# DeepakSridhar/fgdm

Hardware: AMD Instinct MI355X
Metric: 512x512 images/sec @ 50 DDIM steps, seg-ControlNet+CFG (higher is better)
Workload: dtype f16

## Files before the change

fgdm_amd/_lib.py:

```python
import ctypes as C
import os

HERE = os.path.dirname(os.path.abspath(__file__))
LIB_PATH = os.path.join(HERE, 'libfgdm_hip.so')

MAX_LEVELS = 8
MAX_CONTROLNETS = 4

FLAG_USE_ORIGINAL = 1
FLAG_ONLY_MID_CONTROL = 2
FLAG_NO_CONTROL = 4
FLAG_CFG_PAIRS = 8

ACT_NONE, ACT_SILU, ACT_RELU, ACT_GEGLU, ACT_QGELU = 0, 1, 2, 3, 4
OUT_F16, OUT_F32, OUT_F32_NCHW, OUT_F16_T = 0, 1, 2, 3
STRIDE2_PAD_BR = -2


class FgdmConfig(C.Structure):
    _fields_ = [
        ('in_channels', C.c_int32), ('out_channels', C.c_int32), ('model_channels', C.c_int32),
        ('num_res_blocks', C.c_int32), ('n_levels', C.c_int32), ('channel_mult', C.c_int32 * MAX_LEVELS),
        ('n_attention_resolutions', C.c_int32), ('attention_resolutions', C.c_int32 * MAX_LEVELS),
        ('num_heads', C.c_int32), ('context_dim', C.c_int32), ('use_adapter', C.c_int32),
        ('n_controlnets', C.c_int32), ('hint_channels', C.c_int32), ('workspace_bytes', C.c_int64),
        ('vae_ch', C.c_int32), ('vae_n_levels', C.c_int32), ('vae_ch_mult', C.c_int32 * MAX_LEVELS),
        ('vae_num_res_blocks', C.c_int32), ('vae_z_channels', C.c_int32), ('vae_out_ch', C.c_int32),
        ('clip_layers', C.c_int32), ('clip_width', C.c_int32), ('clip_heads', C.c_int32), ('clip_mlp', C.c_int32),
        ('clip_vocab', C.c_int32), ('clip_max_len', C.c_int32),
        ('n_extra_adapters', C.c_int32),
        ('vae_encoder', C.c_int32),
    ]


class FgdmConfig2(FgdmConfig):
    _fields_ = [('num_head_channels', C.c_int32), ('use_linear_in_transformer', C.c_int32)]


class FgdmDdimParams(C.Structure):
    _fields_ = [('struct_size', C.c_int64)] + [(name, C.c_void_p) for name in (
        'x', 'cond', 'uncond', 'timesteps', 'alphas', 'alphas_prev', 'sqrt_one_minus_alphas', 'control_scales', 'sigmas',
        'cfg_scales', 'step_noise', 'mask', 'x0', 'q_noise', 'sqrt_alphas_cumprod_t', 'sqrt_one_minus_alphas_cumprod_t',
        'log_steps', 'x_inter_out', 'pred_x0_out')] + [('cfg_scale', C.c_float)] + [(name, C.c_int32) for name in (
            'S', 'B', 'H', 'W', 'flags', 'n_log', 'reserved0')]


class FgdmPlmsParams(C.Structure):
    _fields_ = [('struct_size', C.c_int64)] + [(name, C.c_void_p) for name in (
        'x', 'cond', 'uncond', 'timesteps', 'alphas', 'alphas_prev', 'sqrt_one_minus_alphas', 'control_scales', 'mask', 'x0',
        'q_noise', 'sqrt_alphas_cumprod_t', 'sqrt_one_minus_alphas_cumprod_t', 'log_steps', 'x_inter_out', 'pred_x0_out')] + [
            ('cfg_scale', C.c_float)] + [(name, C.c_int32) for name in ('S', 'B', 'H', 'W', 'flags', 'n_log', 'reserved0')]


class FgdmDpmppParams(C.Structure):
    _fields_ = [('struct_size', C.c_int64)] + [(name, C.c_void_p) for name in (
        'x', 'cond', 'uncond', 'control_scales', 't_float', 'inv_alpha', 'neg_sigma_over_alpha', 'update_kind', 'c1', 'cm0',
        'cm1')] + [('cfg_scale', C.c_float)] + [(name, C.c_int32) for name in (
            'n_eval', 'B', 'H', 'W', 'flags', 'reserved0', 'reserved1')]


DPMPP_FIRST, DPMPP_SECOND = 1, 2
PLMS_PROBE, PLMS_FINISH_FIRST, PLMS_MULTISTEP = 0, 1, 2

_p = C.c_void_p
_f = C.c_float
_i = C.c_int
_i64 = C.c_int64

SIGNATURES = {
    'fgdm_create': (_i, [C.POINTER(FgdmConfig), _i, C.POINTER(_p)]),
    'fgdm_destroy': (None, [_p]),
    'fgdm_last_error': (C.c_char_p, [_p]),
    'fgdm_param_count': (_i, [C.POINTER(FgdmConfig)]),
    'fgdm_param_info': (_i, [C.POINTER(FgdmConfig), _i, C.c_char_p, _i, C.POINTER(_i64), C.POINTER(_i)]),
    'fgdm_load_tensor': (_i, [_p, C.c_char_p, _p, _i, C.POINTER(_i64), _i]),
    'fgdm_finalize_weights': (_i, [_p]),
    'fgdm_set_hint': (_i, [_p, _i, _p, _i, _i, _i, _p]),
    'fgdm_set_concat': (_i, [_p, _p, _i, _i, _i, _i, _p]),
    'fgdm_set_adapter_conds': (_i, [_p, _p, _i, _i, _i, _i, _p]),
    'fgdm_set_context': (_i, [_p, _p, _i, _p]),
    'fgdm_apply_model': (_i, [_p, _p, _p, _p, _p, _p, _p, _i, _i, _i, _i, _p, _p]),
    'fgdm_clip_encode': (_i, [_p, _p, _i, _i, _p, _p]),
    'fgdm_clip_encode_skip': (_i, [_p, _p, _i, _i, _i, _p, _p]),
    'fgdm_set_context_tokens': (_i, [_p, _i]),
    'fgdm_get_context_tokens': (_i, [_p]),
    'fgdm_run_block': (_i, [_p, C.c_char_p, _p, _i, _p, _i, _p, _p, _i, _i, _i, _p, _i64, C.POINTER(_i64), _p]),
    'fgdm_vae_decode': (_i, [_p, _p, _i, _i, _i, _f, _p, _p]),
    'fgdm_vae_encode': (_i, [_p, _p, _i, _i, _i, _p, _p]),
    'fgdm_unfold': (_i, [_p] + [_i] * 10 + [_p, _p]),
    'fgdm_fold_weighted': (_i, [_p, _p, _p] + [_i] * 9 + [_p, _p]),
    'fgdm_vae_decode_patches': (_i, [_p, _p, _i, _i, _i, _f] + [_i] * 5 + [_p, _p, _i, _p, _p]),
    'fgdm_apply_model_patches': (_i, [_p, _p, _p, _p, _p] + [_i] * 7 + [_p, _p, _i, _i, _p, _p]),
    'fgdm_posterior_sample': (_i, [_p, _p, _f, _p, _i, _i, _i, _p]),
    'fgdm_image_to_uint8': (_i, [_p, _i, _i, _i, _i, _i, _p, _p]),
    'fgdm_resize_linear_uint8': (_i, [_p, _i, _i, _i, _i, _i, _i, _p, _p]),
    'fgdm_uint8_to_hint': (_i, [_p, _i, _i, _i, _i, _p, _p]),
    'fgdm_controlnet': (_i, [_p, _i, _p, _p, _p, _i, _i, _i, _p, _i64, _p]),
    'fgdm_ddim_step': (_i, [_p, _p, _p, _f, _f, _f, _f, _f, _p, _p, _p, _p, _i64, _p]),
    'fgdm_plms_combine': (_i, [_p, _p, _p, _p, _i, _p, _i64, _p]),
    'fgdm_axpby': (_i, [_p, _f, _p, _f, _p, _i64, _p]),
    'fgdm_mask_blend': (_i, [_p, _p, _p, _p, _i64, _p]),
    'fgdm_ancestral_step': (_i, [_p, _p, _f, _f, _f, _f, _f, _p, _p, _i64, _p]),
    'fgdm_sample_ddim': (_i, [_p, _p, _p, _p, _f, _i, C.POINTER(_i64), C.POINTER(_f), C.POINTER(_f), C.POINTER(_f),
                              _p, _i, _i, _i, _i, _p]),
    'fgdm_sample_ddim_ex': (_i, [_p, C.POINTER(FgdmDdimParams), _p]),
    'fgdm_op_ddim_loop_step': (_i, [_p, _p, _p, _f, _f, _f, _f, _f, _p, _p, _p, _p, _f, _f, _p, _p, _p, _p, _p, _i64, _p]),
    'fgdm_sample_plms': (_i, [_p, C.POINTER(FgdmPlmsParams), _p]),
    'fgdm_sample_dpmpp': (_i, [_p, C.POINTER(FgdmDpmppParams), _p]),
    'fgdm_op_plms_loop_step': (_i, [_p, _p, _p, _f, _i, _i, _p, _p, _p, _p, _f, _f, _f, _p, _p, _p, _f, _f, _p, _p, _p, _p, _p,
                                    _i64, _p]),
    'fgdm_op_dpmpp_loop_step': (_i, [_p, _p, _p, _f, _f, _f, _p, _i, _f, _f, _f, _p, _p, _p, _p, _i64, _p]),
    'fgdm_profile_begin': (_i, [_p, _i]),
    'fgdm_profile_end': (_i, [_p, C.POINTER(C.c_double)]),
    'fgdm_workspace_stats': (_i, [_p, C.POINTER(_i64), C.POINTER(_i64)]),
    'fgdm_launch_stats': (_i, [_p, C.POINTER(_i64), C.POINTER(_i64), C.POINTER(_i64)]),
    'fgdm_replay_plan': (_i, [_i, _p, _p, _p, _p, _i, _i, _p, _i, _p]),
    'fgdm_op_conv2d': (_i, [_p, _i, _p, _i, _p, _p, _p, _p, _i, _i, _i, _i, _i, _i, _i, _i, _f, _p, _p]),
    'fgdm_op_linear': (_i, [_p, _p, _p, _p, _i, _i, _i, _i, _i, _i, _i, _p, _p]),
    'fgdm_debug_force_igemm_cfg': (_i, [_i]),
    'fgdm_bench_igemm': (_i, [_i] * 13 + [C.POINTER(_f)]),
    'fgdm_op_linear_ln_linear': (_i, [_p] * 8 + [_i] * 5 + [_p, _p, C.POINTER(_i), _p]),
    'fgdm_bench_norm': (_i, [_i] * 7 + [C.POINTER(_f)]),
    'fgdm_bench_attention': (_i, [_i] * 6 + [C.POINTER(_f)]),
    'fgdm_bench_ff': (_i, [_i] * 4 + [C.POINTER(_f)]),
    'fgdm_op_groupnorm': (_i, [_p, _i, _p, _i, _i, _i, _p, _p, _f, _i, _p, _p]),
    'fgdm_op_layernorm': (_i, [_p, _i, _i, _p, _p, _f, _p, _p]),
    'fgdm_op_attention': (_i, [_p, _i, _p, _i, _p, _i, _p, _i, _i, _i, _i, _i, _i, _p]),
    'fgdm_op_attention_ex': (_i, [_p, _i, _p, _i, _p, _i, _p, _i, _i, _i, _i, _i, _i, _i, _p]),
    'fgdm_debug_last_attention_kernel': (_i, []),
    'fgdm_op_small_attention': (_i, [_p, _i, _i, _i, _p, _i, _i, _i, _i, _i, _i, _p]),
    'fgdm_op_vae_attention': (_i, [_p, _p, _p, _p, _i, _i, _i, _p]),
    'fgdm_op_softmax_rows': (_i, [_p, _p, _i, _i, _p]),
    'fgdm_op_nchw_to_nhwc': (_i, [_p, _p, _i, _i, _i, _i, _p]),
    'fgdm_op_nhwc_to_nchw': (_i, [_p, _p, _i, _i, _i, _p]),
    'fgdm_op_pack_xcat': (_i, [_p, _p, _i, _i, _i, _i, _i, _i, _p, _p]),
    'fgdm_op_avgpool2': (_i, [_p, _p, _i, _i, _i, _i, _p]),
    'fgdm_op_transpose_pad': (_i, [_p, _p, _i, _i, _i, _i, _p]),
    'fgdm_op_timestep_embed': (_i, [_p, _p, _p, _i, _i, _i, _p]),
    'fgdm_op_add_f16': (_i, [_p, _p, _p, _i64, _p]),
    'fgdm_op_ln_qkv': (_i, [_p] * 6 + [_i] * 5 + [_p, _p, _p]),
}

_lib = None


def load():
    global _lib
    if _lib is not None:
        return _lib
    try:
        import torch
    except ImportError:
        pass
    path = os.environ.get('FGDM_LIB') or LIB_PATH
    if not os.path.exists(path):
        raise RuntimeError(f'{path} not found: build it with `python -m fgdm_amd.build` '
                           '(the HIP engine is mandatory, there is no CPU fallback)')
    lib = C.CDLL(os.path.abspath(path))
    for name, (res, args) in SIGNATURES.items():
        fn = getattr(lib, name)
        fn.restype = res
        fn.argtypes = args
    _lib = lib
    return lib
```

fgdm_amd/csrc/common.h:

```cpp
#pragma once
#include <hip/hip_runtime.h>
#include <stdint.h>

typedef _Float16 half_t;
typedef _Float16 h8 __attribute__((ext_vector_type(8)));
typedef _Float16 h4 __attribute__((ext_vector_type(4)));
typedef _Float16 h2 __attribute__((ext_vector_type(2)));
typedef float f32x16 __attribute__((ext_vector_type(16)));
typedef float f32x4 __attribute__((ext_vector_type(4)));

__device__ __forceinline__ float gelu_f(float x) {
    const float z = fminf(fabsf(x), 6.0f);
    float p = -4.7132482596e-04f;
    p = __builtin_fmaf(p, z, 7.0652551839e-03f);
    p = __builtin_fmaf(p, z, -5.1762067461e-02f);
    p = __builtin_fmaf(p, z, -4.6008771426e-01f);
    p = __builtin_fmaf(p, z, -1.1507295505e+00f);
    p = __builtin_fmaf(p, z, -4.8959157159e-05f - 1.0f);
    const float t = __builtin_amdgcn_exp2f(p);
    return __builtin_fmaf(fabsf(x), 0.5f - t, 0.5f * x);
}

typedef float f32x2 __attribute__((ext_vector_type(2)));
__device__ __forceinline__ f32x2 gelu2_f(f32x2 x) {
    const f32x2 ax = {fabsf(x[0]), fabsf(x[1])};
    const f32x2 z = {fminf(ax[0], 6.0f), fminf(ax[1], 6.0f)};
    auto c = [](float k) { return f32x2{k, k}; };
    f32x2 p = c(-4.7132482596e-04f);
    p = __builtin_elementwise_fma(p, z, c(7.0652551839e-03f));
    p = __builtin_elementwise_fma(p, z, c(-5.1762067461e-02f));
    p = __builtin_elementwise_fma(p, z, c(-4.6008771426e-01f));
    p = __builtin_elementwise_fma(p, z, c(-1.1507295505e+00f));
    p = __builtin_elementwise_fma(p, z, c(-4.8959157159e-05f - 1.0f));
    const f32x2 t = {__builtin_amdgcn_exp2f(p[0]), __builtin_amdgcn_exp2f(p[1])};
    return __builtin_elementwise_fma(ax, c(0.5f) - t, c(0.5f) * x);
}

__device__ __forceinline__ float silu_f(float x, float k = 1.0f) {
    return x * __builtin_amdgcn_rcpf(1.0f + __builtin_amdgcn_exp2f(-1.4426950408889634f * k * x));
}

__device__ __forceinline__ float ln_scale(float acc, float mean, float rstd, float u) {
    float t, w;
    asm("v_fma_f32 %0, %1, %2, %3" : "=v"(t) : "v"(-mean), "v"(u), "v"(acc));
    asm("v_mul_f32 %0, %1, %2" : "=v"(w) : "v"(rstd), "v"(t));
    return w;
}

#define FGDM_OK 0
#define FGDM_ERR_ARG -1
#define FGDM_ERR_HIP -2
#define FGDM_ERR_STATE -3
#define FGDM_ERR_NOMEM -4

enum IgemmMode { IG_LINEAR = 0, IG_CONV3 = 1, IG_CONV3_S2 = 2, IG_CONV3_UP2 = 3, IG_CONV3_S2_BR = 4, IG_CONV2_PHASE = 5 };
enum IgemmAct { ACT_NONE = 0, ACT_SILU = 1, ACT_RELU = 2, ACT_GEGLU = 3, ACT_QGELU = 4  };
enum IgemmOut { OUT_F16 = 0, OUT_F32 = 1, OUT_F32_NCHW = 2, OUT_F16_T = 3 };

struct IgemmArgs {
    const half_t* A0;
    const half_t* A1;
    const half_t* Wt;
    const float* bias;
    const float* rowvec;
    const half_t* resid;
    void* out;
    const half_t* zero;
    int C0, C1;
    int B, H, W;
    int Ho, Wo;
    int M, N;
    int K;
    int mode, act, out_kind;
    int ld_out, ld_res;
    int rv_stride;
    int rows_per_sample;
    float scale;
    int force_cfg;
    int splitk;
    float* ws;
    int debug;
    const float* ln_stats;
    const float* ln_u;
    int ln_slots;
    float ln_eps;
    float* stats_out;
    void* out2;
    int split_n, out_kind2, ld_out2;
};

int igemm_launch(const IgemmArgs& a, hipStream_t s);
bool igemm_up_phase(const IgemmArgs& a);
IgemmArgs igemm_phase_args(const IgemmArgs& a, const half_t* wt_phase);
void igemm_set_force_cfg(int cfg);
void igemm_set_twin_layers(bool on);
void igemm_set_pair_hint(int mult);
int igemm2_launch(const IgemmArgs& a, int cfg, hipStream_t s);
int igemm_stats_slots(const IgemmArgs& a);
int row_stats_slots(int C);
int row_stats_launch(const half_t* x, int rows, int C, float* stats , hipStream_t s);
int igemm_splitk_factor(const IgemmArgs& a);
int igemm_splitk_reduce(const IgemmArgs& a, hipStream_t s);
size_t igemm_npad(int n);

#define GN_PIX_PER_CHUNK 256
void groupnorm_set_group(bool on);
int groupnorm_launch(const half_t* x0, int C0, const half_t* x1, int C1, int B, int HW,
                     const float* gamma, const float* beta, float eps, int silu,
                     half_t* out, float* ws , hipStream_t s);
size_t groupnorm_ws_floats(int B, int HW);
int layernorm_launch(const half_t* x, int rows, int C, const float* gamma, const float* beta, float eps,
                     half_t* out, hipStream_t s);

int attention_launch(const half_t* Q, int ldq, const half_t* K, int ldk, const half_t* Vt, int ldvt,
                     half_t* O, int ldo, int B, int H, int T, int Tk, int d, int q_prescaled, hipStream_t s);
int attention_last_kernel();

int nchw_f32_to_nhwc_f16(const float* x, half_t* y, int B, int C, int HW, int Cpad, hipStream_t s);
int pack_xcat(const float* x, const half_t* cc, half_t* y, int B, int Bc, int Cc, int HW, int Cpad, hipStream_t s);
int f32_to_f16(const float* x, half_t* y, size_t n, hipStream_t s);
int silu_f32_to_f16(const float* x, half_t* y, size_t n, hipStream_t s);
int nhwc_f16_to_nchw_f32(const half_t* x, float* y, int B, int C, int HW, hipStream_t s);
int im2col3x3(const half_t* x, half_t* A, int B, int H, int W, int C, int stride, int Kpad, hipStream_t s);
int avgpool2(const half_t* x, half_t* y, int B, int H, int W, int C, hipStream_t s);
int add_f16(const half_t* a, const half_t* b, half_t* y, size_t n, hipStream_t s);
int add_f16_to_f32(const float* a, const half_t* b, float* y, size_t n, hipStream_t s);
int timestep_embed(const int64_t* t, const float* t_float, half_t* y, int B, int dim, int rows_pad, hipStream_t s);
int vae_prequant(const float* z, const float* wb, float scale, half_t* y, int B, int HW, hipStream_t s);
int vae_moments(const float* h, const float* wb, float* moments, int B, int HW, hipStream_t s);
int posterior_sample(const float* moments, const float* noise, float scale, float* z, int B, int zc, int HW, hipStream_t s);
int softmax_rows(const float* S, half_t* P, int rows, int cols, hipStream_t s);
int image_to_u8(const float* x, uint8_t* y, int B, int C, int HW, int mode, hipStream_t s);
int resize_linear_u8(const uint8_t* src, uint8_t* dst, int B, int H, int W, int C, int Ho, int Wo, hipStream_t s);
int u8_to_hint(const uint8_t* src, float* dst, int B, int HW, int C, hipStream_t s);
int embed_tokens(const int64_t* ids, const float* tok, const float* pos, float* out, int rows, int T, int W, int vocab,
                 hipStream_t s);
int layernorm32_launch(const float* x, int rows, int C, const float* gamma, const float* beta, float eps, half_t* out16,
                       float* out32, hipStream_t s);
int f16_to_f32(const half_t* x, float* y, size_t n, hipStream_t s);
int small_attention_launch(const half_t* qkv, int ld, int koff, int voff, half_t* out, int ldo, int B, int heads, int T,
                           int d, int causal, hipStream_t s);
int transpose_pad_keys(const half_t* v, half_t* vt, int B, int Tk, int C, int Tkpad, hipStream_t s);
int ddim_step(const float* x, const float* e_cond, const float* e_uncond, float cfg_scale,
              float a_t, float a_prev, float sigma_t, float sqrt_one_minus_at, const float* noise,
              float* x_prev, float* pred_x0, float* e_out, size_t n, hipStream_t s);
struct DdimLoopStep {
    const float *x, *ec, *eu, *noise, *mask, *x0, *qnoise;
    float *x_out, *xin_a, *xin_b, *log_x, *log_p0;
    float cfg, a_t, a_prev, sigma, s1m, sa_next, s1m_next;
    size_t n;
};
int ddim_loop_step(const DdimLoopStep& a, hipStream_t s);
enum { PLMS_PROBE = 0, PLMS_FINISH_FIRST = 1, PLMS_MULTISTEP = 2 };
struct PlmsLoopStep {
    const float *x, *ec, *eu, *e1, *e2, *e3, *mask, *x0, *qnoise;
    float *e_out, *x_out, *xin_a, *xin_b, *log_x, *log_p0;
    float cfg, a_t, a_prev, s1m, sa_next, s1m_next;
    int mode, order;
    size_t n;
};
int plms_loop_step(const PlmsLoopStep& a, hipStream_t s);
enum { DPMPP_FIRST = 1, DPMPP_SECOND = 2 };
struct DpmppLoopStep {
    const float *x, *ec, *eu, *m1;
    float *m0_out, *x_out, *xin_a, *xin_b;
    float cfg, inv_alpha, neg_sigma_over_alpha, c1, cm0, cm1;
    int kind;
    size_t n;
};
int dpmpp_loop_step(const DpmppLoopStep& a, hipStream_t s);
int plms_combine(const float* e_t, const float* e1, const float* e2, const float* e3, int order,
                 float* e_prime, size_t n, hipStream_t s);
int axpby(const float* a, float ca, const float* b, float cb, float* y, size_t n, hipStream_t s);
int mask_blend(const float* a, const float* b, const float* m, float* y, size_t n, hipStream_t s);
int ancestral_step(const float* x, const float* eps, float sqrt_recip, float sqrt_recipm1, float coef1, float coef2,
                   float std, const float* noise, float* out, size_t n, hipStream_t s);

struct PatchGeom { int B, C, H, W, kh, kw, sh, sw, Ly, Lx; };
int patch_plan(int H, int W, int kh, int kw, int sh, int sw, bool must_cover, int* Ly, int* Lx);
int unfold_crops(const float* x, float* out , const PatchGeom& g, int l0, int n, hipStream_t s);
int fold_accumulate(const float* o, const float* w_pix, const float* w_tie, float* acc, const PatchGeom& g, int l0, int n,
                    hipStream_t s);
int fold_finish(const float* acc, const float* w_pix, const float* w_tie, float* out, const PatchGeom& g, hipStream_t s);
int repeat_words(const void* src, void* dst , size_t words , int reps, hipStream_t s);

#define HIP_TRY(expr) do { hipError_t _e = (expr); if (_e != hipSuccess) return FGDM_ERR_HIP; } while (0)

template <auto Kernel>
int fgdm_dyn_lds(int bytes) {
    constexpr int MAXDEV = 64;
    static bool set[MAXDEV] = {};
    int dev = -1;
    if (hipGetDevice(&dev) != hipSuccess || dev < 0 || dev >= MAXDEV) return FGDM_ERR_HIP;
    if (!set[dev]) {
        HIP_TRY(hipFuncSetAttribute((const void*)Kernel, hipFuncAttributeMaxDynamicSharedMemorySize, bytes));
        set[dev] = true;
    }
    return FGDM_OK;
}

#include <functional>
#define FGDM_MAX_GROUP 5
bool fgdm_recording();
void fgdm_record(std::function<int(hipStream_t)> run);
#define FGDM_GROUP_BLOB sizeof(IgemmArgs)
typedef int (*FgdmGroupFn)(const void* const* args, int n, unsigned grid_x, hipStream_t s);
void fgdm_record(std::function<int(hipStream_t)> run, const void* key, FgdmGroupFn group, const void* args, size_t nbytes,
                 unsigned grid_x, unsigned long long shape);
#define FGDM_LAUNCH(kernel, grid, block, smem, stream, ...)                                                                  \
    do {                                                                                                                     \
        if (fgdm_recording()) {                                                                                              \
            fgdm_record([=](hipStream_t fgdm_s_) -> int {                                                                    \
                hipLaunchKernelGGL(kernel, grid, block, smem, fgdm_s_, __VA_ARGS__);                                         \
                return hipGetLastError() == hipSuccess ? FGDM_OK : FGDM_ERR_HIP;                                             \
            });                                                                                                              \
        } else {                                                                                                             \
            hipLaunchKernelGGL(kernel, grid, block, smem, stream, __VA_ARGS__);                                              \
        }                                                                                                                    \
    } while (0)
```

fgdm_amd/csrc/engine.hip:

```cpp
#include "model.h"
#include "knobs.h"
#include "replay.h"

#include <algorithm>
#include <array>
#include <cmath>
#include <cstdlib>
#include <cstdio>
#include <cstring>
#include <map>
#include <memory>
#include <string>
#include <unordered_map>
#include <vector>

namespace {

struct Arena {
    struct Blk { char* p; size_t sz; bool free; };
    std::vector<std::vector<Blk>> slabs;
    std::vector<char*> bases;
    size_t slab_bytes = (size_t)4 << 30;
    size_t in_use = 0, peak = 0;
    bool scoped = false;
// ... 174 lines not shown
        }
        g.N = N; g.K = K; g.k_real = K_src;
        g.w = upload(w);
        g.bias = upload(bias);
        g.ln_u = ln_gamma ? upload(lnu) : nullptr;
        if (ln_gamma && !kmap.empty()) return fail(FGDM_ERR_ARG, "LayerNorm fold: plain Linear weights only");
        return (g.w && g.bias && (!ln_gamma || g.ln_u)) ? FGDM_OK : fail(FGDM_ERR_NOMEM, "hipMalloc failed while packing weights");
    }
    int pack_linear(GemmW& g, const std::string& pre, bool has_bias, bool geglu = false, float wscale = 1.f,
                    const std::string& ln = std::string()) {
        const ParamSlot* w = slot(pre + ".weight");
        if (!w) return FGDM_ERR_STATE;
        const ParamSlot *lg = nullptr, *lb = nullptr;
        if (!ln.empty()) { lg = slot(ln + ".weight"); lb = slot(ln + ".bias"); if (!lg || !lb) return FGDM_ERR_STATE; }
        const ParamSlot* b = has_bias ? slot(pre + ".bias") : nullptr;
        if (has_bias && !b) return FGDM_ERR_STATE;
        const int N = (int)w->shape[0], K = (int)(w->numel() / w->shape[0]);
        if (K & 63) return fail(FGDM_ERR_ARG, "linear K not a multiple of 64: " + pre);
        if (lg && (int)lg->numel() != K) return fail(FGDM_ERR_ARG, "LayerNorm fold: width mismatch for " + pre);
        return pack_rows(g, {{w->host.data(), N}}, K, K, {}, {b ? b->host.data() : nullptr}, geglu, {wscale},
                         lg ? lg->host.data() : nullptr, lb ? lb->host.data() : nullptr);
    }
    int pack_stack(GemmW& g, const std::vector<std::string>& pres, bool has_bias, const std::vector<float>& scales = {},
                   const std::string& ln = std::string()) {
        const ParamSlot *lg = nullptr, *lb = nullptr;
        if (!ln.empty()) { lg = slot(ln + ".weight"); lb = slot(ln + ".bias"); if (!lg || !lb) return FGDM_ERR_STATE; }
        std::vector<std::pair<const float*, int>> srcs;
        std::vector<const float*> biases;
        int K = 0;
        for (auto& pre : pres) {
            const ParamSlot* w = slot(pre + ".weight");
            if (!w) return FGDM_ERR_STATE;
            K = (int)(w->numel() / w->shape[0]);
            srcs.push_back({w->host.data(), (int)w->shape[0]});
            if (has_bias) { const ParamSlot* b = slot(pre + ".bias"); if (!b) return FGDM_ERR_STATE; biases.push_back(b->host.data()); }
        }
        return pack_rows(g, srcs, K, K, {}, biases, false, scales, lg ? lg->host.data() : nullptr, lb ? lb->host.data() : nullptr);
    }
    int pack_conv3(GemmW& g, const std::string& pre, bool up = false) {
        const ParamSlot* w = slot(pre + ".weight");
        const ParamSlot* b = slot(pre + ".bias");
        if (!w || !b) return FGDM_ERR_STATE;
        const int N = (int)w->shape[0], Cin = (int)w->shape[1];
        int cp = 0;
        const std::vector<int> kmap = conv3_kmap(Cin, &cp);
        g.im2col = (Cin % 64) != 0;
        g.cin_pad = cp;
        g.wph = nullptr;
        if (up && Cin % 64 == 0 && N % 320 == 0) {
            g.wph = upload(up_phase_pack(w->host.data(), N, Cin, igemm_npad(N)));
            if (!g.wph) return fail(FGDM_ERR_NOMEM, "hipMalloc failed while packing weights");
        }
        return pack_rows(g, {{w->host.data(), N}}, Cin * 9, (int)kmap.size(), kmap, {b->host.data()}, false);
    }
    int pack_norm(NormW& n, const std::string& pre) {
        const ParamSlot* w = slot(pre + ".weight");
        const ParamSlot* b = slot(pre + ".bias");
        if (!w || !b) return FGDM_ERR_STATE;
        n.C = (int)w->shape[0];
        n.g = upload(w->host);
        n.b = upload(b->host);
        return (n.g && n.b) ? FGDM_OK : fail(FGDM_ERR_NOMEM, "hipMalloc failed");
    }
    int pack_pointwise(float** dst, const std::string& pre) {
        const ParamSlot* w = slot(pre + ".weight");
        const ParamSlot* b = slot(pre + ".bias");
        if (!w || !b) return FGDM_ERR_STATE;
        std::vector<float> wb(w->host);
        wb.insert(wb.end(), b->host.begin(), b->host.end());
        *dst = upload(wb);
        return *dst ? FGDM_OK : fail(FGDM_ERR_NOMEM, "hipMalloc failed");
    }
    int pack_table(float** dst, const std::string& name) {
        const ParamSlot* w = slot(name);
        if (!w) return FGDM_ERR_STATE;
        *dst = upload(w->host);
        return *dst ? FGDM_OK : fail(FGDM_ERR_NOMEM, "hipMalloc failed");
    }
    struct Packer {
        fgdm_engine& e;
        int rc = FGDM_OK;
        template <class F> void run(F pack) { if (rc == FGDM_OK) rc = pack(); }
        static float qscale(const LinOpt& o) { return o.q_head_dim ? 1.4426950408889634f / sqrtf((float)o.q_head_dim) : 1.f; }
        std::string fold(const LinOpt& o) const { return e.ln_fold ? o.ln : std::string(); }
        void layernorm(NormW& n, const std::string& pre, int C) { if (!e.ln_fold) norm(n, pre, C); }
        void norm(NormW& n, const std::string& pre, int) { run([&] { return e.pack_norm(n, pre); }); }
        void conv3(GemmW& g, const std::string& pre, int, int) { run([&] { return e.pack_conv3(g, pre); }); }
        void conv3_up(GemmW& g, const std::string& pre, int, int) { run([&] { return e.pack_conv3(g, pre, true); }); }
        void pointwise(float*& dst, const std::string& pre, int, int) { run([&] { return e.pack_pointwise(&dst, pre); }); }
        void table(float*& dst, const std::string& key, int, int) { run([&] { return e.pack_table(&dst, key); }); }
        void source(const std::string&, int, int, bool) {}
        void linear(GemmW& g, const std::string& pre, int, int, bool, bool bias, const LinOpt& o = LinOpt()) {
            run([&] { return e.pack_linear(g, pre, bias, o.geglu, qscale(o), fold(o)); });
        }
        void stack(GemmW& g, const std::vector<std::string>& pres, bool bias, const LinOpt& o = LinOpt()) {
            run([&] { return e.pack_stack(g, pres, bias, o.q_head_dim ? std::vector<float>{qscale(o)} : std::vector<float>(), fold(o)); });
        }
    };
    int repack(int c) {
        Component& comp = comps[c];
        if (comp.packed && !comp.dirty) return FGDM_OK;
        for (auto& name : order) {
            const ParamSlot& ps = params[name];
            if (ps.comp == c && ps.loaded && ps.host.empty())
                return fail(FGDM_ERR_STATE, "tensor " + name + " was released after packing: reload every tensor of " + comp.prefix +
                                            " before finalizing again");
        }
        for (void* p : comp.allocs) (void)hipFree(p);
        comp.allocs.clear();
        cur_comp = c;
        Packer pk{*this};
        visit_component(c, pk);
        cur_comp = -1;
        if (pk.rc != FGDM_OK) return pk.rc;
        for (auto& name : order) { ParamSlot& ps = params[name]; if (ps.comp == c) std::vector<float>().swap(ps.host); }
        comp.packed = true;
        comp.dirty = false;
        return FGDM_OK;
    }

#define CHK(x) do { int _rc = (x); if (_rc != FGDM_OK) return _rc; } while (0)
    int dcopy(void* dst, const void* src, size_t bytes) {
        auto run = [=](hipStream_t rs) -> int { return hipMemcpyAsync(dst, src, bytes, hipMemcpyDeviceToDevice, rs) == hipSuccess ? FGDM_OK : FGDM_ERR_HIP; };
        if (!fgdm_recording()) return run(s);
        fgdm_record(run);
        return FGDM_OK;
    }
    int dzero(void* dst, size_t bytes) {
        auto run = [=](hipStream_t rs) -> int { return hipMemsetAsync(dst, 0, bytes, rs) == hipSuccess ? FGDM_OK : FGDM_ERR_HIP; };
        if (!fgdm_recording()) return run(s);
        fgdm_record(run);
        return FGDM_OK;
    }
    Tensor talloc(int B, int H, int W, int C) {
        Tensor t; t.B = B; t.H = H; t.W = W; t.C = C;
        t.p = (half_t*)ar->alloc(t.numel() * sizeof(half_t));
        return t;
    }
    void tfree(Tensor& t) { ar->release(t.p); t.p = nullptr; }

    struct LnStats { float* p = nullptr; int slots = 0; };
    struct Epi {
        const LnStats* ln = nullptr;
        LnStats* stats = nullptr;
        int act = ACT_NONE;
        const float* rowvec = nullptr; int rv_stride = 0;
        const half_t* resid = nullptr; int ld_res = 0;
        float scale = 1.f;
        int out_kind = OUT_F16;
        void* out = nullptr;
        int ld_out = 0;
        void* out2 = nullptr; int out_kind2 = OUT_F16, ld_out2 = 0, split_n = 0;
        int rps = 0;
    };
    int gemm(const GemmW& w, int mode, const Tensor& x0, const Tensor* x1, int Ho, int Wo, const Epi& e, Tensor* out) {
        IgemmArgs a{};
        a.A0 = x0.p; a.C0 = x0.C;
        a.A1 = x1 ? x1->p : nullptr; a.C1 = x1 ? x1->C : 0;
        a.Wt = w.w; a.bias = w.bias;
        a.rowvec = e.rowvec; a.rv_stride = e.rv_stride;
        a.resid = e.resid; a.ld_res = e.ld_res;
        a.zero = zero;
        a.B = x0.B; a.H = x0.H; a.W = x0.W; a.Ho = Ho; a.Wo = Wo;
        a.M = x0.B * Ho * Wo;
        a.N = w.N;
        a.K = w.K;
        a.mode = mode; a.act = e.act; a.out_kind = e.out_kind;
        const int nout = e.act == ACT_GEGLU ? w.N / 2 : w.N;
        a.out = e.out ? e.out : (void*)out->p;
        a.ld_out = e.ld_out ? e.ld_out : nout;
        a.rows_per_sample = e.rps ? e.rps : Ho * Wo;
        a.scale = e.scale;
        a.out2 = e.out2; a.out_kind2 = e.out_kind2; a.ld_out2 = e.ld_out2; a.split_n = e.split_n;
        const int taps = mode == IG_LINEAR ? 1 : 9;
        if (taps * (a.C0 + a.C1) != a.K) return fail(FGDM_ERR_ARG, "gemm: K mismatch");
        if (!a.out) return fail(FGDM_ERR_NOMEM, "gemm: null output (workspace exhausted?)");
        if (w.wph && !e.stats && !e.ln && igemm_up_phase(a)) a = igemm_phase_args(a, w.wph);
        char tag[56] = "";
        if (prof.on) snprintf(tag, sizeof(tag), "igemm M%d N%d K%d mode%d act%d out%d l%ds%dr%dv%d", a.M, a.N, a.K, a.mode, a.act, a.out_kind,
                              e.ln ? 1 : 0, e.stats ? 1 : 0, e.resid ? 1 : 0, e.rowvec ? 1 : 0);
        a.splitk = igemm_splitk_factor(a);
        if (a.splitk > 1) {
            a.ws = (float*)ar->alloc((size_t)a.splitk * a.M * a.N * sizeof(float));
            if (!a.ws) return fail(FGDM_ERR_NOMEM, "workspace (split-K partials)");
        }
        if (e.ln) {
            if (!w.ln_u || !e.ln->p || a.splitk > 1) return fail(FGDM_ERR_STATE, "gemm: LayerNorm fold without folded weights / statistics");
            a.ln_stats = e.ln->p; a.ln_slots = e.ln->slots; a.ln_u = w.ln_u; a.ln_eps = w.ln_eps;
        } else if (w.ln_u) {
            return fail(FGDM_ERR_STATE, "gemm: these weights have a LayerNorm folded in; statistics are required");
        }
        if (e.stats) {
            e.stats->slots = igemm_stats_slots(a);
            e.stats->p = (float*)ar->alloc((size_t)a.M * std::max(e.stats->slots, row_stats_slots(nout)) * 2 * sizeof(float));
            if (!e.stats->p) return fail(FGDM_ERR_NOMEM, "workspace (LayerNorm statistics)");
            if (e.stats->slots) a.stats_out = e.stats->p;
        }
        double nbytes = 0.0;
        if (prof.on) {
            const double in_b = 2.0 * ((double)x0.numel() + (x1 ? (double)x1->numel() : 0.0));
            const double out_b = (double)a.M * nout * (e.out_kind == OUT_F16 || e.out_kind == OUT_F16_T ? 2.0 : 4.0);
            nbytes = in_b + 2.0 * (double)w.N * w.K + out_b + (e.resid ? 2.0 * (double)a.M * nout : 0.0);
        }
        prof.begin(PC_IGEMM, s, 2.0 * (double)x0.B * Ho * Wo * (double)w.N * (double)w.k_real, tag, nbytes);
        int rc = igemm_launch(a, s);
        prof.end(s);
        if (a.ws) ar->release(a.ws);
        if (rc == FGDM_OK && e.stats && e.stats->slots == 0) {
            if (a.out_kind != OUT_F16 || a.ld_out != nout) return fail(FGDM_ERR_ARG, "gemm: row statistics need a dense fp16 output");
            e.stats->slots = row_stats_slots(nout);
            prof.begin(PC_NORM, s, 2.0 * (double)a.M * nout, "row_stats");
            rc = row_stats_launch((const half_t*)a.out, a.M, nout, e.stats->p, s);
            prof.end(s);
        }
        return rc == FGDM_OK ? rc : fail(rc, "igemm launch failed");
    }
    int conv3(const GemmW& w, const Tensor& x, const Tensor* x1, int stride, bool up, Epi e, Tensor* out) {
        int Ho = x.H, Wo = x.W, mode = IG_CONV3;
        if (up) { Ho *= 2; Wo *= 2; mode = IG_CONV3_UP2; }
        else if (stride == 2) { Ho = (x.H - 1) / 2 + 1; Wo = (x.W - 1) / 2 + 1; mode = IG_CONV3_S2; }
        else if (stride == FGDM_STRIDE2_PAD_BR) { Ho = (x.H - 2) / 2 + 1; Wo = (x.W - 2) / 2 + 1; mode = IG_CONV3_S2_BR; }
        const bool own_out = (e.out == nullptr);
        if (own_out) { *out = talloc(x.B, Ho, Wo, w.N); if (!out->p) return fail(FGDM_ERR_NOMEM, "workspace"); }
        if (!w.im2col) return gemm(w, mode, x, x1, Ho, Wo, e, out);
        if (up || x1 || x.C != w.cin_pad || stride == FGDM_STRIDE2_PAD_BR) return fail(FGDM_ERR_ARG, "im2col conv path: unsupported combination");
        Tensor A = talloc(1, 1, x.B * Ho * Wo, w.K);
        if (!A.p) return fail(FGDM_ERR_NOMEM, "workspace (im2col)");
        prof.begin(PC_ELEM, s, 2.0 * (double)A.numel() + 2.0 * (double)x.numel());
        bool in_gemm = false;
        const int rc = im2col_conv(x.p, A.p, x.B, x.H, x.W, x.C, stride, w.K, s, [&]() { prof.end(s); },
            [&](half_t* Ap, int Bv, int Hv, int Wv, int Kv, int rps) {
                in_gemm = true;
                Tensor Av; Av.p = Ap; Av.B = Bv; Av.H = Hv; Av.W = Wv; Av.C = Kv;
                if (!e.rps) e.rps = rps;
                return gemm(w, IG_LINEAR, Av, nullptr, Hv, Wv, e, out);
            });
        if (rc != FGDM_OK && !in_gemm) return fail(rc, "im2col failed");
        tfree(A);
        return rc;
    }
    int linear(const GemmW& w, const Tensor& x, Epi e, Tensor* out, const Tensor* x1 = nullptr) {
        if (!e.out) { *out = talloc(x.B, x.H, x.W, e.act == ACT_GEGLU ? w.N / 2 : w.N); if (!out->p) return fail(FGDM_ERR_NOMEM, "workspace"); }
        return gemm(w, IG_LINEAR, x, x1, x.H, x.W, e, out);
    }
    int gnorm(const NormW& n, const Tensor& x, const Tensor* x1, float eps, bool silu, Tensor* out) {
        const int C = x.C + (x1 ? x1->C : 0);
        *out = talloc(x.B, x.H, x.W, C);
        float* ws = (float*)ar->alloc(groupnorm_ws_floats(x.B, x.H * x.W) * sizeof(float));
        if (!out->p || !ws) return fail(FGDM_ERR_NOMEM, "workspace");
        char tag[56] = "";
        if (prof.on) snprintf(tag, sizeof(tag), "groupnorm B%d HW%d C%d", x.B, x.H * x.W, C);
        prof.begin(PC_NORM, s, 4.0 * (double)out->numel(), tag);
        const int rc = groupnorm_launch(x.p, x.C, x1 ? x1->p : nullptr, x1 ? x1->C : 0, x.B, x.H * x.W, n.g, n.b, eps,
                                        silu ? 1 : 0, out->p, ws, s);
        prof.end(s);
        ar->release(ws);
        return rc == FGDM_OK ? rc : fail(rc, "groupnorm launch failed");
    }
    int lnorm(const NormW& n, const Tensor& x, Tensor* out) {
        *out = talloc(x.B, x.H, x.W, x.C);
        if (!out->p) return fail(FGDM_ERR_NOMEM, "workspace");
        char tag[56] = "";
        if (prof.on) snprintf(tag, sizeof(tag), "layernorm rows%d C%d", x.rows(), x.C);
        prof.begin(PC_NORM, s, 4.0 * (double)out->numel(), tag);
        const int rc = layernorm_launch(x.p, x.rows(), x.C, n.g, n.b, 1e-5f, out->p, s);
        prof.end(s);
        return rc == FGDM_OK ? rc : fail(rc, "layernorm launch failed");
    }

    struct EmbCtx { const float* emb_all; int stride; };

    int res_fwd(const Layer& l, const Tensor& x, const Tensor* x1, const EmbCtx& ec, Tensor* out) {
        Tensor g1, h, g2, sk, xp;
        CHK(gnorm(l.gn1, x, x1, l.eps, true, &g1));
        const Tensor* xs = &x;
        if (l.down) {
            if (x1) return fail(FGDM_ERR_ARG, "down ResBlock with a concatenated input");
            Tensor gp = talloc(x.B, x.H / 2, x.W / 2, x.C);
            xp = talloc(x.B, x.H / 2, x.W / 2, x.C);
            if (!gp.p || !xp.p) return fail(FGDM_ERR_NOMEM, "workspace");
            if (avgpool2(g1.p, gp.p, x.B, x.H, x.W, x.C, s) != FGDM_OK || avgpool2(x.p, xp.p, x.B, x.H, x.W, x.C, s) != FGDM_OK)
                return fail(FGDM_ERR_ARG, "avgpool2: latent size must be divisible by 8 for the adapter");
            tfree(g1);
            g1 = gp;
            xs = &xp;
        }
        Epi e1;
        if (l.emb_off >= 0) { e1.rowvec = ec.emb_all + l.emb_off; e1.rv_stride = ec.stride; }
        CHK(conv3(l.c1, g1, nullptr, 1, false, e1, &h));
        tfree(g1);
        CHK(gnorm(l.gn2, h, nullptr, l.eps, true, &g2));
        tfree(h);
        Epi e2;
        if (l.cin != l.cout) {
            CHK(linear(l.skip, *xs, Epi{}, &sk, x1));
            e2.resid = sk.p; e2.ld_res = sk.C;
        } else {
            e2.resid = xs->p; e2.ld_res = xs->C;
        }
        CHK(conv3(l.c2, g2, nullptr, 1, false, e2, out));
        tfree(g2);
        if (sk.p) tfree(sk);
        if (xp.p) tfree(xp);
        return FGDM_OK;
    }

    int cross_kv(const Layer& l, const Tensor& ctx16, bool persistent, Tensor* k2, Tensor* v2t) {
        const int B = ctx16.B, C = l.cin, Tk = ctx16.H * ctx16.W, Tkp = roundup(Tk, 64);
        if (persistent) {
            k2->B = B; k2->H = ctx16.H; k2->W = ctx16.W; k2->C = C;
            v2t->B = B; v2t->H = 1; v2t->W = C; v2t->C = Tkp;
            if (hipMalloc(&k2->p, k2->numel() * sizeof(half_t)) != hipSuccess ||
                hipMalloc(&v2t->p, v2t->numel() * sizeof(half_t)) != hipSuccess) return fail(FGDM_ERR_NOMEM, "hipMalloc (context cache)");
            { Epi e; e.out = k2->p; e.ld_out = C; CHK(linear(l.k2, ctx16, e, nullptr)); }
        } else {
            CHK(linear(l.k2, ctx16, Epi{}, k2));
            *v2t = talloc(B, 1, C, Tkp);
            if (!v2t->p) return fail(FGDM_ERR_NOMEM, "workspace");
        }
        if (Tkp != Tk) CHK(dzero(v2t->p, v2t->numel() * sizeof(half_t)));
        { Epi e; e.out_kind = OUT_F16_T; e.out = v2t->p; e.ld_out = Tkp; e.rps = Tk; CHK(linear(l.v2, ctx16, e, nullptr)); }
        return FGDM_OK;
    }
    void drop_context() {
        for (auto& kv : ctx_cache) { (void)hipFree(kv.second.k.p); (void)hipFree(kv.second.vt.p); }
        ctx_cache.clear();
        ctx_B = 0;
    }
    int set_context(const float* ctx, int B) {
        if (!finalized) return fail(FGDM_ERR_STATE, "weights not finalized");
        if (B <= 0) return fail(FGDM_ERR_ARG, "bad shape");
        drop_context();
        Tensor ctx16 = talloc(B, 1, ctx_tokens, cfg.context_dim);
        if (!ctx16.p) return fail(FGDM_ERR_NOMEM, "workspace");
        if (f32_to_f16(ctx, ctx16.p, ctx16.numel(), s) != FGDM_OK) return fail(FGDM_ERR_HIP, "convert kernel");
        auto walk = [&](const Block& blk) -> int {
            for (const Layer& l : blk)
                if (l.type == L_ATTN) { CtxKV kv; CHK(cross_kv(l, ctx16, true, &kv.k, &kv.vt)); ctx_cache[&l] = kv; }
            return FGDM_OK;
        };
        CHK(for_each_block(unet, false, walk));
        for (auto& n : cns) CHK(for_each_block(n, false, walk));
        tfree(ctx16);
        ctx_B = B; ctx_T = ctx_tokens;
        return FGDM_OK;
    }

    int attn_fwd(const Layer& l, const Tensor& x_in, const Tensor& ctx16, Tensor* out, bool dup = false) {
        Tensor x = x_in, x_full;
        int B = x.B;
        const int T = x.H * x.W, C = x.C, d = C / l.heads;
        Tensor g, h, qk, vt, a, h2, q2, k2, v2t, f;
        LnStats s1, s2, s3;
        CHK(gnorm(l.gn, x, nullptr, 1e-6f, false, &g));
        Tensor nrm;
        { Epi e; if (ln_fold) e.stats = &s1; CHK(linear(l.pin, g, e, &h)); }
        tfree(g);
        if (!ln_fold) CHK(lnorm(l.ln1, h, &nrm));
        const Tensor& a1 = ln_fold ? h : nrm;
        const int Tp = roundup(T, 64);
        qk = talloc(B, x.H, x.W, 2 * C);
        vt = talloc(B, 1, C, Tp);
        if (!qk.p || !vt.p) return fail(FGDM_ERR_NOMEM, "workspace");
        if (Tp != T) CHK(dzero(vt.p, vt.numel() * sizeof(half_t)));
        { Epi e; if (ln_fold) e.ln = &s1; e.out = qk.p; e.ld_out = 2 * C; e.rps = T;
          e.out2 = vt.p; e.out_kind2 = OUT_F16_T; e.ld_out2 = Tp; e.split_n = 2 * C;
          CHK(linear(l.qkv1, a1, e, nullptr)); }
        if (s1.p) ar->release(s1.p);
        if (nrm.p) tfree(nrm);
        a = talloc(B, x.H, x.W, C);
        if (!a.p) return fail(FGDM_ERR_NOMEM, "workspace");
        { char tag[56]; snprintf(tag, sizeof(tag), "attn B%d T%d Tk%d d%d", B, T, T, d);
          prof.begin(PC_ATTN, s, 4.0 * (double)B * T * (double)T * C, tag);
          int rc = attention_launch(qk.p, 2 * C, qk.p + C, 2 * C, vt.p, Tp, a.p, C, B, l.heads, T, T, d, 1, s);
          prof.end(s);
          if (rc != FGDM_OK) return fail(rc, "attention launch failed (unsupported head dim?)"); }
        tfree(qk); tfree(vt);
        { Epi e; e.resid = h.p; e.ld_res = C; if (ln_fold) e.stats = &s2; CHK(linear(l.o1, a, e, &h2)); }
        tfree(a); tfree(h);
        if (dup) {
            Tensor f2;
            CHK(dup_rows(h2, &f2)); tfree(h2); h2 = f2;
            CHK(dup_rows(x, &x_full)); x = x_full;
            B *= 2;
        }
        if (dup && ln_fold) {
            const size_t sb = (size_t)(B / 2) * T * s2.slots * 2 * sizeof(float);
            float* s2f = (float*)ar->alloc(2 * sb);
            if (!s2f) return fail(FGDM_ERR_NOMEM, "workspace");
            CHK(dcopy(s2f, s2.p, sb));
            CHK(dcopy((char*)s2f + sb, s2.p, sb));
            ar->release(s2.p); s2.p = s2f;
        }
        if (!ln_fold) CHK(lnorm(l.ln2, h2, &nrm));
        { Epi e; if (ln_fold) e.ln = &s2; CHK(linear(l.q2, ln_fold ? h2 : nrm, e, &q2)); }
        if (s2.p) ar->release(s2.p);
        if (nrm.p) tfree(nrm);
        int Tk, Tkp;
        const bool cached = (ctx16.p == nullptr);
        if (cached) {
            auto it = ctx_cache.find(&l);
            if (it == ctx_cache.end() || ctx_B != B) return fail(FGDM_ERR_STATE, "no cached context for this batch (fgdm_set_context)");
            k2 = it->second.k; v2t = it->second.vt;
            Tk = ctx_T; Tkp = roundup(Tk, 64);
        } else {
            Tk = ctx16.H * ctx16.W; Tkp = roundup(Tk, 64);
            CHK(cross_kv(l, ctx16, false, &k2, &v2t));
        }
        a = talloc(B, x.H, x.W, C);
        if (!a.p) return fail(FGDM_ERR_NOMEM, "workspace");
        { char tag[56]; snprintf(tag, sizeof(tag), "attn B%d T%d Tk%d d%d", B, T, Tk, d);
          prof.begin(PC_ATTN, s, 4.0 * (double)B * T * (double)Tk * C, tag);
          int rc = attention_launch(q2.p, C, k2.p, C, v2t.p, Tkp, a.p, C, B, l.heads, T, Tk, d, 1, s);
          prof.end(s);
          if (rc != FGDM_OK) return fail(rc, "attention launch failed"); }
        tfree(q2);
        if (!cached) { tfree(k2); tfree(v2t); }
        { Epi e; e.resid = h2.p; e.ld_res = C; if (ln_fold) e.stats = &s3; CHK(linear(l.o2, a, e, &h)); }
        tfree(a); tfree(h2);
        if (!ln_fold) CHK(lnorm(l.ln3, h, &nrm));
        { Epi e; if (ln_fold) e.ln = &s3; e.act = ACT_GEGLU; CHK(linear(l.ffp, ln_fold ? h : nrm, e, &f)); }
        if (s3.p) ar->release(s3.p);
        if (nrm.p) tfree(nrm);
        { Epi e; e.resid = h.p; e.ld_res = C; CHK(linear(l.ffo, f, e, &h2)); }
        tfree(f); tfree(h);
        { Epi e; e.resid = x.p; e.ld_res = C; CHK(linear(l.pout, h2, e, out)); }
        tfree(h2);
        if (x_full.p) tfree(x_full);
        return FGDM_OK;
    }

    int dup_rows(const Tensor& h, Tensor* full) {
        *full = talloc(2 * h.B, h.H, h.W, h.C);
        if (!full->p) return fail(FGDM_ERR_NOMEM, "workspace");
        const size_t bytes = h.numel() * sizeof(half_t);
        CHK(dcopy(full->p, h.p, bytes));
        CHK(dcopy((char*)full->p + bytes, h.p, bytes));
        return FGDM_OK;
    }
    int block_fwd_shared(const Block& blk, Tensor xh, bool own_x, const EmbCtx& ec, const Tensor& ctx16, Tensor* out) {
        Tensor cur = xh;
        bool own = own_x, full = false;
        for (size_t j = 0; j < blk.size(); ++j) {
            const Layer& l = blk[j];
            Tensor nxt;
            switch (l.type) {
                case L_CONV: CHK(conv3(l.conv, cur, nullptr, 1, false, Epi{}, &nxt)); break;
// ... 1370 lines not shown
```

fgdm_amd/csrc/igemm.hip:

```cpp
#include "common.h"
#include "knobs.h"
#include <algorithm>

#define LDS_AS __attribute__((address_space(3)))
#define GLB_AS __attribute__((address_space(1)))

__device__ __forceinline__ void glds16(const void* g, void* lds_wave_base) {
    __builtin_amdgcn_global_load_lds((const GLB_AS void*)g, (LDS_AS void*)lds_wave_base, 16, 0, 0);
}

template <int BM, int BN, int WM, int WN>
__global__ __launch_bounds__(WM * WN * 64) void igemm_kernel(const IgemmArgs a) {
    constexpr int T = WM * WN * 64;
    constexpr int TM = BM / WM, TN = BN / WN;
    constexpr int MI = TM / 32, NI = TN / 32;
    constexpr int A_IT = BM * 8 / T, B_IT = BN * 8 / T;
    constexpr int A_BYTES = BM * 128, STAGE = (BM + BN) * 128;
    static_assert(A_IT >= 1 && B_IT >= 1, "tile too small for the thread count");
    extern __shared__ __attribute__((aligned(16))) char smem[];

    const int tid = threadIdx.x, lane = tid & 63;
    const int wave = __builtin_amdgcn_readfirstlane(tid >> 6);
    const int wm = wave / WN, wn = wave % WN;

// ... 168 lines not shown
            float gbias = 0.f;
            if (geglu) gbias = a.bias ? a.bias[pcol + 32] : 0.f;
            const int ocol = geglu ? ((pcol >> 6) << 5) + lrow : pcol - ncol0;
            float rvv[16];
#pragma unroll
            for (int r = 0; r < 16; ++r) {
                const int row = m0 + wm * TM + i * 32 + (r & 3) + 8 * (r >> 2) + 4 * lh;
                rvv[r] = (a.rowvec && row < a.M) ? a.rowvec[(size_t)(row / rps) * a.rv_stride + pcol] : 0.f;
            }
#pragma unroll
            for (int g = 0; g < 4; ++g) {
                const int row0 = m0 + wm * TM + i * 32 + 8 * g + 4 * lh;
                float v[4];
#pragma unroll
                for (int e = 0; e < 4; ++e) {
                    const int row = row0 + e;
                    float x = acc[i][j][g * 4 + e] + bias + rvv[g * 4 + e];
                    if (a.act == ACT_SILU) x = silu_f(x);
                    else if (a.act == ACT_RELU) x = fmaxf(x, 0.f);
                    else if (a.act == ACT_QGELU) x = silu_f(x, 1.702f);
                    else if (geglu) {
                        if constexpr (NI >= 2) x = x * gelu_f(acc[i][j | 1][g * 4 + e] + gbias);
                    }
                    v[e] = x * a.scale;
                }
                if (okind == OUT_F16) {
                    half_t* o = (half_t*)outp;
#pragma unroll
                    for (int e = 0; e < 4; ++e) {
                        const int row = row0 + e;
                        if (row < a.M) {
                            half_t x = (half_t)v[e];
                            if (a.resid) x = (half_t)((float)x + (float)a.resid[(size_t)row * a.ld_res + ocol]);
                            o[(size_t)row * ldo + ocol] = x;
                        }
                    }
                } else if (okind == OUT_F32) {
                    float* o = (float*)outp;
#pragma unroll
                    for (int e = 0; e < 4; ++e)
                        if (row0 + e < a.M) o[(size_t)(row0 + e) * ldo + ocol] = v[e];
                } else {
                    const bool vec = ((rps & 3) == 0) && (row0 + 3 < a.M);
                    if (vec) {
                        const int b = row0 / rps, t = row0 - b * rps;
                        const size_t off = ((size_t)b * nchan + ocol) * ldo + t;
                        if (okind == OUT_F16_T) {
                            h4 pk = {(half_t)v[0], (half_t)v[1], (half_t)v[2], (half_t)v[3]};
                            *(h4*)((half_t*)outp + off) = pk;
                        } else {
                            f32x4 pk = {v[0], v[1], v[2], v[3]};
                            *(f32x4*)((float*)outp + off) = pk;
                        }
                    } else {
#pragma unroll
                        for (int e = 0; e < 4; ++e) {
                            const int row = row0 + e;
                            if (row < a.M) {
                                const int b = row / rps, t = row - b * rps;
                                const size_t off = ((size_t)b * nchan + ocol) * ldo + t;
                                if (okind == OUT_F16_T) ((half_t*)outp)[off] = (half_t)v[e];
                                else ((float*)outp)[off] = v[e];
                            }
                        }
                    }
                }
            }
        }
    }
}

size_t igemm_npad(int n) { return (size_t)((n + 127) / 128) * 128; }

template <int BM, int BN, int WM, int WN>
static int launch_cfg(const IgemmArgs& a, hipStream_t s) {
    constexpr int smem = 2 * (BM + BN) * 128;
    constexpr auto k = igemm_kernel<BM, BN, WM, WN>;
    if (fgdm_dyn_lds<k>(smem) != FGDM_OK) return FGDM_ERR_HIP;
    const int ntm = (a.M + BM - 1) / BM, ntn = (a.N + BN - 1) / BN;
    FGDM_LAUNCH(k, dim3(ntm * ntn), dim3(WM * WN * 64), smem, s, a);
    return hipGetLastError() == hipSuccess ? FGDM_OK : FGDM_ERR_HIP;
}

static int g_force_cfg = 0;
void igemm_set_force_cfg(int cfg) { g_force_cfg = cfg; }
static thread_local int g_pair_mult = 1;
void igemm_set_pair_hint(int mult) { g_pair_mult = mult > 1 ? mult : 1; }

static int pick_force(const IgemmArgs& a) {
    int force = a.force_cfg ? a.force_cfg : g_force_cfg;
    if (a.act == ACT_QGELU) {
        if (force >= 4) force = 0;
        if (force == 0) return 0;
    }
    const bool small_tiles = knob_once(KNOB_IGEMM_SMALL_TILES) != 0;
    const bool other_widths = knob_once(KNOB_IGEMM_OTHER_WIDTHS) != 0;
    if (a.mode == IG_CONV2_PHASE) {
        if (force >= 4) return force;
        return (long)((a.M + 255) / 256) * (a.N / 320) * 4 * g_pair_mult >= 192 ? 4 : 6;
    }
    if (force == 0) {
        const bool geglu = a.act == ACT_GEGLU;
        if (!geglu && a.N % 320 == 0) {
            const long b256 = (long)((a.M + 255) / 256) * (a.N / 320);
            const long b128 = (long)((a.M + 127) / 128) * (a.N / 320);
            const bool small_m = knob_once(KNOB_IGEMM_SMALL_M) != 0;
            const bool lin64 = a.mode == IG_LINEAR && !(a.K & 31) && !(a.C0 & 31) && !(a.C1 & 31) && small_tiles;
            const long b64 = (long)((a.M + 63) / 64) * (a.N / 160);
            const long b256n = (long)((a.M + 255) / 256) * (a.N / 128);
            if (b256 * g_pair_mult >= 192) force = 4;
            else if (small_m && lin64 && a.K >= 2560 && !(a.N % 128) && !a.ln_stats && !a.stats_out && !a.out2 && b128 >= 96 && b128 * g_pair_mult < 192 &&
                     b64 >= 512 && b256n >= 144 && b256n <= 256) force = 10;
            else if (b128 >= 96 && !(small_m && lin64 && b128 * g_pair_mult < 192 && b64 >= 512)) force = 6;
            else if (lin64 && b64 >= 128) force = 11;
        } else if (geglu && a.N % 256 == 0 && (long)((a.M + 255) / 256) * (a.N / 256) >= 128) {
            force = 5;
        } else if (!geglu && !a.ln_stats && !(a.K & 31) && !(a.C0 & 31) && !(a.C1 & 31) && other_widths) {
            const long rows = (a.M + 255) / 256;
            if (a.N % 256 == 0 && rows * (a.N / 256) >= 192) force = 5;
            else if (a.N == 128 && rows >= 192) force = 10;
        }
    }
    return force;
}

int igemm_stats_slots(const IgemmArgs& a) {
    if (a.out_kind != OUT_F16 || a.act == ACT_GEGLU || a.splitk > 1 || (a.N % 320) || (a.K & 31) || (a.C0 & 31) || (a.C1 & 31)) return 0;
    const int f = pick_force(a);
    if (f < 4) return 0;
    const int tile = (f - 4) & 15;
    const bool stats64 = knob_once(KNOB_IGEMM_STATS64) != 0;
    return (tile == 0 || tile == 2 || tile == 3 || tile == 5 || (tile == 7 && stats64)) ? a.N / 160 : 0;
}

bool igemm_up_phase(const IgemmArgs& a) {
    if (!knob_once(KNOB_IGEMM_UP_PHASE)) return false;
    const int force = a.force_cfg ? a.force_cfg : g_force_cfg;
    if (force >= 1 && force <= 3) return false;
    if (a.H * a.W < 64) return false;
    return a.mode == IG_CONV3_UP2 && !a.C1 && a.C0 > 0 && !(a.C0 & 63) && a.K == 9 * a.C0 && a.N % 320 == 0 && a.out_kind == OUT_F16 &&
           a.act != ACT_GEGLU && a.act != ACT_QGELU && !a.rowvec && !a.stats_out && !a.out2 && !a.ln_stats;
}
IgemmArgs igemm_phase_args(const IgemmArgs& a, const half_t* wt_phase) {
    IgemmArgs p = a;
    p.mode = IG_CONV2_PHASE;
    p.Wt = wt_phase;
    p.K = 4 * a.C0;
    p.M = a.B * a.H * a.W;
    p.rows_per_sample = a.H * a.W;
    p.splitk = 1; p.ws = nullptr;
    return p;
}

int igemm_launch(const IgemmArgs& a, hipStream_t s) {
    if (a.M <= 0 || a.N <= 0 || a.K <= 0 || (a.K & 63) || (a.C0 & 63) || (a.C1 & 63)) return FGDM_ERR_ARG;
    if (a.act == ACT_GEGLU && (a.N & 63)) return FGDM_ERR_ARG;
    if (a.ln_stats && (a.mode != IG_LINEAR || a.C1 || a.ln_slots <= 0 || !a.ln_u)) return FGDM_ERR_ARG;
    if (a.stats_out && igemm_stats_slots(a) == 0) return FGDM_ERR_ARG;
    if (a.out2 && (a.act == ACT_GEGLU || a.splitk > 1 || a.stats_out || a.split_n <= 0 || a.split_n >= a.N || (a.split_n % 640))) return FGDM_ERR_ARG;
    if (a.mode == IG_CONV2_PHASE && (a.splitk > 1 || a.N % 320)) return FGDM_ERR_ARG;
    if (a.splitk > 1) {
        if (!a.ws || a.ln_stats) return FGDM_ERR_ARG;
        const bool fat = (long)((a.M + 255) / 256) * (a.N / 320) * a.splitk >= 192 && !(a.K & 31) && !(a.C0 & 31) && !(a.C1 & 31);
        const int rc = igemm2_launch(a, fat ? 0 : 2, s);
        return rc == FGDM_OK ? igemm_splitk_reduce(a, s) : rc;
    }
    int force = pick_force(a);
    const bool mfma32 = knob_once(KNOB_IGEMM_MFMA32) != 0;
    if (mfma32 && force >= 4 && force <= 6 && !a.force_cfg && !g_force_cfg) force += 3;
    if (force >= 4) return igemm2_launch(a, force - 4, s);
    struct Cfg { int bm, bn; float eff; int per_cu; };
    static const Cfg cfgs[] = {{128, 128, 1.00f, 2}, {128, 64, 0.80f, 3}, {64, 64, 0.62f, 4}};
    int best = 0;
    float best_cost = 1e30f;
    for (int i = 0; i < 3; ++i) {
        const Cfg& c = cfgs[i];
        const long nblk = (long)((a.M + c.bm - 1) / c.bm) * ((a.N + c.bn - 1) / c.bn);
        const long slots = 256L * c.per_cu;
        const float rounds = (float)((nblk + slots - 1) / slots);
        const long conc = std::min<long>(c.per_cu, (nblk + 255) / 256);
        const float cost = rounds * (float)conc * (float)(c.bm * c.bn) / c.eff;
        if (cost < best_cost) { best_cost = cost; best = i; }
    }
    if ((long)((a.M + 127) / 128) * ((a.N + 127) / 128) < 256) best = 2;
    if (a.act == ACT_GEGLU) best = 0;
    if (force >= 1 && force <= 3) best = force - 1;
    switch (best) {
        case 0: return launch_cfg<128, 128, 2, 2>(a, s);
        case 1: return launch_cfg<128, 64, 2, 2>(a, s);
        default: return launch_cfg<64, 64, 2, 2>(a, s);
    }
}
```

fgdm_amd/csrc/igemm2.hip:

```cpp
#include "common.h"
#include "knobs.h"
#include <algorithm>
#include <type_traits>

#pragma clang diagnostic ignored "-Winline-asm"
#define LDS_AS __attribute__((address_space(3)))
#define GLB_AS __attribute__((address_space(1)))

namespace {

__device__ __forceinline__ void glds16(const void* g, unsigned lds_wave_addr) {
    unsigned keep;
    asm volatile("s_mov_b32 %0, m0\n\ts_mov_b32 m0, %2\n\ts_nop 0\n\tglobal_load_lds_dwordx4 %1, off\n\ts_mov_b32 m0, %0"
                 : "=&s"(keep)
                 : "v"(g), "s"(lds_wave_addr)
                 : "memory", "m0");
}
__device__ __forceinline__ void glds16_m0(const void* g, unsigned lds_wave_addr) {
    asm volatile("s_mov_b32 m0, %1\n\ts_nop 0\n\tglobal_load_lds_dwordx4 %0, off" ::"v"(g), "s"(lds_wave_addr) : "memory", "m0");
}
__device__ __forceinline__ void glds16_sv(unsigned voff, const void* sbase, unsigned lds_wave_addr) {
    asm volatile("s_mov_b32 m0, %2\n\ts_nop 0\n\tglobal_load_lds_dwordx4 %0, %1" ::"v"(voff), "s"(sbase), "s"(lds_wave_addr) : "memory", "m0");
}
__device__ __forceinline__ unsigned lds_addr(const void* p) { return (unsigned)(size_t)(LDS_AS const void*)p; }
template <int N> __device__ __forceinline__ void wait_vmcnt() {
    asm volatile("s_waitcnt vmcnt(%0)" ::"n"(N) : "memory");
}

constexpr int BK = 32;
constexpr int ROWB = BK * 2;

constexpr int RV_MAX = 6;

template <int BM> constexpr int halo_px() { return BM == 256 ? 400 : 272; }
template <int BM, int BN, int STAGES, int PIPE> constexpr int ring_bytes() {
    return PIPE == 2 ? 2 * halo_px<BM>() * ROWB + STAGES * BN * ROWB : STAGES * (BM + BN) * ROWB;
}

template <int BM, int BN, int WM, int WN, int STAGES, int CONV, bool GEGLU, bool SPLIT, int MS, bool LN, int PATH, int PIPE, bool ABL>
__device__ __forceinline__ void igemm2_body(const IgemmArgs& a, const int yb) {
    constexpr int NW = WM * WN, T = NW * 64;
    constexpr int TM = BM / WM, TN = BN / WN;
    constexpr int MI = TM / MS, NI = TN / MS;
    constexpr int KS = MS == 32 ? 2 : 1;
    constexpr int AR = MS == 32 ? 16 : 4;
    typedef float acc_t __attribute__((ext_vector_type(AR)));
    auto swz_of = [](int r) { return MS == 32 ? ((r >> 2) & 3) : (((r >> 3) & 1) << 1); };
    constexpr int A_INSTR = BM * 4 / 64, B_INSTR = BN * 4 / 64;
    static_assert(A_INSTR % NW == 0, "A tile must split evenly over the waves");
    constexpr int LA = A_INSTR / NW, LB = (B_INSTR + NW - 1) / NW;
    constexpr int LPS = LA + LB;
    constexpr int STAGE_BYTES = (BM + BN) * ROWB;
    constexpr int A_BYTES = BM * ROWB;
    constexpr int RING_BYTES = ring_bytes<BM, BN, STAGES, PIPE>();
    static_assert(TM % 32 == 0 && TN % MS == 0, "wave tile: 32-pixel epilogue passes, MFMA-sized channel tiles");
    static_assert(!GEGLU || TN % 64 == 0, "GEGLU: whole 64-row [32 value | 32 gate] groups per wave");
    extern __shared__ __attribute__((aligned(16))) char smem[];

    const int tid = threadIdx.x, lane = tid & 63;
    const int wave = __builtin_amdgcn_readfirstlane(tid >> 6);
    const int wm = wave / WN, wn = wave % WN;

    const int ntn = (a.N + BN - 1) / BN;
    const int nb = gridDim.x;
    int logical;
    {
        const int bid = blockIdx.x, xcd = bid & 7, q = nb >> 3, r = nb & 7;
        logical = (xcd < r ? xcd * (q + 1) : r * (q + 1) + (xcd - r) * q) + (bid >> 3);
    }
    const int nsplit = SPLIT ? a.splitk : 1;
    int split = 0, m0, n0;
    if (SPLIT) {
        const int ntm = (a.M + BM - 1) / BM;
        const int row = logical % ntm, pair = logical / ntm;
        split = pair % nsplit; n0 = (pair / nsplit) * BN; m0 = row * BM;
    } else {
        m0 = (logical / ntn) * BM; n0 = (logical % ntn) * BN;
    }

    const int nk_all = a.K >> 5;
    const int per = (nk_all + nsplit - 1) / nsplit;
    const int k_begin = split * per;
    const int nk = max(0, min(per, nk_all - k_begin));

    int a_pix[LA], a_yx[LA], a_off[LA];
    int b_off[LB], b_lds[LB];
    const int br = (CONV && a.mode == IG_CONV3_S2_BR) ? 1 : 0;
    const int sy = (CONV && (a.mode == IG_CONV3_S2 || a.mode == IG_CONV3_S2_BR)) ? 2 : 1;
    const int up = (CONV && a.mode == IG_CONV3_UP2) ? 1 : 0;
    constexpr bool ph = CONV == 2;
    const int pa = ph ? (yb >> 1) : 0, pb = ph ? (yb & 1) : 0;
    const int NT = ph ? 4 : 9;
    const int Wq = ph ? a.W : a.Wo, hwq = ph ? a.H * a.W : a.Ho * a.Wo;
    const half_t* const Wt = ph ? a.Wt + (size_t)yb * (size_t)((a.N + 127) / 128 * 128) * (size_t)a.K : a.Wt;
#pragma unroll
    for (int i = 0; i < LA; ++i) {
        const int q = (wave + i * NW) * 64 + lane, r = q >> 2, s = q & 3;
        a_off[i] = (s ^ swz_of(r)) << 3;
        a_pix[i] = -1; a_yx[i] = 0;
        const int m = m0 + r;
        if (PIPE == 0 && m < a.M) {
            if (!CONV) {
                a_pix[i] = m;
            } else {
                const int b = m / hwq, rem = m - b * hwq;
                const int oy = rem / Wq, ox = rem - oy * Wq;
                a_pix[i] = b * a.H * a.W;
                a_yx[i] = ((oy * sy + br) << 16) | (ox * sy + br);
            }
        }
    }
#pragma unroll
    for (int i = 0; i < LB; ++i) {
        int idx = wave + i * NW;
        if (idx >= B_INSTR) idx = B_INSTR - 1;
        const int q = idx * 64 + lane, r = q >> 2, s = q & 3;
        b_off[i] = (n0 + r) * a.K + ((s ^ swz_of(r)) << 3);
        b_lds[i] = A_BYTES + idx * 1024;
    }
    const unsigned Hu = (unsigned)(a.H << up), Wu = (unsigned)(a.W << up);
    unsigned a_b0[LA], a_b1[LA], a_msk[LA], b_b[LB];
    if constexpr (PIPE == 2) {
#pragma unroll
        for (int i = 0; i < LB; ++i) b_b[i] = (unsigned)b_off[i] * 2u;
    }
    if constexpr (PIPE == 1) {
#pragma unroll
        for (int i = 0; i < LA; ++i) {
            a_b0[i] = a_b1[i] = a_msk[i] = 0;
            const int q = (wave + i * NW) * 64 + lane, r = q >> 2;
            const int m = m0 + r;
            if (m < a.M) {
                unsigned cen = (unsigned)m;
                a_msk[i] = 1;
                if (CONV) {
                    const int b = m / hwq, rem = m - b * hwq;
                    const int oy = (rem / Wq) * sy + br, ox = (rem - (rem / Wq) * Wq) * sy + br;
                    cen = (unsigned)(b * a.H * a.W + (oy >> up) * a.W + (ox >> up));
                    unsigned msk = 0;
#pragma unroll
                    for (int t = 0; t < 9; ++t) {
                        const int uy = oy + (ph ? pa - 1 + (t >> 1) : t / 3 - 1), ux = ox + (ph ? pb - 1 + (t & 1) : t % 3 - 1);
                        if ((!ph || t < 4) && (unsigned)uy < Hu && (unsigned)ux < Wu) msk |= 1u << t;
                    }
                    if (up) msk |= ((oy & 1) ? 0u : 1u << 16) | ((ox & 1) ? 0u : 1u << 17);
                    a_msk[i] = msk;
                }
                a_b0[i] = (cen * (unsigned)a.C0 + (unsigned)a_off[i]) * 2u;
                a_b1[i] = (cen * (unsigned)a.C1 + (unsigned)a_off[i]) * 2u;
            }
        }
#pragma unroll
        for (int i = 0; i < LB; ++i) b_b[i] = (unsigned)b_off[i] * 2u;
    }

    auto stage_piece = [&](int kt, int tap, int cc, int buf, int p) {
        const unsigned base = __builtin_amdgcn_readfirstlane(lds_addr(smem) + buf * STAGE_BYTES);
        if (p < LA) {
            const int i = p;
            const half_t* src = a.A0;
            int Cs = a.C0, co = cc;
            if (co >= a.C0) { src = a.A1; Cs = a.C1; co -= a.C0; }
            const int ky = ph ? pa - 1 + (tap >> 1) : tap / 3 - 1, kx = ph ? pb - 1 + (tap & 1) : tap - (tap / 3) * 3 - 1;
            const half_t* ptr = a.zero;
            if (!CONV) {
                if (a_pix[i] >= 0) ptr = src + (size_t)a_pix[i] * Cs + co + a_off[i];
            } else {
                const int uy = (a_yx[i] >> 16) + ky, ux = (a_yx[i] & 0xffff) + kx;
                if (a_pix[i] >= 0 && (unsigned)uy < Hu && (unsigned)ux < Wu)
                    ptr = src + (size_t)(a_pix[i] + (uy >> up) * a.W + (ux >> up)) * Cs + co + a_off[i];
            }
            if constexpr (ABL) { if (a.debug & 8) ptr = a.zero; }
            glds16(ptr, base + (wave + i * NW) * 1024);
        } else {
            const int i = p - LA;
            const half_t* ptr = Wt + (size_t)b_off[i] + (ph ? (size_t)(tap * a.C0 + cc) : ((size_t)(k_begin + kt) << 5));
            if constexpr (ABL) { if (a.debug & 8) ptr = a.zero; }
            glds16(ptr, base + b_lds[i]);
        }
    };
    auto stage = [&](int kt, int tap, int cc, int buf) {
#pragma unroll
        for (int p = 0; p < LPS; ++p) stage_piece(kt, tap, cc, buf, p);
    };

    acc_t acc[NI][MI];
#pragma unroll
    for (int j = 0; j < NI; ++j)
#pragma unroll
        for (int i = 0; i < MI; ++i)
#pragma unroll
            for (int r = 0; r < AR; ++r) acc[j][i][r] = 0.f;

    const int lrow = lane & (MS - 1), lh = lane / MS, swz = swz_of(lrow);
    const int lq = 4 * lh;
    int koff[KS];
#pragma unroll
    for (int ks = 0; ks < KS; ++ks) koff[ks] = lrow * ROWB + ((((MS == 32 ? ks * 2 : 0) + lh) ^ swz) << 4);

    int tap = 0, cc = k_begin << 5;
    if (CONV) { const int q = k_begin >> 1; tap = q % NT; cc = (q / NT) * 64 + (k_begin & 1) * 32; }
    auto advance = [&]() {
        if (!CONV) { cc += 32; return; }
        if (cc & 32) {
            if (++tap == NT) { tap = 0; cc += 32; } else { cc -= 32; }
        } else {
            cc += 32;
        }
    };
    struct StageSc { const char* sbase; const char* wbase; unsigned lbase; bool s1; int tap; int dyE, dyO, dxE, dxO; };
    auto stage_scalars = [&](int kn, int tap, int cc) {
        StageSc sc;
        sc.s1 = cc >= a.C0;
        const half_t* src = sc.s1 ? a.A1 : a.A0;
        const int Cs = sc.s1 ? a.C1 : a.C0;
        int disp = sc.s1 ? cc - a.C0 : cc;
        const int ky = ph ? pa - 1 + (tap >> 1) : tap / 3 - 1, kx = ph ? pb - 1 + (tap & 1) : tap - (tap / 3) * 3 - 1;
        sc.dyE = sc.dyO = sc.dxE = sc.dxO = 0;
        if (CONV) {
            if (!up) {
                disp += (ky * a.W + kx) * Cs;
            } else {
                sc.dyE = ky < 0 ? -a.W * Cs * 2 : 0; sc.dyO = ky > 0 ? a.W * Cs * 2 : 0;
                sc.dxE = kx < 0 ? -Cs * 2 : 0;       sc.dxO = kx > 0 ? Cs * 2 : 0;
            }
        }
        sc.sbase = (const char*)src + (ptrdiff_t)disp * 2;
        sc.wbase = (const char*)Wt + (ph ? ((size_t)(tap * a.C0 + cc) << 1) : ((size_t)(k_begin + kn) << 6));
        sc.lbase = __builtin_amdgcn_readfirstlane(lds_addr(smem) + (kn & 3) * STAGE_BYTES);
        sc.tap = tap;
        return sc;
    };
    auto lean_piece = [&](const StageSc& sc, int p) {
        bool zsrc = false;
        if constexpr (ABL) zsrc = (a.debug & 8) != 0;
        if (p < LA) {
            unsigned off = sc.s1 ? a_b1[p] : a_b0[p];
            if (CONV && up) off += (unsigned)(((a_msk[p] >> 16) & 1 ? sc.dyE : sc.dyO) + ((a_msk[p] >> 17) & 1 ? sc.dxE : sc.dxO));
            const char* ptr = ((a_msk[p] >> sc.tap) & 1) ? sc.sbase + off : (const char*)a.zero;
            if constexpr (ABL) { if (zsrc) ptr = (const char*)a.zero; }
            glds16_m0(ptr, sc.lbase + (wave + p * NW) * 1024);
        } else if (ABL && zsrc) {
            glds16_m0(a.zero, sc.lbase + b_lds[p - LA]);
        } else {
            glds16_sv(b_b[p - LA], sc.wbase, sc.lbase + b_lds[p - LA]);
        }
    };
    auto advance_bf = [&]() {
        if (!CONV) { cc += 32; return; }
        const bool second = (cc & 32) != 0, wrap = second && tap == NT - 1;
        cc = second ? (wrap ? cc + 32 : cc - 32) : cc + 32;
        tap = second ? (wrap ? 0 : tap + 1) : tap;
    };
#pragma unroll
    for (int s = 0; s < STAGES - 1; ++s) {
        if (PIPE != 2 && s < nk) {
            if constexpr (PIPE == 0) { stage(s, tap, cc, s); advance(); }
            else if constexpr (PIPE == 1) {
                const StageSc sc = stage_scalars(s, tap, cc);
#pragma unroll
                for (int pp = 0; pp < LPS; ++pp) lean_piece(sc, pp);
                advance_bf();
            }
        }
    }

    float* bias_l = (float*)(smem + RING_BYTES);
    float* rv_l = bias_l + BN;
    float* mr_l = rv_l + RV_MAX * BN;
    float* u_l = mr_l + 2 * BM;
    const int rps = a.rows_per_sample;
    const int smp0 = m0 / rps;
    const int last_row = min(m0 + BM, a.M) - 1;
    const int nsmp = a.rowvec ? last_row / rps - smp0 + 1 : 0;
    const bool rv_in_lds = nsmp <= RV_MAX;
    for (int c = tid; c < BN; c += T) bias_l[c] = a.bias ? a.bias[n0 + c] : 0.f;
    if constexpr (LN) {
        for (int c = tid; c < BN; c += T) u_l[c] = a.ln_u[n0 + c];
        for (int r = tid; r < BM; r += T) {
            float mean = 0.f, rstd = 0.f;
            if (m0 + r < a.M) {
                const float* sp = a.ln_stats + (size_t)(m0 + r) * a.ln_slots * 2;
                float sm = 0.f, sq = 0.f;
                for (int p = 0; p < a.ln_slots; ++p) { sm += sp[2 * p]; sq += sp[2 * p + 1]; }
                const double mu = (double)sm / (double)a.C0;
                double var = (double)sq / (double)a.C0 - mu * mu;
                if (var < 0.0) var = 0.0;
                mean = (float)mu;
                rstd = (float)(1.0 / sqrt(var + (double)a.ln_eps));
            }
            mr_l[2 * r] = mean; mr_l[2 * r + 1] = rstd;
        }
    }
    if (a.rowvec && rv_in_lds)
        for (int c = tid; c < nsmp * BN; c += T) {
            const int sidx = c / BN, ch = c - sidx * BN;
            rv_l[c] = a.rowvec[(size_t)(smp0 + sidx) * a.rv_stride + n0 + ch];
        }

    if constexpr (PIPE == 0) {
        auto wait_stage = [&](int k_needed) {
            const int younger = min(nk - 1 - k_needed, STAGES - 2);
            if (STAGES >= 4 && younger >= 2) wait_vmcnt<2 * LPS>();
            else if (STAGES >= 3 && younger == 1) wait_vmcnt<LPS>();
            else wait_vmcnt<0>();
        };
        for (int kt = 0; kt < nk; ++kt) {
            wait_stage(kt);
            __builtin_amdgcn_s_waitcnt(0xC07F);
            __builtin_amdgcn_s_barrier();
            bool refill = kt + STAGES - 1 < nk;
            if constexpr (ABL) refill = refill && !(a.debug & 1);
            if (refill) { stage(kt + STAGES - 1, tap, cc, (kt + STAGES - 1) % STAGES); advance(); }
            const char* As = smem + (kt % STAGES) * STAGE_BYTES + (wm * TM) * ROWB;
            const char* Bs = smem + (kt % STAGES) * STAGE_BYTES + A_BYTES + (wn * TN) * ROWB;
            h8 xf[KS][MI], wf[KS][NI];
#pragma unroll
            for (int ks = 0; ks < KS; ++ks) {
#pragma unroll
                for (int i = 0; i < MI; ++i) xf[ks][i] = *(const h8*)(As + i * MS * ROWB + koff[ks]);
#pragma unroll
                for (int j = 0; j < NI; ++j) wf[ks][j] = *(const h8*)(Bs + j * MS * ROWB + koff[ks]);
            }
            __builtin_amdgcn_sched_barrier(0);
#pragma unroll
            for (int ks = 0; ks < KS; ++ks)
#pragma unroll
                for (int j = 0; j < NI; ++j)
#pragma unroll
                    for (int i = 0; i < MI; ++i) {
                        if constexpr (MS == 32) acc[j][i] = __builtin_amdgcn_mfma_f32_32x32x16_f16(wf[ks][j], xf[ks][i], acc[j][i], 0, 0, 0);
                        else acc[j][i] = __builtin_amdgcn_mfma_f32_16x16x32_f16(wf[ks][j], xf[ks][i], acc[j][i], 0, 0, 0);
                    }
        }
    } else if constexpr (PIPE == 2) {
        static_assert(CONV && MS == 16 && STAGES == 4 && !ABL, "halo loop: 3x3 stride-1 convolution on the 16x16x32 MFMA");
        constexpr int RW = NI % 5 == 0 ? 5 : 4, WD = 3;
        static_assert(NI % RW == 0 && WD < RW && NI >= RW, "W ring");
        constexpr int HB = halo_px<BM>() * ROWB, HPCS = halo_px<BM>() / 16;
        constexpr int LH = (HPCS + NW - 1) / NW;
        constexpr int WST = BN * ROWB;
        const int Wd = a.W, Pp = Wd + 2, hwp = a.H * a.W;
        const bool whole = hwp < BM;
        const int RS = whole ? a.H : BM / Wd, HP1 = (RS + 2) * Pp, NSL = whole ? BM / hwp : 1, NPX = NSL * HP1;
        const int bimg = m0 / hwp, y0 = whole ? 0 : (m0 - bimg * hwp) / Wd;
        const int nsub = nk / 9, sub0 = k_begin / 9;
        unsigned h_pix[LH], h_pc[LH];
        bool h_ok[LH];
#pragma unroll
        for (int u = 0; u < LH; ++u) {
            const int q = (wave + u * NW) * 64 + lane, hp = q >> 2, sp = q & 3;
            const int img = hp / HP1, rem = hp - img * HP1, hr = rem / Pp, hx = rem - hr * Pp, y = y0 + hr - 1, x = hx - 1;
            h_ok[u] = hp < NPX && (unsigned)x < (unsigned)Wd && (unsigned)y < (unsigned)a.H && bimg + img < a.B;
            h_pix[u] = h_ok[u] ? (unsigned)((bimg + img) * hwp + y * Wd + x) : 0u;
            h_pc[u] = (unsigned)((sp ^ ((hp >> 2) & 3)) << 4);
        }
        const unsigned lds_h = __builtin_amdgcn_readfirstlane(lds_addr(smem)), lds_w = lds_h + 2 * HB;
        auto issue_halo = [&](int sub) {
            const int cch = (sub0 + sub) << 5;
            const bool s1 = cch >= a.C0;
            const char* sb = s1 ? (const char*)(a.A1 + (cch - a.C0)) : (const char*)(a.A0 + cch);
            const unsigned rowb = (unsigned)(s1 ? a.C1 : a.C0) * 2u;
            const unsigned lb = lds_h + (unsigned)(sub & 1) * HB;
#pragma unroll
            for (int u = 0; u < LH; ++u)
                if (wave + u * NW < HPCS) {
                    const char* ptr = h_ok[u] ? sb + (h_pix[u] * rowb + h_pc[u]) : (const char*)a.zero;
                    glds16_m0(ptr, lb + (unsigned)(wave + u * NW) * 1024u);
                }
        };
        auto w_src = [&](int sub, int tp) { const int sa = sub0 + sub; return (const char*)a.Wt + ((size_t)(((sa >> 1) * 9 + tp) * 64 + (sa & 1) * 32) << 1); };
        auto issue_w = [&](int kn, int sub, int tp, int p) { glds16_sv(b_b[p], w_src(sub, tp), lds_w + (unsigned)(kn & 3) * WST + (unsigned)(b_lds[p] - A_BYTES)); };
        int hpc[MI];
#pragma unroll
        for (int i = 0; i < MI; ++i) {
            const int pl = wm * TM + i * MS + lrow, img = pl / (RS * Wd), rem = pl - img * RS * Wd, r = rem / Wd, x = rem - r * Wd;
            hpc[i] = img * HP1 + (r + 1) * Pp + x + 1;
        }
        auto rdXh = [&](int sub, int tp, int i) {
            const int hp = hpc[i] + (tp / 3 - 1) * Pp + (tp - (tp / 3) * 3 - 1);
            return *(const h8*)(smem + (sub & 1) * HB + hp * ROWB + ((lh ^ ((hp >> 2) & 3)) << 4));
        };
        auto rdWh = [&](int kt, int j) { return *(const h8*)(smem + 2 * HB + (kt & 3) * WST + (wn * TN + j * MS) * ROWB + koff[0]); };
        int subI = 0, tapI = 0;
        auto next_st = [](int& sub, int& tp) { const bool wrap = tp == 8; tp = wrap ? 0 : tp + 1; sub += wrap ? 1 : 0; };
        issue_halo(0);
#pragma unroll
        for (int sg = 0; sg < STAGES - 1; ++sg)
            if (sg < nk) {
#pragma unroll
                for (int p2 = 0; p2 < LB; ++p2) issue_w(sg, subI, tapI, p2);
                next_st(subI, tapI);
            }
        h8 xa[MI], xb[MI], wr[RW];
        {
            const int younger = min(nk - 1, STAGES - 2);
            if (younger >= 2) wait_vmcnt<2 * LB>(); else if (younger == 1) wait_vmcnt<LB>(); else wait_vmcnt<0>();
            __builtin_amdgcn_s_barrier();
#pragma unroll
            for (int i = 0; i < MI; ++i) xa[i] = rdXh(0, 0, i);
#pragma unroll
            for (int d = 0; d < WD; ++d) wr[d] = rdWh(0, d);
        }
        int subK = 0, tapK = 0, subR = 0, tapR = 1;
        auto step = [&](auto RF, int kt, h8 (&cur)[MI], h8 (&nxt)[MI]) {
            constexpr bool REFILL = decltype(RF)::value;
            if (REFILL || kt + 2 < nk) wait_vmcnt<LB>(); else wait_vmcnt<0>();
            __builtin_amdgcn_s_waitcnt(0xC07F);
            __builtin_amdgcn_s_barrier();
            if (tapK == 0 && subK + 1 < nsub) issue_halo(subK + 1);
#pragma unroll
            for (int j = 0; j < NI; ++j) {
                __builtin_amdgcn_sched_barrier(0);
                if constexpr (REFILL) {
#pragma unroll
                    for (int p2 = 0; p2 < LB; ++p2)
                        if (p2 * NI / LB == j) issue_w(kt + STAGES - 1, subI, tapI, p2);
                }
                { const int jn = j + WD; wr[jn % RW] = jn < NI ? rdWh(kt, jn) : rdWh(kt + 1, jn - NI); }
#pragma unroll
                for (int i = 0; i < MI; ++i)
                    if (i * NI / MI == j) nxt[i] = rdXh(subR, tapR, i);
#pragma unroll
                for (int i = 0; i < MI; ++i)
                    acc[j][i] = __builtin_amdgcn_mfma_f32_16x16x32_f16(wr[j % RW], cur[i], acc[j][i], 0, 0, 0);
            }
            __builtin_amdgcn_sched_barrier(0);
            if constexpr (REFILL) next_st(subI, tapI);
// ... 169 lines not shown
                if (PATH == 2 || (PATH == 0 && a.rowvec)) {
                    if (PATH == 2 || rv_in_lds) {
                        const f32x4 rq = *(const f32x4*)(rw + wc);
#pragma unroll
                        for (int e = 0; e < 4; ++e) v[e] += rq[e];
                    } else if (row < a.M) {
#pragma unroll
                        for (int e = 0; e < 4; ++e) v[e] += a.rowvec[(size_t)bsmp * a.rv_stride + n0 + wn * TN + wc + e];
                    }
                }
                if (PATH == 0 && a.act == ACT_SILU) {
#pragma unroll
                    for (int e = 0; e < 4; ++e) v[e] = silu_f(v[e]);
                } else if (PATH == 0 && a.act == ACT_RELU) {
#pragma unroll
                    for (int e = 0; e < 4; ++e) v[e] = fmaxf(v[e], 0.f);
                }
                if constexpr (GEGLU) {
                    constexpr int GJ = MS == 32 ? 1 : 2;
                    const f32x4 gq = *(const f32x4*)(bw + wc + 32);
                    const f32x2 g01 = gelu2_f(f32x2{acc[j + GJ][i][g * 4] + gq[0], acc[j + GJ][i][g * 4 + 1] + gq[1]});
                    const f32x2 g23 = gelu2_f(f32x2{acc[j + GJ][i][g * 4 + 2] + gq[2], acc[j + GJ][i][g * 4 + 3] + gq[3]});
                    v[0] *= g01[0]; v[1] *= g01[1]; v[2] *= g23[0]; v[3] *= g23[1];
                }
#pragma unroll
                for (int e = 0; e < 4; ++e) v[e] *= a.scale;
                const int oc = !GEGLU ? wc : (MS == 32 ? (j >> 1) * 32 + 8 * g + lq : (j >> 2) * 32 + (j & 1) * 16 + lq);
                if (TR && tr) {
#pragma unroll
                    for (int e = 0; e < 4; ++e) *(half_t*)(cst + (oc + e) * TPITCH + prow * 2) = (half_t)v[e];
                } else if (PATH != 0 || okind == OUT_F16) {
                    h4 pk = {(half_t)v[0], (half_t)v[1], (half_t)v[2], (half_t)v[3]};
                    *(h4*)(cst + prow * PITCH + oc * 2) = pk;
                } else if (row < a.M && ocol0 + oc < nvalid) {
                    const int ch = ocol0 + oc;
                    if (okind == OUT_F32) {
                        f32x4 pk = {v[0], v[1], v[2], v[3]};
                        *(f32x4*)((float*)outp + (size_t)row * ldo + ch) = pk;
                    } else {
                        const int b = row / rps, t = row - b * rps;
#pragma unroll
                        for (int e = 0; e < 4; ++e) {
                            const size_t off = ((size_t)b * nvalid + ch + e) * ldo + t;
                            if (okind == OUT_F16_T) ((half_t*)outp)[off] = (half_t)v[e];
                            else ((float*)outp)[off] = v[e];
                        }
                    }
                }
            }
        }
      }
        if (TR && tr) {
            asm volatile("s_waitcnt lgkmcnt(0)" ::: "memory");
            const int row0 = m0 + wm * TM + ip * 32;
            const int b = row0 / rps, t0 = row0 - b * rps;
            constexpr int TT = OUT_TN * 4;
            if (row0 < a.M) {
#pragma unroll
                for (int it = 0; it < (TT + 63) / 64; ++it) {
                    const int task = lane + it * 64, c = task >> 2, q = task & 3;
                    if (task < TT && ocol0 + c < nvalid) {
                        const h8 val = *(const h8*)(cst + c * TPITCH + q * 16);
                        *(h8*)((half_t*)outp + ((size_t)b * nvalid + ocol0 + c) * ldo + t0 + q * 8) = val;
                    }
                }
            }
            asm volatile("s_waitcnt lgkmcnt(0)" ::: "memory");
        } else if (PATH != 0 || okind == OUT_F16) {
            asm volatile("s_waitcnt lgkmcnt(0)" ::: "memory");
            h8 v[WB_IT], rr[WB_IT];
            size_t goff[WB_IT];
            bool ok[WB_IT];
#pragma unroll
            for (int it = 0; it < WB_IT; ++it) {
                const int c = lane + it * 64;
                const int pr = c / CPR, ck = c - pr * CPR;
                const int grow = m0 + wm * TM + ip * 32 + pr;
                const int gcol = ocol0 + ck * 8;
                ok[it] = c < 32 * CPR && grow < a.M && gcol < nvalid;
                size_t orow = (size_t)grow;
                if (ph) {
                    const int img = grow / hwq, rem = grow - img * hwq, si = rem / a.W, sj = rem - si * a.W;
                    orow = ((size_t)img * a.Ho + (size_t)(2 * si + pa)) * a.Wo + (size_t)(2 * sj + pb);
                }
                goff[it] = orow * ldo + gcol;
                if (ok[it]) {
                    const char* sp = cst + pr * PITCH + ck * 16;
                    const h4 lo = *(const h4*)sp, hi = *(const h4*)(sp + 8);
                    v[it] = h8{lo[0], lo[1], lo[2], lo[3], hi[0], hi[1], hi[2], hi[3]};
                    if (a.resid) rr[it] = *(const h8*)(a.resid + orow * a.ld_res + gcol);
                }
            }
            bool want_stats = false;
            constexpr bool HALF = OUT_TN == 80 && WN == 2 && TM == 32 && !GEGLU;
            if constexpr (OUT_TN == 160 || HALF) want_stats = a.stats_out != nullptr;
            float* tab = (float*)cst;
            if (want_stats) asm volatile("s_waitcnt lgkmcnt(0)" ::: "memory");
#pragma unroll
            for (int it = 0; it < WB_IT; ++it) {
                if (ok[it]) {
                    if (a.resid) v[it] = v[it] + rr[it];
                    *(h8*)((half_t*)outp + goff[it]) = v[it];
                }
                if (want_stats) {
                    const int c = lane + it * 64;
                    if (c < 32 * CPR) {
                        float sm = 0.f, sq = 0.f;
                        if (ok[it]) {
#pragma unroll
                            for (int e = 0; e < 8; ++e) { const float f = (float)v[it][e]; sm += f; sq += f * f; }
                        }
                        tab[2 * c] = sm; tab[2 * c + 1] = sq;
                    }
                }
            }
            asm volatile("s_waitcnt lgkmcnt(0)" ::: "memory");
            if constexpr (HALF) {
                if (want_stats) {
                    __builtin_amdgcn_s_barrier();
                    if (wn == 0 && lane < 32) {
                        const float* tab1 = (const float*)(smem + (wave + 1) * CST_BYTES);
                        const int grow = m0 + wm * TM + ip * 32 + lane;
                        float sm = 0.f, sq = 0.f;
#pragma unroll
                        for (int k = 0; k < CPR; ++k) { sm += tab[2 * (lane * CPR + k)]; sq += tab[2 * (lane * CPR + k) + 1]; }
#pragma unroll
                        for (int k = 0; k < CPR; ++k) { sm += tab1[2 * (lane * CPR + k)]; sq += tab1[2 * (lane * CPR + k) + 1]; }
                        if (grow < a.M) {
                            float* dst = a.stats_out + ((size_t)grow * (a.N / 160) + n0 / 160) * 2;
                            dst[0] = sm; dst[1] = sq;
                        }
                    }
                    asm volatile("s_waitcnt lgkmcnt(0)" ::: "memory");
                }
            } else
            if (want_stats) {
                if (lane < 32) {
                    const int grow = m0 + wm * TM + ip * 32 + lane;
                    float sm = 0.f, sq = 0.f;
#pragma unroll
                    for (int k = 0; k < CPR; ++k) { sm += tab[2 * (lane * CPR + k)]; sq += tab[2 * (lane * CPR + k) + 1]; }
                    if (grow < a.M) {
                        float* dst = a.stats_out + ((size_t)grow * (a.N / 160) + (n0 + wn * TN) / 160) * 2;
                        dst[0] = sm; dst[1] = sq;
                    }
                }
                asm volatile("s_waitcnt lgkmcnt(0)" ::: "memory");
            }
        }
    }
    }
}

template <int BM, int BN, int WM, int WN, int STAGES, int CONV, bool GEGLU, bool SPLIT, int MS, bool LN, int PATH, int PIPE, bool ABL>
__global__ __launch_bounds__(WM * WN * 64) void igemm2_kernel(const IgemmArgs a) {
    igemm2_body<BM, BN, WM, WN, STAGES, CONV, GEGLU, SPLIT, MS, LN, PATH, PIPE, ABL>(a, (int)blockIdx.y);
}
struct IgemmArgsG { IgemmArgs g[FGDM_MAX_GROUP]; };
template <int BM, int BN, int WM, int WN, int STAGES, int CONV, bool GEGLU, bool SPLIT, int MS, bool LN, int PATH, int PIPE, bool ABL>
__global__ __launch_bounds__(WM * WN * 64) void igemm2_pair_kernel(const IgemmArgsG p) {
    igemm2_body<BM, BN, WM, WN, STAGES, CONV, GEGLU, SPLIT, MS, LN, PATH, PIPE, ABL>(p.g[blockIdx.y], 0);
}

template <bool LN>
__global__ __launch_bounds__(512) void igemm2_geglu_persist_kernel(const IgemmArgs a, int ntiles, int contiguous) {
    constexpr int BM = 256, BN = 256, WM = 4, WN = 2, NW = 8, T = 512, STAGES = 4, MS = 16;
    constexpr int TM = BM / WM, TN = BN / WN, MI = TM / MS, NI = TN / MS, AR = 4;
    typedef float acc_t __attribute__((ext_vector_type(AR)));
    constexpr int LA = BM * 4 / 64 / NW, LB = BN * 4 / 64 / NW, LPS = LA + LB;
    constexpr int STAGE_BYTES = (BM + BN) * ROWB, A_BYTES = BM * ROWB, RING_BYTES = STAGES * STAGE_BYTES;
    constexpr int OPS_FLOATS = BN + 2 * BM + BN;
    extern __shared__ __attribute__((aligned(16))) char smem[];
    auto swz_of = [](int r) { return ((r >> 3) & 1) << 1; };

    const int tid = threadIdx.x, lane = tid & 63;
    const int wave = __builtin_amdgcn_readfirstlane(tid >> 6);
    const int wm = wave / WN, wn = wave % WN;
    const int ntn = a.N / BN;
    const int nk = a.K >> 5;
    const int xcd = blockIdx.x & 7, G8 = gridDim.x >> 3, tq = ntiles >> 3, tr = ntiles & 7;
    const int x_first = xcd < tr ? xcd * (tq + 1) : tr * (tq + 1) + (xcd - tr) * tq, x_count = tq + (xcd < tr ? 1 : 0);
    const int per = (x_count + G8 - 1) / G8, jw = blockIdx.x >> 3;
    const int t_first = contiguous ? x_first + jw * per : x_first + jw;
    const int t_count = contiguous ? min(per, x_count - jw * per) : (x_count - jw + G8 - 1) / G8;
    const int t_step = contiguous ? 1 : G8;
    int local = 0;
    if (t_count <= 0) return;

    const int lrow = lane & (MS - 1), lh = lane / MS, lq = 4 * lh;
    const int koff = lrow * ROWB + ((lh ^ swz_of(lrow)) << 4);
    unsigned a_b0[LA], a_ok[LA], b_b[LB];
    int b_lds[LB];
    auto setup = [&](int m0x, int n0x) {
#pragma unroll
        for (int i = 0; i < LA; ++i) {
            const int q = (wave + i * NW) * 64 + lane, r = q >> 2, sp = q & 3, m = m0x + r;
            a_ok[i] = m < a.M ? 1u : 0u;
            a_b0[i] = a_ok[i] ? ((unsigned)m * (unsigned)a.C0 + (unsigned)((sp ^ swz_of(r)) << 3)) * 2u : 0u;
        }
#pragma unroll
        for (int i = 0; i < LB; ++i) {
            const int idx = wave + i * NW, q = idx * 64 + lane, r = q >> 2, sp = q & 3;
            b_b[i] = ((unsigned)(n0x + r) * (unsigned)a.K + (unsigned)((sp ^ swz_of(r)) << 3)) * 2u;
            b_lds[i] = A_BYTES + idx * 1024;
        }
    };
    const unsigned lds0 = __builtin_amdgcn_readfirstlane(lds_addr(smem));
    auto issue_stage = [&](int kn) {
        const char* sbase = (const char*)a.A0 + ((size_t)kn << 6);
        const char* wbase = (const char*)a.Wt + ((size_t)kn << 6);
        const unsigned lbase = lds0 + (unsigned)(kn & 3) * STAGE_BYTES;
#pragma unroll
        for (int p2 = 0; p2 < LA; ++p2) glds16_m0(a_ok[p2] ? sbase + a_b0[p2] : (const char*)a.zero, lbase + (unsigned)(wave + p2 * NW) * 1024u);
#pragma unroll
        for (int p2 = 0; p2 < LB; ++p2) glds16_sv(b_b[p2], wbase, lbase + (unsigned)b_lds[p2]);
    };
    float* const ops = (float*)(smem + RING_BYTES);
    auto stage_ops = [&](int m0x, int n0x, int set, bool same_rows) {
        float* bias_l = ops + set * OPS_FLOATS, *mr_l = bias_l + BN, *u_l = mr_l + 2 * BM;
        for (int c = tid; c < BN; c += T) bias_l[c] = a.bias ? a.bias[n0x + c] : 0.f;
        if constexpr (LN) {
            for (int c = tid; c < BN; c += T) u_l[c] = a.ln_u[n0x + c];
            if (same_rows) {
                const float* prev = ops + (set ^ 1) * OPS_FLOATS + BN;
                for (int r = tid; r < 2 * BM; r += T) mr_l[r] = prev[r];
            } else
            for (int r = tid; r < BM; r += T) {
                float mean = 0.f, rstd = 0.f;
                if (m0x + r < a.M) {
                    const float* sp = a.ln_stats + (size_t)(m0x + r) * a.ln_slots * 2;
                    float sm = 0.f, sq = 0.f;
                    for (int p2 = 0; p2 < a.ln_slots; ++p2) { sm += sp[2 * p2]; sq += sp[2 * p2 + 1]; }
                    const double mu = (double)sm / (double)a.C0;
                    double var = (double)sq / (double)a.C0 - mu * mu;
                    if (var < 0.0) var = 0.0;
                    mean = (float)mu;
                    rstd = (float)(1.0 / sqrt(var + (double)a.ln_eps));
                }
                mr_l[2 * r] = mean; mr_l[2 * r + 1] = rstd;
            }
        }
    };

    int logical = t_first;
    int m0 = (logical / ntn) * BM, n0 = (logical % ntn) * BN;
    setup(m0, n0);
#pragma unroll
    for (int sg = 0; sg < STAGES - 1; ++sg)
        if (sg < nk) issue_stage(sg);
    stage_ops(m0, n0, 0, false);
    int set = 0;
    bool first = true;
    for (;;) {
        acc_t acc[NI][MI];
#pragma unroll
        for (int j = 0; j < NI; ++j)
#pragma unroll
            for (int i = 0; i < MI; ++i)
#pragma unroll
                for (int r = 0; r < AR; ++r) acc[j][i][r] = 0.f;
        constexpr int RW = 4, WD = 3;
        auto rdX = [&](int kt, int i) { return *(const h8*)(smem + (kt & 3) * STAGE_BYTES + (wm * TM + i * MS) * ROWB + koff); };
        auto rdW = [&](int kt, int j) { return *(const h8*)(smem + (kt & 3) * STAGE_BYTES + A_BYTES + (wn * TN + j * MS) * ROWB + koff); };
        h8 xa[MI], xb[MI], wr[RW];
        {
            if (first) {
                const int younger = min(nk - 1, STAGES - 2);
                if (younger >= 2) wait_vmcnt<2 * LPS>(); else if (younger == 1) wait_vmcnt<LPS>(); else wait_vmcnt<0>();
            } else {
                if (nk > 2) wait_vmcnt<LPS>(); else wait_vmcnt<0>();
            }
            __builtin_amdgcn_s_waitcnt(0xC07F);
            __builtin_amdgcn_s_barrier();
#pragma unroll
            for (int i = 0; i < MI; ++i) xa[i] = rdX(0, i);
#pragma unroll
            for (int d = 0; d < WD; ++d) wr[d] = rdW(0, d);
        }
        auto step = [&](auto RF, int kt, h8 (&cur)[MI], h8 (&nxt)[MI]) {
            constexpr bool REFILL = decltype(RF)::value;
            if (REFILL || kt + 2 < nk) wait_vmcnt<LPS>(); else wait_vmcnt<0>();
            __builtin_amdgcn_s_waitcnt(0xC07F);
            __builtin_amdgcn_s_barrier();
            const char* sbase = (const char*)a.A0 + ((size_t)(kt + STAGES - 1) << 6);
            const char* wbase = (const char*)a.Wt + ((size_t)(kt + STAGES - 1) << 6);
            const unsigned lbase = lds0 + (unsigned)((kt + STAGES - 1) & 3) * STAGE_BYTES;
#pragma unroll
            for (int j = 0; j < NI; ++j) {
                __builtin_amdgcn_sched_barrier(0);
                if constexpr (REFILL) {
#pragma unroll
                    for (int p2 = 0; p2 < LPS; ++p2)
                        if (p2 * NI / LPS == j) {
                            if (p2 < LA) glds16_m0(a_ok[p2] ? sbase + a_b0[p2] : (const char*)a.zero, lbase + (unsigned)(wave + p2 * NW) * 1024u);
                            else glds16_sv(b_b[p2 - LA], wbase, lbase + (unsigned)b_lds[p2 - LA]);
                        }
                }
                { const int jn = j + WD; wr[jn % RW] = jn < NI ? rdW(kt, jn) : rdW(kt + 1, jn - NI); }
#pragma unroll
                for (int i = 0; i < MI; ++i)
                    if (i * NI / MI == j) nxt[i] = rdX(kt + 1, i);
#pragma unroll
                for (int i = 0; i < MI; ++i)
                    acc[j][i] = __builtin_amdgcn_mfma_f32_16x16x32_f16(wr[j % RW], cur[i], acc[j][i], 0, 0, 0);
            }
            __builtin_amdgcn_sched_barrier(0);
        };
        {
            const int nr = max(nk - (STAGES - 1), 0);
            int kt = 0;
            for (; kt + 1 < nr; kt += 2) {
                step(std::true_type{}, kt, xa, xb);
                step(std::true_type{}, kt + 1, xb, xa);
            }
            if (kt < nr) {
                step(std::true_type{}, kt, xa, xb);
                ++kt;
#pragma unroll
                for (int i = 0; i < MI; ++i) xa[i] = xb[i];
            }
            if (kt < nk) step(std::false_type{}, kt, xa, xb);
            if (kt + 1 < nk) step(std::false_type{}, kt + 1, xb, xa);
            if (kt + 2 < nk) step(std::false_type{}, kt + 2, xa, xb);
            wait_vmcnt<0>();
        }
        asm volatile("s_waitcnt lgkmcnt(0)" ::: "memory");
        __builtin_amdgcn_s_barrier();
        local += 1;
        const bool more = local < t_count;
        const int m0c = m0, n0c = n0;
        if (more) {
            logical = t_first + local * t_step;
            m0 = (logical / ntn) * BM; n0 = (logical % ntn) * BN;
            setup(m0, n0);
            if (nk > 0) issue_stage(0);
            if (nk > 1) issue_stage(1);
        }
        const float* bias_l = ops + set * OPS_FLOATS, *mr_l = bias_l + BN, *u_l = mr_l + 2 * BM;
        if constexpr (LN) {
            const float* uw = u_l + wn * TN;
#pragma unroll
            for (int j = 0; j < NI; ++j) {
                const f32x4 uq = *(const f32x4*)(uw + j * MS + lq);
#pragma unroll
                for (int i = 0; i < MI; ++i) {
                    const int trow = wm * TM + i * MS + lrow;
                    const float mean = mr_l[2 * trow], rstd = mr_l[2 * trow + 1];
#pragma unroll
                    for (int e = 0; e < 4; ++e) acc[j][i][e] = ln_scale(acc[j][i][e], mean, rstd, uq[e]);
                }
            }
        }
        constexpr int OUT_TN = TN / 2, PITCH = OUT_TN * 2 + 8, CPR = OUT_TN / 8, WB_IT = (32 * CPR + 63) / 64, CST_BYTES = 32 * PITCH;
        static_assert(NW * CST_BYTES <= 2 * STAGE_BYTES, "epilogue staging must fit ring slots 2 and 3");
        char* cst = smem + 2 * STAGE_BYTES + wave * CST_BYTES;
        const int ocol0 = (n0c + wn * TN) >> 1, nvalid = a.N / 2;
        const float* bw = bias_l + wn * TN;
#pragma unroll
        for (int ip = 0; ip < TM / 32; ++ip) {
#pragma unroll
            for (int hf = 0; hf < 2; ++hf) {
                const int i = ip * 2 + hf;
                const int prow = hf * MS + lrow;
#pragma unroll
                for (int j = 0; j < NI; ++j) {
                    if (j & 2) continue;
                    const int wc = j * MS + lq;
                    const f32x4 bq = *(const f32x4*)(bw + wc);
                    float v[4];
#pragma unroll
                    for (int e = 0; e < 4; ++e) v[e] = acc[j][i][e] + bq[e];
                    const f32x4 gq = *(const f32x4*)(bw + wc + 32);
                    const f32x2 g01 = gelu2_f(f32x2{acc[j + 2][i][0] + gq[0], acc[j + 2][i][1] + gq[1]});
                    const f32x2 g23 = gelu2_f(f32x2{acc[j + 2][i][2] + gq[2], acc[j + 2][i][3] + gq[3]});
                    v[0] *= g01[0]; v[1] *= g01[1]; v[2] *= g23[0]; v[3] *= g23[1];
#pragma unroll
                    for (int e = 0; e < 4; ++e) v[e] *= a.scale;
                    const int oc = (j >> 2) * 32 + (j & 1) * 16 + lq;
                    const h4 pk = {(half_t)v[0], (half_t)v[1], (half_t)v[2], (half_t)v[3]};
                    *(h4*)(cst + prow * PITCH + oc * 2) = pk;
                }
            }
            asm volatile("s_waitcnt lgkmcnt(0)" ::: "memory");
#pragma unroll
            for (int it = 0; it < WB_IT; ++it) {
                const int c = lane + it * 64, pr = c / CPR, ck = c - pr * CPR;
                const int grow = m0c + wm * TM + ip * 32 + pr, gcol = ocol0 + ck * 8;
                if (c < 32 * CPR && grow < a.M && gcol < nvalid) {
                    const char* sp = cst + pr * PITCH + ck * 16;
                    const h4 lo = *(const h4*)sp, hi = *(const h4*)(sp + 8);
                    *(h8*)((half_t*)a.out + (size_t)grow * a.ld_out + gcol) = h8{lo[0], lo[1], lo[2], lo[3], hi[0], hi[1], hi[2], hi[3]};
                }
            }
            asm volatile("s_waitcnt lgkmcnt(0)" ::: "memory");
        }
        if (!more) break;
        set ^= 1;
        stage_ops(m0, n0, set, m0 == m0c);
        asm volatile("s_waitcnt lgkmcnt(0)" ::: "memory");
        __builtin_amdgcn_s_barrier();
        if (nk > 2) issue_stage(2);
        first = false;
    }
}

template <bool LN>
int launch_geglu_persist(const IgemmArgs& a, int ntiles, int contiguous, hipStream_t s) {
    constexpr int smem = 4 * (256 + 256) * ROWB + 2 * (256 + 2 * 256 + 256) * 4;
    static_assert(smem <= 160 * 1024, "LDS budget");
    constexpr auto k = igemm2_geglu_persist_kernel<LN>;
    if (fgdm_dyn_lds<k>(smem) != FGDM_OK) return FGDM_ERR_HIP;
    FGDM_LAUNCH(k, dim3(256), dim3(512), smem, s, a, ntiles, contiguous);
    return hipGetLastError() == hipSuccess ? FGDM_OK : FGDM_ERR_HIP;
}

template <int BM, int BN, int WM, int WN, int STAGES, int CONV, bool GEGLU, bool SPLIT, int MS, bool LN, int PATH, int PIPE, bool ABL>
int launch2p(const IgemmArgs& a, hipStream_t s) {
    constexpr int ring = ring_bytes<BM, BN, STAGES, PIPE>();
    constexpr int smem = ring + (1 + RV_MAX) * BN * 4 + (2 * BM + BN) * 4;
    static_assert(smem <= 160 * 1024, "LDS budget");
    constexpr auto k = igemm2_kernel<BM, BN, WM, WN, STAGES, CONV, GEGLU, SPLIT, MS, LN, PATH, PIPE, ABL>;
    if (fgdm_dyn_lds<k>(smem) != FGDM_OK) return FGDM_ERR_HIP;
    const int ntm = (a.M + BM - 1) / BM, ntn = (a.N + BN - 1) / BN;
    const unsigned gx = (unsigned)(ntm * ntn * (SPLIT ? a.splitk : 1));
    constexpr bool phases = CONV == 2;
    const unsigned gy = phases ? 4u : 1u;
    if (fgdm_recording()) {
        auto single = [=](hipStream_t rs) -> int {
            hipLaunchKernelGGL(k, dim3(gx, gy), dim3(WM * WN * 64), smem, rs, a);
            return hipGetLastError() == hipSuccess ? FGDM_OK : FGDM_ERR_HIP;
        };
        if (phases) { fgdm_record(single); return FGDM_OK; }
        if constexpr (PIPE != 0 && PATH != 0 && !SPLIT && !ABL && MS == 16) {
            constexpr auto kp = igemm2_pair_kernel<BM, BN, WM, WN, STAGES, CONV, GEGLU, SPLIT, MS, LN, PATH, PIPE, ABL>;
            if (fgdm_dyn_lds<kp>(smem) != FGDM_OK) return FGDM_ERR_HIP;
            static_assert(sizeof(IgemmArgs) <= FGDM_GROUP_BLOB, "the recorded blob holds an IgemmArgs");
            FgdmGroupFn pf = [](const void* const* av, int n, unsigned grid_x, hipStream_t rs) -> int {
                if (n < 2 || n > FGDM_MAX_GROUP) return FGDM_ERR_ARG;
                IgemmArgsG pg;
                for (int i = 0; i < FGDM_MAX_GROUP; ++i) pg.g[i] = *(const IgemmArgs*)av[i < n ? i : 0];
                hipLaunchKernelGGL((igemm2_pair_kernel<BM, BN, WM, WN, STAGES, CONV, GEGLU, SPLIT, MS, LN, PATH, PIPE, ABL>), dim3(grid_x, n),
                                   dim3(WM * WN * 64), smem, rs, pg);
                return hipGetLastError() == hipSuccess ? FGDM_OK : FGDM_ERR_HIP;
            };
            fgdm_record(single, (const void*)kp, pf, &a, sizeof(a), gx, 0);
        } else {
            fgdm_record(single);
        }
        return FGDM_OK;
    }
    hipLaunchKernelGGL(k, dim3(gx, gy), dim3(WM * WN * 64), smem, s, a);
    return hipGetLastError() == hipSuccess ? FGDM_OK : FGDM_ERR_HIP;
}
template <int BM, bool GEGLU, bool LN>
int epilogue_path(const IgemmArgs& a) {
    if (a.out_kind != OUT_F16 || !(a.act == ACT_NONE || GEGLU)) return 0;
    if (a.out2 && a.out_kind2 != OUT_F16) {
        const bool staged = LN && a.out_kind2 == OUT_F16_T && a.rows_per_sample % 32 == 0 && a.M % 32 == 0 && a.ld_out2 % 8 == 0 &&
                            ((size_t)a.out2 & 15) == 0;
        if (!staged || a.rowvec) return 0;
    }
    if (!a.rowvec) return 1;
    return (BM - 1) / a.rows_per_sample + 2 <= RV_MAX ? 2 : 0;
}
template <int BM, int BN, int WM, int WN, int STAGES, int CONV, bool GEGLU, bool SPLIT, int MS, bool LN, bool FAST, int PIPE>
int launch2(const IgemmArgs& a, hipStream_t s) {
    const bool fast_on = knob_once(KNOB_IGEMM_EPI_PATHS) != 0;
    if constexpr (FAST && !SPLIT && !LN) {
        if (a.debug)
            return epilogue_path<BM, GEGLU, LN>(a) == 1 ? launch2p<BM, BN, WM, WN, STAGES, CONV, GEGLU, SPLIT, MS, LN, 1, (PIPE == 2 ? 1 : PIPE), true>(a, s)
                                                        : FGDM_ERR_ARG;
    }
    if (a.debug) return FGDM_ERR_ARG;
    if constexpr (SPLIT) return launch2p<BM, BN, WM, WN, STAGES, CONV, GEGLU, SPLIT, MS, LN, 0, PIPE, false>(a, s);
    if constexpr (FAST && !SPLIT) {
        switch (fast_on ? epilogue_path<BM, GEGLU, LN>(a) : 0) {
            case 1: return launch2p<BM, BN, WM, WN, STAGES, CONV, GEGLU, SPLIT, MS, LN, 1, PIPE, false>(a, s);
            case 2: if constexpr (!GEGLU && !LN && CONV != 2) return launch2p<BM, BN, WM, WN, STAGES, CONV, GEGLU, SPLIT, MS, LN, 2, PIPE, false>(a, s);
            default: break;
        }
    }
    if constexpr (CONV == 2 && BM == 256 && BN == 320 && MS == 16) return launch2p<128, BN, WM, WN, STAGES, CONV, GEGLU, SPLIT, MS, LN, 0, 0, false>(a, s);
    else return launch2p<BM, BN, WM, WN, STAGES, CONV, GEGLU, SPLIT, MS, LN, 0, 0, false>(a, s);
}
template <int BM, int BN, bool GEGLU, int MS, int PIPE, int WM, int WN>
int launch2m(const IgemmArgs& a, hipStream_t s) {
    constexpr int PL = PIPE == 2 ? 1 : PIPE;
    if (a.mode == IG_CONV2_PHASE) {
        if constexpr (!GEGLU) return launch2<BM, BN, WM, WN, 4, 2, false, false, MS, false, MS == 16, PL>(a, s);
        else return FGDM_ERR_ARG;
    }
    return a.mode == IG_LINEAR ? launch2<BM, BN, WM, WN, 4, 0, GEGLU, false, MS, false, MS == 16, PL>(a, s)
                               : launch2<BM, BN, WM, WN, 4, 1, GEGLU, false, MS, false, MS == 16, (GEGLU ? PL : PIPE)>(a, s);
}
template <int BM, int BN, bool GEGLU, int MS, int PIPE, int WM, int WN>
int launch2ln(const IgemmArgs& a, hipStream_t s) {
    return launch2<BM, BN, WM, WN, 4, false, GEGLU, false, MS, true, MS == 16, (PIPE == 2 ? 1 : PIPE)>(a, s);
}
template <int BM, int BN, int MS, int PIPE, int WM = 4, int WN = 2>
int launch_tile(const IgemmArgs& a, hipStream_t s) {
    const bool g = a.act == ACT_GEGLU;
    if (a.ln_stats) {
        if constexpr (BN == 256) { if (g) return launch2ln<BM, BN, true, MS, PIPE, WM, WN>(a, s); }
        if constexpr (BN == 128) return FGDM_ERR_ARG;
        else return launch2ln<BM, BN, false, MS, PIPE, WM, WN>(a, s);
    }
    if constexpr (BN == 256) { if (g) return launch2m<BM, BN, true, MS, PIPE, WM, WN>(a, s); }
    return launch2m<BM, BN, false, MS, PIPE, WM, WN>(a, s);
}

__global__ __launch_bounds__(256) void splitk_reduce_kernel(const IgemmArgs a) {
    const size_t total4 = (size_t)a.M * a.N / 4, plane = (size_t)a.M * a.N;
    for (size_t i = (size_t)blockIdx.x * 256 + threadIdx.x; i < total4; i += (size_t)gridDim.x * 256) {
        const size_t e0 = i * 4;
        const int row = (int)(e0 / a.N), col = (int)(e0 - (size_t)row * a.N);
        f32x4 v = *(const f32x4*)(a.ws + e0);
        for (int s = 1; s < a.splitk; ++s) {
            const f32x4 u = *(const f32x4*)(a.ws + (size_t)s * plane + e0);
            v[0] += u[0]; v[1] += u[1]; v[2] += u[2]; v[3] += u[3];
        }
        h4 r = {(half_t)0, (half_t)0, (half_t)0, (half_t)0};
        if (a.resid) r = *(const h4*)(a.resid + (size_t)row * a.ld_res + col);
        h4 o;
#pragma unroll
        for (int e = 0; e < 4; ++e) {
            float x = v[e] + (a.bias ? a.bias[col + e] : 0.f);
            if (a.rowvec) x += a.rowvec[(size_t)(row / a.rows_per_sample) * a.rv_stride + col + e];
            if (a.act == ACT_SILU) x = silu_f(x);
            else if (a.act == ACT_RELU) x = fmaxf(x, 0.f);
            else if (a.act == ACT_QGELU) x = silu_f(x, 1.702f);
            const half_t y = (half_t)(x * a.scale);
            o[e] = a.resid ? (half_t)((float)y + (float)r[e]) : y;
        }
        *(h4*)((half_t*)a.out + (size_t)row * a.ld_out + col) = o;
    }
}

}

static thread_local bool g_twin_layers = false;
void igemm_set_twin_layers(bool on) { g_twin_layers = on; }

int igemm_splitk_factor(const IgemmArgs& a) {
    if (a.force_cfg || a.act == ACT_GEGLU || a.out_kind != OUT_F16 || a.N % 320 || (a.K & 31)) return 1;
    if (a.mode == IG_CONV2_PHASE) return 1;
    const int nk = a.K >> 5;
    const bool fat = knob_once(KNOB_SPLITK_FAT) != 0;
    if (fat && a.rows_per_sample > 64 && a.rows_per_sample <= 256 && (nk >= 540 || (nk >= 360 && !g_twin_layers))) return 2;
    if (a.rows_per_sample > 64 || nk < 96) return 1;
    return (fat && nk >= 360) ? 8 : 4;
}
int igemm_splitk_reduce(const IgemmArgs& a, hipStream_t s) {
    const size_t total4 = (size_t)a.M * a.N / 4;
    const int grid = (int)std::min<size_t>(2048, (total4 + 255) / 256);
    FGDM_LAUNCH(splitk_reduce_kernel, dim3(grid), dim3(256), 0, s, a);
    return hipGetLastError() == hipSuccess ? FGDM_OK : FGDM_ERR_HIP;
}

static bool halo_geometry(const IgemmArgs& a) {
    if (a.mode != IG_CONV3 || a.Ho != a.H || a.Wo != a.W || (a.C0 & 63) || (a.C1 & 63) || (a.K % 288) || a.debug) return false;
    if ((a.W == 16 || a.W == 32 || a.W == 64) && (a.H * a.W) % 256 == 0) return true;
    return a.W == 8 && a.H == 8;
}

int igemm2_launch(const IgemmArgs& a, int cfg, hipStream_t s) {
    if ((a.K & 31) || (a.C0 & 31) || (a.C1 & 31)) return FGDM_ERR_ARG;
    const int pipe_default = knob_once(KNOB_IGEMM_PIPE);
    const int tile = cfg & 15, psel = cfg >> 4;
    const size_t px = a.mode == IG_LINEAR ? (size_t)a.M : (size_t)a.B * a.H * a.W;
    const bool small = px * (size_t)std::max(a.C0, a.C1) * 2 < (1ull << 32) && (size_t)(a.N + 320) * a.K * 2 < (1ull << 32);
    const bool pipe = (psel == 0 ? pipe_default != 0 : psel == 2) && small;
    if (a.mode == IG_CONV2_PHASE && (a.splitk > 1 || a.C1 || a.out_kind != OUT_F16 || a.stats_out || a.out2 || a.ln_stats || a.act == ACT_GEGLU ||
                                     a.Ho != 2 * a.H || a.Wo != 2 * a.W || a.K != 4 * a.C0 || a.M != a.B * a.H * a.W || !small))
        return FGDM_ERR_ARG;
    const bool halo = knob_once(KNOB_IGEMM_HALO) != 0 && pipe && halo_geometry(a);
    const int bn = (tile == 1 || tile == 4) ? 256 : tile == 6 ? 128 : tile == 7 ? 160 : 320;
    if (a.N % bn) return FGDM_ERR_ARG;
    if (a.act == ACT_GEGLU && bn != 256) return FGDM_ERR_ARG;
    if (a.splitk > 1) {
        if ((tile != 2 && tile != 0) || a.ln_stats) return FGDM_ERR_ARG;
        const int nk_all = a.K >> 5;
        if (halo && nk_all % a.splitk == 0 && (nk_all / a.splitk) % 9 == 0)
            return tile == 0 ? launch2<256, 320, 4, 2, 4, true, false, true, 16, false, false, 2>(a, s)
                             : launch2<128, 320, 4, 2, 4, true, false, true, 16, false, false, 2>(a, s);
        if (tile == 0 && pipe)
            return a.mode == IG_LINEAR ? launch2<256, 320, 4, 2, 4, false, false, true, 16, false, false, 1>(a, s)
                                       : launch2<256, 320, 4, 2, 4, true, false, true, 16, false, false, 1>(a, s);
        if (pipe)
            return a.mode == IG_LINEAR ? launch2<128, 320, 4, 2, 4, false, false, true, 16, false, false, 1>(a, s)
                                       : launch2<128, 320, 4, 2, 4, true, false, true, 16, false, false, 1>(a, s);
        return a.mode == IG_LINEAR ? launch2<128, 320, 4, 2, 4, false, false, true, 16, false, false, 0>(a, s)
                                   : launch2<128, 320, 4, 2, 4, true, false, true, 16, false, false, 0>(a, s);
    }
    if (a.ln_stats && a.mode != IG_LINEAR) return FGDM_ERR_ARG;
    const int persist_mode = knob_once(KNOB_IGEMM_PERSIST);
    const bool persist_on = persist_mode != 0;
    if (persist_on && tile == 1 && pipe && a.act == ACT_GEGLU && a.mode == IG_LINEAR && !a.C1 && a.out_kind == OUT_F16 && !a.rowvec &&
        !a.resid && !a.out2 && !a.stats_out && !a.debug && a.N % 256 == 0) {
        const int ntiles = ((a.M + 255) / 256) * (a.N / 256);
        if (ntiles > 256) return a.ln_stats ? launch_geglu_persist<true>(a, ntiles, persist_mode == 2, s) : launch_geglu_persist<false>(a, ntiles, persist_mode == 2, s);
    }
    switch (tile) {
        case 0: return halo ? launch_tile<256, 320, 16, 2>(a, s) : pipe ? launch_tile<256, 320, 16, 1>(a, s) : launch_tile<256, 320, 16, 0>(a, s);
        case 1: return pipe ? launch_tile<256, 256, 16, 1>(a, s) : launch_tile<256, 256, 16, 0>(a, s);
        case 2: return halo ? launch_tile<128, 320, 16, 2>(a, s) : pipe ? launch_tile<128, 320, 16, 1>(a, s) : launch_tile<128, 320, 16, 0>(a, s);
        case 3: return launch_tile<256, 320, 32, 0>(a, s);
        case 4: return launch_tile<256, 256, 32, 0>(a, s);
        case 5: return launch_tile<128, 320, 32, 0>(a, s);
        case 6: return pipe ? launch_tile<256, 128, 16, 1>(a, s) : launch_tile<256, 128, 16, 0>(a, s);
        case 7: return a.mode != IG_LINEAR ? FGDM_ERR_ARG : pipe ? launch_tile<64, 160, 16, 1, 2, 2>(a, s) : launch_tile<64, 160, 16, 0, 2, 2>(a, s);
        default: return FGDM_ERR_ARG;
    }
}
```

fgdm_amd/csrc/knobs.h:

```cpp
#pragma once
#include "common.h"
#include <array>
#include <cstdlib>

#define FGDM_STR_(x) #x
#define FGDM_STR(x) FGDM_STR_(x)

#define FGDM_KNOBS(X)                                                                                                          \
    X(ATTN_PP, "FGDM_ATTN_PP", "1", "0: the four-wave attention kernel where the eight-wave ping-pong one would run")           \
    X(ATTN_DQ, "FGDM_ATTN_DQ", "3", "long self-attention, d = 40: 3 = two-strand kernel, 32-wide V^T P^T; 1 = 16-wide; 0 = off") \
    X(ATTN_DQ80, "FGDM_ATTN_DQ80", "1", "0: the ping-pong kernel instead of the two-strand one at d = 64 / 80")                 \
    X(ATTN_ABL, "FGDM_ATTN_ABL", "0", "ablation instantiations of the two-strand kernel (tools/bench_attention.py only)")       \
    X(ATTN_CROSS, "FGDM_ATTN_CROSS", "4", "query chunks per wave of the text-token kernel (65 - 96 keys); 0 = off")             \
    X(ATTN_CROSS_LONG, "FGDM_ATTN_CROSS_LONG", "8", "query chunks per wave of the key-resident kernel (97 - 256 keys); 0 = off") \
    X(IGEMM_EPI_PATHS, "FGDM_IGEMM_EPI_PATHS", "1", "0: the general GEMM epilogue instead of the host-selected straight-line paths") \
    X(IGEMM_HALO, "FGDM_IGEMM_HALO", "1", "0: per-tap K loop instead of the halo-tile loop (stride-1 3x3 convolutions, split K too)") \
    X(IGEMM_MFMA32, "FGDM_IGEMM_MFMA32", "0", "1: automatic tile choices take the 32x32x16 MFMA instantiations")                \
    X(IGEMM_OTHER_WIDTHS, "FGDM_IGEMM_OTHER_WIDTHS", "1", "0: widths 128 / 256 / 512 back on the 2-stage kernel")               \
    X(IGEMM_PERSIST, "FGDM_IGEMM_PERSIST", "1", "GEGLU projections: 1 = persistent, tiles round-robin; 2 = contiguous runs; 0 = off") \
    X(IGEMM_PIPE, "FGDM_IGEMM_PIPE", "1", "0: the phase-locked K loop instead of the software-pipelined one")                   \
    X(IGEMM_UP_PHASE, "FGDM_IGEMM_UP_PHASE", "1", "0: Upsample convs as the 3x3 walk over the virtual upsampled image, not four 2x2 phase GEMMs") \
    X(IGEMM_SMALL_M, "FGDM_IGEMM_SMALL_M", "1", "0: linears with a thin 128-row grid stay on 128 x 320 tiles")                  \
    X(IGEMM_SMALL_TILES, "FGDM_IGEMM_SMALL_TILES", "1", "0: the 8x8 level's linears back on the 2-stage kernel")                \
    X(IGEMM_STATS64, "FGDM_IGEMM_STATS64", "1", "0: the 64 x 160 tile leaves the LayerNorm partial sums to the row-statistics pass") \
    X(SPLITK_FAT, "FGDM_SPLITK_FAT", "1", "0: split K four ways on 128 x 320 tiles at the 8x8 level only")                      \
    X(PAIR_FAT_TILES, "FGDM_PAIR_FAT_TILES", "1", "0: grouped launches keep the tile a single problem would take")              \
    X(GN_REG, "FGDM_GN_REG", "1024", "largest pixel count per sample of the register-resident GroupNorm; 0 = off")              \
    X(GN_REG_NG, "FGDM_GN_REG_NG", "4", "widest slice of the register-resident GroupNorm, in groups")                           \
    X(GN_FUSED_MAXKB, "FGDM_GN_FUSED_MAXKB", "64", "largest LDS slice (KB) of the single-kernel GroupNorm; 0 = always two kernels") \
    X(GN_CHUNK, "FGDM_GN_CHUNK", FGDM_STR(GN_PIX_PER_CHUNK), "pixels per partial-sum chunk of the two-kernel GroupNorm (multiples of 64)") \
    X(LN_FOLD, "FGDM_LN_FOLD", "1", "fgdm_create; 0: the transformer blocks' LayerNorms as kernels of their own")               \
    X(TWIN_STREAMS, "FGDM_TWIN_STREAMS", "0", "fgdm_create; 1: the ControlNets on a second stream next to the UNet encoder")    \
    X(PAIR_LAUNCH, "FGDM_PAIR_LAUNCH", "1", "fgdm_create; 0: no grouped launches of twin layers")                               \
    X(GROUP_MAX, "FGDM_GROUP_MAX", FGDM_STR(FGDM_MAX_GROUP), "fgdm_create; problems per grouped launch, clamped to [2, FGDM_MAX_GROUP]") \
    X(GN_GROUP, "FGDM_GN_GROUP", "1", "fgdm_create; 0: single-pass GroupNorm launches stay out of the grouped launches")        \
    X(PAIR_DEBUG, "FGDM_PAIR_DEBUG", nullptr, "set (to anything): fgdm_destroy prints how many replayed launches were fused")   \
    X(PROF_DUMP, "FGDM_PROF_DUMP", nullptr, "path: fgdm_profile_end writes the per-shape time table there")                     \
    X(BENCH_DATA_SCALE, "FGDM_BENCH_DATA_SCALE", "1", "atof; scale of the random operands of fgdm_bench_igemm / _attention")

enum Knob {
#define X(id, name, dflt, meaning) KNOB_##id,
    FGDM_KNOBS(X)
#undef X
    KNOB_COUNT
};
struct KnobDef { const char* name; const char* dflt; const char* meaning; };
inline constexpr KnobDef KNOB_TABLE[KNOB_COUNT] = {
#define X(id, name, dflt, meaning) {name, dflt, meaning},
    FGDM_KNOBS(X)
#undef X
};

inline const char* knob_text(Knob k) {
    const char* v = getenv(KNOB_TABLE[k].name);
    return v ? v : KNOB_TABLE[k].dflt;
}
inline int knob_int(Knob k) { return atoi(knob_text(k)); }
inline bool knob_on(Knob k) { return knob_int(k) != 0; }
inline int knob_once(Knob k) {
    static const std::array<int, KNOB_COUNT> v = [] {
        std::array<int, KNOB_COUNT> a{};
        for (int i = 0; i < KNOB_COUNT; ++i)
            if (KNOB_TABLE[i].dflt) a[i] = knob_int((Knob)i);
        return a;
    }();
    return v[k];
}
```

fgdm_amd/csrc/ops_abi.hip:

```cpp
#include "engine_shared.h"
#include "replay_plan.h"

static int op_pack(IgemmArgs& a, TmpDev& tmp, const float* w, const float* bias, int N, int K, int Ks, bool geglu,
                   const int* kmap = nullptr, const float* gamma = nullptr, const float* beta = nullptr) {
    auto host = [](const float* d, size_t n, std::vector<float>& v) { v.resize(n); return hipMemcpy(v.data(), d, n * sizeof(float), hipMemcpyDefault) == hipSuccess; };
    std::vector<float> wh, bh(N, 0.f), g, bt;
    if (!host(w, (size_t)N * Ks, wh) || (bias && !host(bias, N, bh))) return FGDM_ERR_HIP;
    if (gamma && (!host(gamma, K, g) || !host(beta, K, bt))) return FGDM_ERR_HIP;
    const size_t npad = igemm_npad(N);
    std::vector<half_t> pk(npad * (size_t)K, (half_t)0);
    std::vector<float> bp(npad, 0.f), u(gamma ? npad : 0, 0.f);
    for (int pr = 0; pr < N; ++pr) {
        int sr = pr;
        if (geglu) { const int grp = pr >> 6, within = pr & 63; sr = within < 32 ? grp * 32 + within : N / 2 + grp * 32 + (within - 32); }
        const float* row = &wh[(size_t)sr * Ks];
        double us = 0.0, cs = 0.0;
        for (int k = 0; k < K; ++k) {
            const int ks = kmap ? kmap[k] : k;
            if (ks < 0) continue;
            const half_t wq = (half_t)(gamma ? row[ks] * g[k] : row[ks]);
            pk[(size_t)pr * K + k] = wq;
            if (gamma) { us += (double)(float)wq; cs += (double)bt[k] * (double)row[ks]; }
        }
        bp[pr] = gamma ? (float)((double)bh[sr] + cs) : bh[sr];
        if (gamma) u[pr] = (float)us;
    }
    a.Wt = tmp.up(pk); a.bias = tmp.up(bp);
    if (gamma) a.ln_u = tmp.up(u);
    return a.Wt && a.bias && (!gamma || a.ln_u) ? FGDM_OK : FGDM_ERR_NOMEM;
}

static int op_gemm_rows(IgemmArgs& a, const half_t* A, int B, int Ho, int Wo, int K, int rps, TmpDev& tmp, hipStream_t s) {
    a.A0 = A; a.C0 = K; a.A1 = nullptr; a.C1 = 0;
    a.zero = g_zero_page();
    if (!a.zero) return FGDM_ERR_NOMEM;
    a.B = B; a.H = Ho; a.W = Wo; a.Ho = Ho; a.Wo = Wo;
    a.M = B * Ho * Wo; a.K = K; a.mode = IG_LINEAR; a.rows_per_sample = rps;
    if (plan_splitk(a, tmp) != FGDM_OK) return FGDM_ERR_NOMEM;
    return igemm_launch(a, s);
}

static int op_conv3_im2col(const half_t* x, int Cin, const float* w, const float* bias, const float* rowvec, const half_t* resid,
                           int B, int H, int W, int Cout, int stride, int act, float scale, void* out, hipStream_t s) {
    int cp = 0;
    const std::vector<int> kmap = conv3_kmap(Cin, &cp);
    const int K = (int)kmap.size(), Ho = (H - 1) / stride + 1, Wo = (W - 1) / stride + 1;
    TmpDev tmp;
    IgemmArgs a{};
    const int prc = op_pack(a, tmp, w, bias, Cout, K, Cin * 9, false, kmap.data());
    if (prc != FGDM_OK) return prc;
    half_t* A = tmp.alloc<half_t>((size_t)B * Ho * Wo * K);
    if (!A) return FGDM_ERR_NOMEM;
    a.rowvec = rowvec; a.rv_stride = Cout;
    a.resid = resid; a.ld_res = Cout;
    a.N = Cout; a.act = act; a.out_kind = OUT_F16; a.out = out; a.ld_out = Cout; a.scale = scale;
    const int rc = im2col_conv(x, A, B, H, W, cp, stride, K, s, []() {},
        [&](half_t* Ap, int Bv, int Hv, int Wv, int Kv, int rps) { return op_gemm_rows(a, Ap, Bv, Hv, Wv, Kv, rps, tmp, s); });
    (void)hipStreamSynchronize(s);
    return rc;
}

extern "C" {

int fgdm_op_conv2d(const void* x0, int C0, const void* x1, int C1, const float* w, const float* bias, const float* rowvec,
                   const void* resid, int B, int H, int W, int Cout, int ksize, int stride, int upsample, int act,
                   float scale, void* out, void* stream) {
    if (!x0 || !w || !out || (ksize != 1 && ksize != 3)) return FGDM_ERR_ARG;
    if (stride == FGDM_STRIDE2_PAD_BR && (ksize != 3 || upsample)) return FGDM_ERR_ARG;
    hipStream_t s = as_stream(stream);
    const int Cin = C0 + C1, taps = ksize * ksize, K = taps * Cin;
    if (B <= 0 || H <= 0 || W <= 0 || Cout <= 0 || C0 <= 0 || C1 < 0) return FGDM_ERR_ARG;
    if (Cin & 63) {
        if (ksize != 3 || C1 || x1 || upsample || (stride != 1 && stride != 2)) return FGDM_ERR_ARG;
        return op_conv3_im2col((const half_t*)x0, C0, w, bias, rowvec, (const half_t*)resid, B, H, W, Cout, stride, act, scale, out, s);
    }
    std::vector<int> kmap(K);
    for (int tap = 0; tap < taps; ++tap)
        for (int c = 0; c < Cin; ++c) kmap[taps == 9 ? ((c >> 6) * 9 + tap) * 64 + (c & 63) : c] = c * taps + tap;
    TmpDev tmp;
    IgemmArgs a{};
    const int prc = op_pack(a, tmp, w, bias, Cout, K, K, false, kmap.data());
    if (prc != FGDM_OK) return prc;
    a.A0 = (const half_t*)x0; a.C0 = C0; a.A1 = (const half_t*)x1; a.C1 = C1;
    a.zero = g_zero_page();
    if (!a.zero) return FGDM_ERR_NOMEM;
    a.rowvec = rowvec; a.rv_stride = Cout;
    a.resid = (const half_t*)resid; a.ld_res = Cout;
    a.B = B; a.H = H; a.W = W;
    a.Ho = H; a.Wo = W; a.mode = IG_LINEAR;
    if (ksize == 3) {
        a.mode = IG_CONV3;
        if (upsample) { a.Ho = 2 * H; a.Wo = 2 * W; a.mode = IG_CONV3_UP2; }
        else if (stride == 2) { a.Ho = (H - 1) / 2 + 1; a.Wo = (W - 1) / 2 + 1; a.mode = IG_CONV3_S2; }
        else if (stride == FGDM_STRIDE2_PAD_BR) {
            if (H < 2 || W < 2) return FGDM_ERR_ARG;
            a.Ho = (H - 2) / 2 + 1; a.Wo = (W - 2) / 2 + 1; a.mode = IG_CONV3_S2_BR;
        }
    }
    a.M = B * a.Ho * a.Wo; a.N = Cout; a.K = K;
    a.act = act; a.out_kind = OUT_F16; a.out = out; a.ld_out = Cout;
    a.rows_per_sample = a.Ho * a.Wo; a.scale = scale;
    if (igemm_up_phase(a)) {
        std::vector<float> wh((size_t)Cout * K);
        if (hipMemcpy(wh.data(), w, wh.size() * sizeof(float), hipMemcpyDefault) != hipSuccess) return FGDM_ERR_HIP;
        const half_t* wph = tmp.up(up_phase_pack(wh.data(), Cout, Cin, igemm_npad(Cout)));
        if (!wph) return FGDM_ERR_NOMEM;
        a = igemm_phase_args(a, wph);
    }
    if (plan_splitk(a, tmp) != FGDM_OK) return FGDM_ERR_NOMEM;
    const int rc = igemm_launch(a, s);
    (void)hipStreamSynchronize(s);
    return rc;
}

int fgdm_op_linear(const void* x, const float* w, const float* bias, const void* resid, int M, int K, int N, int act,
                   int out_kind, int rows_per_sample, int ld_out, void* out, void* stream) {
    if (!x || !w || !out || (K & 63)) return FGDM_ERR_ARG;
    hipStream_t s = as_stream(stream);
    TmpDev tmp;
    IgemmArgs a{};
    const int prc = op_pack(a, tmp, w, bias, N, K, K, act == ACT_GEGLU);
    if (prc != FGDM_OK) return prc;
    a.A0 = (const half_t*)x; a.C0 = K;
    a.zero = g_zero_page();
    if (!a.zero) return FGDM_ERR_NOMEM;
    const int nout = act == ACT_GEGLU ? N / 2 : N;
    a.resid = (const half_t*)resid; a.ld_res = nout;
    a.B = 1; a.H = 1; a.W = M; a.Ho = 1; a.Wo = M;
    a.M = M; a.N = N; a.K = K; a.mode = IG_LINEAR; a.act = act; a.out_kind = out_kind;
    a.out = out; a.ld_out = ld_out ? ld_out : nout;
    a.rows_per_sample = rows_per_sample ? rows_per_sample : M; a.scale = 1.f;
    const int rc = igemm_launch(a, s);
    (void)hipStreamSynchronize(s);
    return rc;
}

int fgdm_op_linear_ln_linear(const void* x, const float* w1, const float* b1, const void* resid, const float* gamma,
                             const float* beta, const float* w2, const float* b2, int M, int K1, int C, int N2, int act2,
                             void* h_out, void* y_out, int* slots_used, void* stream) {
    if (!x || !w1 || !gamma || !beta || !w2 || !h_out || !y_out || (K1 & 63) || (C & 63)) return FGDM_ERR_ARG;
    hipStream_t s = as_stream(stream);
    TmpDev tmp;
    IgemmArgs a{}, b{};
    int rc = op_pack(a, tmp, w1, b1, C, K1, K1, false);
    if (rc == FGDM_OK) rc = op_pack(b, tmp, w2, b2, N2, C, C, act2 == ACT_GEGLU, nullptr, gamma, beta);
    if (rc != FGDM_OK) return rc;
    a.A0 = (const half_t*)x; a.C0 = K1; a.zero = g_zero_page();
    a.resid = (const half_t*)resid; a.ld_res = C;
    a.B = 1; a.H = 1; a.W = M; a.Ho = 1; a.Wo = M; a.M = M; a.N = C; a.K = K1; a.mode = IG_LINEAR; a.act = ACT_NONE;
    a.out_kind = OUT_F16; a.out = h_out; a.ld_out = C; a.rows_per_sample = M; a.scale = 1.f;
    if (!a.zero) return FGDM_ERR_NOMEM;
    int slots = igemm_stats_slots(a);
    float* stats = tmp.alloc<float>((size_t)M * std::max(slots, row_stats_slots(C)) * 2);
    if (!stats) return FGDM_ERR_NOMEM;
// ... 20 lines not shown
    if ((long long)B * T > 0x7fffffffLL / (3 * C)) return FGDM_ERR_ARG;
    hipStream_t s = as_stream(stream);
    const int M = B * T, N = 3 * C;
    const size_t cc = (size_t)C * C;
    std::vector<float> w(3 * cc);
    const float* src[3] = {wq, wk, wv};
    for (int i = 0; i < 3; ++i)
        if (hipMemcpy(&w[i * cc], src[i], cc * sizeof(float), hipMemcpyDefault) != hipSuccess) return FGDM_ERR_HIP;
    TmpDev tmp;
    IgemmArgs a{};
    int rc = op_pack(a, tmp, w.data(), nullptr, N, C, C, false, nullptr, fold ? gamma : nullptr, fold ? beta : nullptr);
    if (rc != FGDM_OK) return rc;
    a.A0 = (const half_t*)h; a.C0 = C; a.zero = g_zero_page();
    if (!a.zero) return FGDM_ERR_NOMEM;
    a.B = B; a.H = 1; a.W = T; a.Ho = 1; a.Wo = T; a.M = M; a.N = N; a.K = C; a.mode = IG_LINEAR; a.act = ACT_NONE;
    a.out_kind = OUT_F16; a.out = qk; a.ld_out = 2 * C; a.rows_per_sample = T; a.scale = 1.f;
    a.out2 = vt; a.out_kind2 = OUT_F16_T; a.ld_out2 = Tp; a.split_n = 2 * C;
    if (fold) {
        const int slots = row_stats_slots(C);
        float* stats = tmp.alloc<float>((size_t)M * slots * 2);
        if (!stats) return FGDM_ERR_NOMEM;
        rc = row_stats_launch((const half_t*)h, M, C, stats, s);
        if (rc != FGDM_OK) { (void)hipStreamSynchronize(s); return rc; }
        a.ln_stats = stats; a.ln_slots = slots; a.ln_eps = 1e-5f;
    }
    rc = igemm_launch(a, s);
    (void)hipStreamSynchronize(s);
    return rc;
}

int fgdm_debug_force_igemm_cfg(int cfg) { igemm_set_force_cfg(cfg); return FGDM_OK; }

int fgdm_op_groupnorm(const void* x0, int C0, const void* x1, int C1, int B, int HW, const float* gamma, const float* beta,
                      float eps, int silu, void* out, void* stream) {
    if (!x0 || !gamma || !beta || !out) return FGDM_ERR_ARG;
    hipStream_t s = as_stream(stream);
    float* ws = nullptr;
    if (hipMalloc(&ws, groupnorm_ws_floats(B, HW) * sizeof(float)) != hipSuccess) return FGDM_ERR_NOMEM;
    const int rc = groupnorm_launch((const half_t*)x0, C0, (const half_t*)x1, C1, B, HW, gamma, beta, eps, silu, (half_t*)out, ws, s);
    (void)hipStreamSynchronize(s);
    (void)hipFree(ws);
    return rc;
}
int fgdm_op_layernorm(const void* x, int rows, int C, const float* gamma, const float* beta, float eps, void* out, void* stream) {
    if (!x || !gamma || !beta || !out) return FGDM_ERR_ARG;
    return layernorm_launch((const half_t*)x, rows, C, gamma, beta, eps, (half_t*)out, as_stream(stream));
}
int fgdm_op_attention(const void* q, int ldq, const void* k, int ldk, const void* vt, int ldvt, void* o, int ldo, int B,
                      int heads, int T, int Tk, int d, void* stream) {
    if (!q || !k || !vt || !o) return FGDM_ERR_ARG;
    return attention_launch((const half_t*)q, ldq, (const half_t*)k, ldk, (const half_t*)vt, ldvt, (half_t*)o, ldo, B, heads, T, Tk, d, 0, as_stream(stream));
}
int fgdm_op_attention_ex(const void* q, int ldq, const void* k, int ldk, const void* vt, int ldvt, void* o, int ldo, int B,
                         int heads, int T, int Tk, int d, int q_prescaled, void* stream) {
    if (!q || !k || !vt || !o) return FGDM_ERR_ARG;
    return attention_launch((const half_t*)q, ldq, (const half_t*)k, ldk, (const half_t*)vt, ldvt, (half_t*)o, ldo, B, heads, T, Tk, d,
                            q_prescaled ? 1 : 0, as_stream(stream));
}
int fgdm_debug_last_attention_kernel(void) { return attention_last_kernel(); }
int fgdm_op_small_attention(const void* qkv, int ld, int koff, int voff, void* out, int ldo, int B, int heads, int T, int d,
                            int causal, void* stream) {
    if (!qkv || !out) return FGDM_ERR_ARG;
    return small_attention_launch((const half_t*)qkv, ld, koff, voff, (half_t*)out, ldo, B, heads, T, d, causal, as_stream(stream));
}

int fgdm_op_vae_attention(const void* q, const void* k, const void* vt, void* out, int B, int T, int C, void* stream) {
    if (!q || !k || !vt || !out || B <= 0 || T <= 0 || C <= 0 || (T & 63) || (C & 63)) return FGDM_ERR_ARG;
    hipStream_t s = as_stream(stream);
    TmpDev tmp;
    float* S = tmp.alloc<float>((size_t)T * T);
    half_t* P = tmp.alloc<half_t>((size_t)T * T);
    if (!S || !P) return FGDM_ERR_NOMEM;
    bool softmax_failed = false;
    const int rc = vattn_core((const half_t*)q, (const half_t*)k, (const half_t*)vt, (half_t*)out, S, P, B, T, C, s, &softmax_failed,
        [&](const half_t* Wt, int N, int K, const half_t* A, int M, int out_kind, void* o, int ld_out, float scale) {
            IgemmArgs a{};
            a.Wt = Wt; a.N = N; a.act = ACT_NONE; a.out_kind = out_kind; a.out = o; a.ld_out = ld_out; a.scale = scale;
            return op_gemm_rows(a, A, 1, 1, M, K, M, tmp, s);
        });
    (void)hipStreamSynchronize(s);
    return rc;
}
int fgdm_op_softmax_rows(const float* S, void* P, int rows, int cols, void* stream) {
    if (!S || !P || rows <= 0 || cols <= 0) return FGDM_ERR_ARG;
    return softmax_rows(S, (half_t*)P, rows, cols, as_stream(stream));
}
int fgdm_op_nchw_to_nhwc(const float* x, void* y, int B, int C, int HW, int Cpad, void* stream) {
    if (!x || !y || B <= 0 || C <= 0 || HW <= 0 || Cpad < C) return FGDM_ERR_ARG;
    return nchw_f32_to_nhwc_f16(x, (half_t*)y, B, C, HW, Cpad, as_stream(stream));
}
int fgdm_op_pack_xcat(const float* x, const void* cc16, int B, int Bc, int Cc, int H, int W, int cin_pad, void* out, void* stream) {
    if (!x || !cc16 || !out || H <= 0 || W <= 0) return FGDM_ERR_ARG;
    return pack_xcat(x, (const half_t*)cc16, (half_t*)out, B, Bc, Cc, H * W, cin_pad, as_stream(stream));
}
int fgdm_op_nhwc_to_nchw(const void* x, float* y, int B, int C, int HW, void* stream) {
    if (!x || !y || B <= 0 || C <= 0 || HW <= 0) return FGDM_ERR_ARG;
    return nhwc_f16_to_nchw_f32((const half_t*)x, y, B, C, HW, as_stream(stream));
}
int fgdm_op_avgpool2(const void* x, void* y, int B, int H, int W, int C, void* stream) {
    if (!x || !y || B <= 0 || H <= 0 || W <= 0 || C <= 0 || (C & 7) || (H & 1) || (W & 1)) return FGDM_ERR_ARG;
    return avgpool2((const half_t*)x, (half_t*)y, B, H, W, C, as_stream(stream));
}
int fgdm_op_transpose_pad(const void* v, void* vt, int B, int Tk, int C, int Tkpad, void* stream) {
    if (!v || !vt || B <= 0 || Tk <= 0 || C <= 0 || Tkpad < Tk) return FGDM_ERR_ARG;
    return transpose_pad_keys((const half_t*)v, (half_t*)vt, B, Tk, C, Tkpad, as_stream(stream));
}
int fgdm_op_timestep_embed(const int64_t* t, const float* t_float, void* y, int B, int dim, int rows_pad, void* stream) {
    if ((!t && !t_float) || !y || B <= 0 || dim < 2 || (dim & 1) || rows_pad < B) return FGDM_ERR_ARG;
    return timestep_embed(t, t_float, (half_t*)y, B, dim, rows_pad, as_stream(stream));
}
int fgdm_op_add_f16(const void* a, const void* b, void* y, int64_t n, void* stream) {
    if (!a || !b || !y || n <= 0 || (n & 7)) return FGDM_ERR_ARG;
    return add_f16((const half_t*)a, (const half_t*)b, (half_t*)y, (size_t)n, as_stream(stream));
}

int fgdm_op_ddim_loop_step(const float* x, const float* e_cond, const float* e_uncond, float cfg_scale, float a_t, float a_prev,
                           float sigma_t, float sqrt_one_minus_at, const float* noise, const float* mask, const float* x0,
                           const float* q_noise, float sqrt_ac_next, float sqrt_one_minus_ac_next, float* x_out, float* xin_a,
                           float* xin_b, float* log_x, float* log_pred_x0, int64_t n, void* stream) {
    if (!x || n <= 0 || (e_uncond && !e_cond) || (mask && (!x0 || !q_noise))) return FGDM_ERR_ARG;
    DdimLoopStep a{};
    a.x = x; a.ec = e_cond; a.eu = e_uncond; a.noise = noise; a.mask = mask; a.x0 = x0; a.qnoise = q_noise;
    a.x_out = x_out; a.xin_a = xin_a; a.xin_b = xin_b; a.log_x = log_x; a.log_p0 = log_pred_x0;
    a.cfg = cfg_scale; a.a_t = a_t; a.a_prev = a_prev; a.sigma = sigma_t; a.s1m = sqrt_one_minus_at;
    a.sa_next = sqrt_ac_next; a.s1m_next = sqrt_one_minus_ac_next; a.n = (size_t)n;
    return ddim_loop_step(a, as_stream(stream));
}

int fgdm_op_plms_loop_step(const float* x, const float* e_cond, const float* e_uncond, float cfg_scale, int mode, int order,
                           const float* e1, const float* e2, const float* e3, float* e_out, float a_t, float a_prev,
                           float sqrt_one_minus_at, const float* mask, const float* x0, const float* q_noise, float sqrt_ac_next,
                           float sqrt_one_minus_ac_next, float* x_out, float* xin_a, float* xin_b, float* log_x, float* log_pred_x0,
                           int64_t n, void* stream) {
    if (n <= 0) return FGDM_ERR_ARG;
    PlmsLoopStep a{};
    a.x = x; a.ec = e_cond; a.eu = e_uncond; a.e1 = e1; a.e2 = e2; a.e3 = e3; a.mask = mask; a.x0 = x0; a.qnoise = q_noise;
    a.e_out = e_out; a.x_out = x_out; a.xin_a = xin_a; a.xin_b = xin_b; a.log_x = log_x; a.log_p0 = log_pred_x0;
    a.cfg = cfg_scale; a.a_t = a_t; a.a_prev = a_prev; a.s1m = sqrt_one_minus_at; a.sa_next = sqrt_ac_next;
    a.s1m_next = sqrt_one_minus_ac_next; a.mode = mode; a.order = order; a.n = (size_t)n;
    return plms_loop_step(a, as_stream(stream));
}

int fgdm_op_dpmpp_loop_step(const float* x, const float* e_cond, const float* e_uncond, float cfg_scale, float inv_alpha,
                            float neg_sigma_over_alpha, const float* m1, int update_kind, float c1, float cm0, float cm1,
                            float* m0_out, float* x_out, float* xin_a, float* xin_b, int64_t n, void* stream) {
    if (n <= 0) return FGDM_ERR_ARG;
    DpmppLoopStep a{};
    a.x = x; a.ec = e_cond; a.eu = e_uncond; a.m1 = m1; a.m0_out = m0_out; a.x_out = x_out; a.xin_a = xin_a; a.xin_b = xin_b;
    a.cfg = cfg_scale; a.inv_alpha = inv_alpha; a.neg_sigma_over_alpha = neg_sigma_over_alpha; a.c1 = c1; a.cm0 = cm0; a.cm1 = cm1;
    a.kind = update_kind; a.n = (size_t)n;
    return dpmpp_loop_step(a, as_stream(stream));
}

int fgdm_replay_plan(int n_walks, const int32_t* lens, const uint64_t* key, const uint32_t* grid_x, const uint64_t* shape, int group_max,
                     int chunk, int32_t* out, int out_cap, int* limits) {
    if (limits) { limits[0] = REPLAY_LOOK; limits[1] = FGDM_MAX_GROUP; }
    if (n_walks < 0 || group_max < 1 || out_cap < 0 || (n_walks && !lens) || (out_cap && !out)) return FGDM_ERR_ARG;
    std::vector<PlanWalk> walks(n_walks);
    size_t u = 0;
    for (int w = 0; w < n_walks; ++w) {
        if (lens[w] < 0 || (lens[w] && (!key || !grid_x || !shape))) return FGDM_ERR_ARG;
        for (int i = 0; i < lens[w]; ++i, ++u) walks[w].push_back(PlanUnit{key[u], grid_x[u], shape[u]});
    }
    std::vector<int32_t> steps;
    replay_plan_chunked(walks.data(), n_walks, chunk, group_max, REPLAY_LOOK, steps);
    for (size_t i = 0; i < steps.size() && i < (size_t)out_cap; ++i) out[i] = steps[i];
    return (int)steps.size();
}

}
```

include/fgdm.h:

```cpp
#ifndef FGDM_H
#define FGDM_H
#include <stdint.h>
#ifdef __cplusplus
extern "C" {
#endif

#define FGDM_MAX_LEVELS 8
#define FGDM_MAX_CONTROLNETS 4

typedef struct fgdm_engine fgdm_engine;

typedef struct fgdm_config {
    int32_t in_channels, out_channels, model_channels, num_res_blocks;
    int32_t n_levels;
    int32_t channel_mult[FGDM_MAX_LEVELS];
    int32_t n_attention_resolutions;
    int32_t attention_resolutions[FGDM_MAX_LEVELS];
    int32_t num_heads, context_dim;
    int32_t use_adapter;
    int32_t n_controlnets;
    int32_t hint_channels;
    int64_t workspace_bytes;
    int32_t vae_ch, vae_n_levels;
    int32_t vae_ch_mult[FGDM_MAX_LEVELS];
// ... 27 lines not shown
int fgdm_set_hint(fgdm_engine* e, int cn, const float* hint, int B, int Hh, int Wh, void* stream);

int fgdm_set_adapter_conds(fgdm_engine* e, const float* const* conds, int n_conds, int B, int H, int W, void* stream);

int fgdm_set_context(fgdm_engine* e, const float* ctx, int B, void* stream);
int fgdm_set_context_tokens(fgdm_engine* e, int tokens);
int fgdm_get_context_tokens(const fgdm_engine* e);
int fgdm_set_concat(fgdm_engine* e, const float* c_concat, int B, int Cc, int H, int W, void* stream);
int fgdm_apply_model(fgdm_engine* e, const float* x, const int64_t* t, const float* t_float, const float* ctx,
                     const float* pcond, const float* control_scales, int B, int H, int W, int flags, float* eps_out,
                     void* stream);

int fgdm_clip_encode(fgdm_engine* e, const int64_t* ids, int B, int T, float* out, void* stream);
int fgdm_clip_encode_skip(fgdm_engine* e, const int64_t* ids, int B, int T, int clip_skip, float* out, void* stream);

int fgdm_vae_decode(fgdm_engine* e, const float* z, int B, int H, int W, float scale, float* image, void* stream);
int fgdm_vae_encode(fgdm_engine* e, const float* image, int B, int H, int W, float* moments, void* stream);
int fgdm_posterior_sample(const float* moments, const float* noise , float scale, float* z,
                          int B, int zc, int HW, void* stream);

int fgdm_unfold(const float* x, int B, int C, int H, int W, int kh, int kw, int sh, int sw, int l0, int n, float* crops,
                void* stream);
int fgdm_fold_weighted(const float* crops, const float* w_pix, const float* w_tie, int B, int C, int Ho, int Wo, int kh, int kw,
                       int sh, int sw, int crops_per_pass, float* out, void* stream);
int fgdm_vae_decode_patches(fgdm_engine* e, const float* z, int B, int H, int W, float scale, int kh, int kw, int sh, int sw,
                            int f, const float* w_pix, const float* w_tie, int max_crops_per_pass, float* image, void* stream);
int fgdm_apply_model_patches(fgdm_engine* e, const float* x, const int64_t* t, const float* t_float, const float* ctx, int B,
                             int H, int W, int kh, int kw, int sh, int sw, const float* w_pix, const float* w_tie,
                             int max_crops_per_pass, int flags, float* eps_out, void* stream);

int fgdm_image_to_uint8(const float* image, int B, int C, int H, int W, int mode, uint8_t* out, void* stream);
int fgdm_resize_linear_uint8(const uint8_t* src, int B, int H, int W, int C, int Ho, int Wo, uint8_t* dst, void* stream);
int fgdm_uint8_to_hint(const uint8_t* src, int B, int H, int W, int C, float* hint, void* stream);

int fgdm_controlnet(fgdm_engine* e, int cn, const float* x, const int64_t* t, const float* ctx, int B, int H, int W,
                    float* out, int64_t out_capacity_floats, void* stream);

int fgdm_run_block(fgdm_engine* e, const char* prefix, const float* x, int C, const float* x_skip, int Cs, const float* emb,
                   const float* ctx, int B, int H, int W, float* out, int64_t out_capacity_floats, int64_t* out_numel,
                   void* stream);

int fgdm_ddim_step(const float* x, const float* e_cond, const float* e_uncond, float cfg_scale, float a_t,
                   float a_prev, float sigma_t, float sqrt_one_minus_at, const float* noise, float* x_prev,
                   float* pred_x0, float* e_out, int64_t n, void* stream);
int fgdm_plms_combine(const float* e_t, const float* e1, const float* e2, const float* e3, int order,
                      float* e_prime, int64_t n, void* stream);
int fgdm_axpby(const float* a, float ca, const float* b, float cb, float* y, int64_t n, void* stream);
int fgdm_mask_blend(const float* a, const float* b, const float* mask, float* y, int64_t n, void* stream);
int fgdm_ancestral_step(const float* x, const float* eps, float sqrt_recip_ac, float sqrt_recipm1_ac, float coef1,
                        float coef2, float std, const float* noise, float* out, int64_t n, void* stream);

int fgdm_sample_ddim(fgdm_engine* e, float* x, const float* cond, const float* uncond, float cfg_scale, int S,
                     const int64_t* timesteps, const float* alphas, const float* alphas_prev,
                     const float* sqrt_one_minus_alphas, const float* control_scales, int B, int H, int W,
                     int flags, void* stream);

#define FGDM_DDIM_PARAMS_SIZE_V1 192
typedef struct fgdm_ddim_params {
    int64_t struct_size;
    float* x;
    const float* cond;
    const float* uncond;
    const int64_t* timesteps;
    const float* alphas;
    const float* alphas_prev;
    const float* sqrt_one_minus_alphas;
    const float* control_scales;
    const float* sigmas;
    const float* cfg_scales;
    const float* step_noise;
    const float* mask;
    const float* x0;
    const float* q_noise;
    const float* sqrt_alphas_cumprod_t;
    const float* sqrt_one_minus_alphas_cumprod_t;
    const int32_t* log_steps;
    float* x_inter_out;
    float* pred_x0_out;
    float cfg_scale;
    int32_t S;
    int32_t B;
    int32_t H;
    int32_t W;
    int32_t flags;
    int32_t n_log;
    int32_t reserved0;
} fgdm_ddim_params;
int fgdm_sample_ddim_ex(fgdm_engine* e, const fgdm_ddim_params* p, void* stream);

#define FGDM_PLMS_PARAMS_SIZE_V1 168
typedef struct fgdm_plms_params {
    int64_t struct_size;
    float* x;
    const float* cond;
    const float* uncond;
    const int64_t* timesteps;
    const float* alphas;
    const float* alphas_prev;
    const float* sqrt_one_minus_alphas;
    const float* control_scales;
    const float* mask;
    const float* x0;
    const float* q_noise;
    const float* sqrt_alphas_cumprod_t;
    const float* sqrt_one_minus_alphas_cumprod_t;
    const int32_t* log_steps;
    float* x_inter_out;
    float* pred_x0_out;
    float cfg_scale;
    int32_t S;
    int32_t B;
    int32_t H;
    int32_t W;
    int32_t flags;
    int32_t n_log;
    int32_t reserved0;
} fgdm_plms_params;
int fgdm_sample_plms(fgdm_engine* e, const fgdm_plms_params* p, void* stream);

#define FGDM_DPMPP_FIRST 1
#define FGDM_DPMPP_SECOND 2
#define FGDM_DPMPP_PARAMS_SIZE_V1 128
typedef struct fgdm_dpmpp_params {
    int64_t struct_size;
    float* x;
    const float* cond;
    const float* uncond;
    const float* control_scales;
    const float* t_float;
    const float* inv_alpha;
    const float* neg_sigma_over_alpha;
    const int32_t* update_kind;
    const float* c1;
    const float* cm0;
    const float* cm1;
    float cfg_scale;
    int32_t n_eval;
    int32_t B;
    int32_t H;
    int32_t W;
    int32_t flags;
    int32_t reserved0;
    int32_t reserved1;
} fgdm_dpmpp_params;
int fgdm_sample_dpmpp(fgdm_engine* e, const fgdm_dpmpp_params* p, void* stream);

int fgdm_profile_begin(fgdm_engine* e, int stride );
int fgdm_profile_end(fgdm_engine* e, double* out);
int fgdm_workspace_stats(fgdm_engine* e, int64_t* peak_bytes, int64_t* reserved_bytes);
int fgdm_launch_stats(fgdm_engine* e, int64_t* replayed_launches, int64_t* fused_launches, int64_t* fused_problems);
int fgdm_replay_plan(int n_walks, const int32_t* lens, const uint64_t* key, const uint32_t* grid_x, const uint64_t* shape,
                     int group_max, int chunk, int32_t* out, int out_cap, int* limits);

#define FGDM_STRIDE2_PAD_BR (-2)
int fgdm_op_conv2d(const void* x0, int C0, const void* x1, int C1, const float* w, const float* bias,
                   const float* rowvec, const void* resid, int B, int H, int W, int Cout, int ksize, int stride,
                   int upsample, int act, float scale, void* out, void* stream);
int fgdm_op_linear(const void* x, const float* w, const float* bias, const void* resid, int M, int K, int N,
                   int act, int out_kind, int rows_per_sample, int ld_out, void* out, void* stream);
int fgdm_op_linear_ln_linear(const void* x, const float* w1, const float* b1, const void* resid, const float* gamma,
                             const float* beta, const float* w2, const float* b2, int M, int K1, int C, int N2, int act2,
                             void* h_out, void* y_out, int* slots_used, void* stream);
int fgdm_debug_force_igemm_cfg(int cfg);
int fgdm_bench_igemm(int B, int H, int W, int C0, int C1, int Cout, int ksize, int stride, int upsample, int act,
                     int use_resid, int cfg, int iters, float* avg_ms);
int fgdm_bench_ff(int M, int C, int chunk_rows, int iters, float* avg_ms);
int fgdm_bench_attention(int B, int heads, int T, int Tk, int d, int iters, float* avg_ms);
int fgdm_bench_norm(int kind, int B, int HW, int C0, int C1, int silu, int iters, float* avg_ms);
int fgdm_op_groupnorm(const void* x0, int C0, const void* x1, int C1, int B, int HW, const float* gamma,
                      const float* beta, float eps, int silu, void* out, void* stream);
int fgdm_op_layernorm(const void* x, int rows, int C, const float* gamma, const float* beta, float eps,
                      void* out, void* stream);
int fgdm_op_attention(const void* q, int ldq, const void* k, int ldk, const void* vt, int ldvt, void* o, int ldo,
                      int B, int heads, int T, int Tk, int d, void* stream);
int fgdm_op_attention_ex(const void* q, int ldq, const void* k, int ldk, const void* vt, int ldvt, void* o, int ldo,
                         int B, int heads, int T, int Tk, int d, int q_prescaled, void* stream);
int fgdm_debug_last_attention_kernel(void);
int fgdm_op_small_attention(const void* qkv, int ld, int koff, int voff, void* out, int ldo, int B, int heads, int T, int d,
                            int causal, void* stream);

int fgdm_op_vae_attention(const void* q, const void* k, const void* vt, void* out, int B, int T, int C, void* stream);
int fgdm_op_softmax_rows(const float* S, void* P, int rows, int cols, void* stream);
int fgdm_op_nchw_to_nhwc(const float* x, void* y, int B, int C, int HW, int Cpad, void* stream);
int fgdm_op_nhwc_to_nchw(const void* x, float* y, int B, int C, int HW, void* stream);
int fgdm_op_pack_xcat(const float* x, const void* cc16, int B, int Bc, int Cc, int H, int W, int cin_pad, void* out, void* stream);
int fgdm_op_avgpool2(const void* x, void* y, int B, int H, int W, int C, void* stream);
int fgdm_op_transpose_pad(const void* v, void* vt, int B, int Tk, int C, int Tkpad, void* stream);
int fgdm_op_timestep_embed(const int64_t* t, const float* t_float, void* y, int B, int dim, int rows_pad, void* stream);
int fgdm_op_add_f16(const void* a, const void* b, void* y, int64_t n, void* stream);

int fgdm_op_ddim_loop_step(const float* x, const float* e_cond, const float* e_uncond, float cfg_scale, float a_t, float a_prev,
                           float sigma_t, float sqrt_one_minus_at, const float* noise, const float* mask, const float* x0,
                           const float* q_noise, float sqrt_ac_next, float sqrt_one_minus_ac_next, float* x_out, float* xin_a,
                           float* xin_b, float* log_x, float* log_pred_x0, int64_t n, void* stream);

int fgdm_op_plms_loop_step(const float* x, const float* e_cond, const float* e_uncond, float cfg_scale, int mode, int order,
                           const float* e1, const float* e2, const float* e3, float* e_out, float a_t, float a_prev,
                           float sqrt_one_minus_at, const float* mask, const float* x0, const float* q_noise, float sqrt_ac_next,
                           float sqrt_one_minus_ac_next, float* x_out, float* xin_a, float* xin_b, float* log_x, float* log_pred_x0,
                           int64_t n, void* stream);
int fgdm_op_dpmpp_loop_step(const float* x, const float* e_cond, const float* e_uncond, float cfg_scale, float inv_alpha,
                            float neg_sigma_over_alpha, const float* m1, int update_kind, float c1, float cm0, float cm1,
                            float* m0_out, float* x_out, float* xin_a, float* xin_b, int64_t n, void* stream);

int fgdm_op_ln_qkv(const void* h, const float* gamma, const float* beta, const float* wq, const float* wk, const float* wv,
                   int B, int T, int C, int Tp, int fold, void* qk, void* vt, void* stream);

#ifdef __cplusplus
}
#endif
#endif
```

Measured before the change: 8.187.

## Fold ResBlock 1x1 skip projection into second conv's GEMM as prologue

When a ResBlock changes channel count, its 1x1 skip projection previously ran as its own GEMM launch whose output was then read back as a residual by the second 3x3 conv. This change runs the skip GEMM as a prologue inside the conv's igemm2 kernel, accumulating into the same registers and summing both biases. That removes a launch plus a full write and read of the skip tensor. It only applies to a narrow set of shapes (halo pipeline, N multiple of 320, no split-K) and adds a new template variant with larger LDS use, which may lower occupancy.

```diff
diff --git a/fgdm_amd/_lib.py b/fgdm_amd/_lib.py
--- a/fgdm_amd/_lib.py
+++ b/fgdm_amd/_lib.py
@@ -115,6 +115,8 @@
     'fgdm_workspace_stats': (_i, [_p, C.POINTER(_i64), C.POINTER(_i64)]),
     'fgdm_launch_stats': (_i, [_p, C.POINTER(_i64), C.POINTER(_i64), C.POINTER(_i64)]),
     'fgdm_replay_plan': (_i, [_i, _p, _p, _p, _p, _i, _i, _p, _i, _p]),
+    'fgdm_skip_fold_rule': (_i, [_i] * 17),
+    'fgdm_op_conv2d_skip': (_i, [_p, _i, _p, _p, _p, _i, _p, _i, _p, _p, _i, _i, _i, _i, _p, _p, _p]),
     'fgdm_op_conv2d': (_i, [_p, _i, _p, _i, _p, _p, _p, _p, _i, _i, _i, _i, _i, _i, _i, _i, _f, _p, _p]),
     'fgdm_op_linear': (_i, [_p, _p, _p, _p, _i, _i, _i, _i, _i, _i, _i, _p, _p]),
     'fgdm_debug_force_igemm_cfg': (_i, [_i]),
diff --git a/fgdm_amd/csrc/common.h b/fgdm_amd/csrc/common.h
--- a/fgdm_amd/csrc/common.h
+++ b/fgdm_amd/csrc/common.h
@@ -87,9 +87,16 @@
     float* stats_out;
     void* out2;
     int split_n, out_kind2, ld_out2;
+    const half_t* pA0;
+    const half_t* pA1;
+    const half_t* pWt;
+    const float* bias2;
+    int pC0, pC1, pK;
 };
 
 int igemm_launch(const IgemmArgs& a, hipStream_t s);
+bool igemm_skip_fold(const IgemmArgs& a);
+bool igemm2_prologue_ok(const IgemmArgs& a, int cfg);
 bool igemm_up_phase(const IgemmArgs& a);
 IgemmArgs igemm_phase_args(const IgemmArgs& a, const half_t* wt_phase);
 void igemm_set_force_cfg(int cfg);
diff --git a/fgdm_amd/csrc/engine.hip b/fgdm_amd/csrc/engine.hip
--- a/fgdm_amd/csrc/engine.hip
+++ b/fgdm_amd/csrc/engine.hip
@@ -350,6 +350,7 @@
         int ld_out = 0;
         void* out2 = nullptr; int out_kind2 = OUT_F16, ld_out2 = 0, split_n = 0;
         int rps = 0;
+        const GemmW* skip_w = nullptr; const Tensor* skip_x = nullptr; const Tensor* skip_x1 = nullptr;
     };
     int gemm(const GemmW& w, int mode, const Tensor& x0, const Tensor* x1, int Ho, int Wo, const Epi& e, Tensor* out) {
         IgemmArgs a{};
@@ -375,12 +376,28 @@
         if (!a.out) return fail(FGDM_ERR_NOMEM, "gemm: null output (workspace exhausted?)");
         if (w.wph && !e.stats && !e.ln && igemm_up_phase(a)) a = igemm_phase_args(a, w.wph);
         char tag[56] = "";
-        if (prof.on) snprintf(tag, sizeof(tag), "igemm M%d N%d K%d mode%d act%d out%d l%ds%dr%dv%d", a.M, a.N, a.K, a.mode, a.act, a.out_kind,
-                              e.ln ? 1 : 0, e.stats ? 1 : 0, e.resid ? 1 : 0, e.rowvec ? 1 : 0);
         a.splitk = igemm_splitk_factor(a);
         if (a.splitk > 1) {
             a.ws = (float*)ar->alloc((size_t)a.splitk * a.M * a.N * sizeof(float));
             if (!a.ws) return fail(FGDM_ERR_NOMEM, "workspace (split-K partials)");
+        }
+        Tensor sk;
+        const GemmW* pro = nullptr;
+        if (e.skip_w) {
+            const GemmW& pw = *e.skip_w;
+            const Tensor& px = *e.skip_x;
+            if (e.resid || pw.N != w.N || px.rows() != a.M || pw.K != px.C + (e.skip_x1 ? e.skip_x1->C : 0))
+                return fail(FGDM_ERR_ARG, "gemm: skip projection does not match the problem");
+            a.pA0 = px.p; a.pC0 = px.C;
+            a.pA1 = e.skip_x1 ? e.skip_x1->p : nullptr; a.pC1 = e.skip_x1 ? e.skip_x1->C : 0;
+            a.pWt = pw.w; a.bias2 = pw.bias; a.pK = pw.K;
+            if (igemm_skip_fold(a)) {
+                pro = &pw;
+            } else {
+                a.pA0 = a.pA1 = a.pWt = nullptr; a.bias2 = nullptr; a.pC0 = a.pC1 = a.pK = 0;
+                CHK(linear(pw, px, Epi{}, &sk, e.skip_x1));
+                a.resid = sk.p; a.ld_res = sk.C;
+            }
         }
         if (e.ln) {
             if (!w.ln_u || !e.ln->p || a.splitk > 1) return fail(FGDM_ERR_STATE, "gemm: LayerNorm fold without folded weights / statistics");
@@ -388,6 +405,11 @@
         } else if (w.ln_u) {
             return fail(FGDM_ERR_STATE, "gemm: these weights have a LayerNorm folded in; statistics are required");
         }
+        if (prof.on) {
+            const int n = snprintf(tag, sizeof(tag), "igemm M%d N%d K%d mode%d act%d out%d l%ds%dr%dv%d", a.M, a.N, a.K, a.mode, a.act, a.out_kind,
+                                   e.ln ? 1 : 0, e.stats ? 1 : 0, a.resid ? 1 : 0, e.rowvec ? 1 : 0);
+            if (pro && n > 0 && n < (int)sizeof(tag)) snprintf(tag + n, sizeof(tag) - n, "+pK%d", a.pK);
+        }
         if (e.stats) {
             e.stats->slots = igemm_stats_slots(a);
             e.stats->p = (float*)ar->alloc((size_t)a.M * std::max(e.stats->slots, row_stats_slots(nout)) * 2 * sizeof(float));
@@ -398,12 +420,16 @@
         if (prof.on) {
             const double in_b = 2.0 * ((double)x0.numel() + (x1 ? (double)x1->numel() : 0.0));
             const double out_b = (double)a.M * nout * (e.out_kind == OUT_F16 || e.out_kind == OUT_F16_T ? 2.0 : 4.0);
-            nbytes = in_b + 2.0 * (double)w.N * w.K + out_b + (e.resid ? 2.0 * (double)a.M * nout : 0.0);
-        }
-        prof.begin(PC_IGEMM, s, 2.0 * (double)x0.B * Ho * Wo * (double)w.N * (double)w.k_real, tag, nbytes);
+            nbytes = in_b + 2.0 * (double)w.N * w.K + out_b + (a.resid ? 2.0 * (double)a.M * nout : 0.0);
+            if (pro) nbytes += 2.0 * ((double)e.skip_x->numel() + (e.skip_x1 ? (double)e.skip_x1->numel() : 0.0)) + 2.0 * (double)pro->N * pro->K;
+        }
+        double flops = 2.0 * (double)x0.B * Ho * Wo * (double)w.N * (double)w.k_real;
+        if (pro) flops += 2.0 * (double)a.M * (double)pro->N * (double)pro->k_real;
+        prof.begin(PC_IGEMM, s, flops, tag, nbytes);
         int rc = igemm_launch(a, s);
         prof.end(s);
         if (a.ws) ar->release(a.ws);
+        if (sk.p) tfree(sk);
         if (rc == FGDM_OK && e.stats && e.stats->slots == 0) {
             if (a.out_kind != OUT_F16 || a.ld_out != nout) return fail(FGDM_ERR_ARG, "gemm: row statistics need a dense fp16 output");
             e.stats->slots = row_stats_slots(nout);
@@ -490,7 +516,9 @@
         CHK(gnorm(l.gn2, h, nullptr, l.eps, true, &g2));
         tfree(h);
         Epi e2;
-        if (l.cin != l.cout) {
+        if (l.cin != l.cout && !l.down && knob_once(KNOB_IGEMM_SKIP_FOLD) != 0) {
+            e2.skip_w = &l.skip; e2.skip_x = xs; e2.skip_x1 = x1;
+        } else if (l.cin != l.cout) {
             CHK(linear(l.skip, *xs, Epi{}, &sk, x1));
             e2.resid = sk.p; e2.ld_res = sk.C;
         } else {
diff --git a/fgdm_amd/csrc/igemm.hip b/fgdm_amd/csrc/igemm.hip
--- a/fgdm_amd/csrc/igemm.hip
+++ b/fgdm_amd/csrc/igemm.hip
@@ -344,7 +344,15 @@
     return p;
 }
 
+bool igemm_skip_fold(const IgemmArgs& a) {
+    if (!knob_once(KNOB_IGEMM_SKIP_FOLD) || a.pK <= 0 || a.splitk > 1 || a.mode != IG_CONV3) return false;
+    if (knob_once(KNOB_IGEMM_MFMA32) && !a.force_cfg && !g_force_cfg) return false;
+    const int force = pick_force(a);
+    return force >= 4 && igemm2_prologue_ok(a, force - 4);
+}
+
 int igemm_launch(const IgemmArgs& a, hipStream_t s) {
+    if (a.pK && !igemm_skip_fold(a)) return FGDM_ERR_ARG;
     if (a.M <= 0 || a.N <= 0 || a.K <= 0 || (a.K & 63) || (a.C0 & 63) || (a.C1 & 63)) return FGDM_ERR_ARG;
     if (a.act == ACT_GEGLU && (a.N & 63)) return FGDM_ERR_ARG;
     if (a.ln_stats && (a.mode != IG_LINEAR || a.C1 || a.ln_slots <= 0 || !a.ln_u)) return FGDM_ERR_ARG;
diff --git a/fgdm_amd/csrc/igemm2.hip b/fgdm_amd/csrc/igemm2.hip
--- a/fgdm_amd/csrc/igemm2.hip
+++ b/fgdm_amd/csrc/igemm2.hip
@@ -1,5 +1,6 @@
 #include "common.h"
 #include "knobs.h"
+#include "skip_fold.h"
 #include <algorithm>
 #include <type_traits>
 
@@ -36,8 +37,11 @@
 template <int BM, int BN, int STAGES, int PIPE> constexpr int ring_bytes() {
     return PIPE == 2 ? 2 * halo_px<BM>() * ROWB + STAGES * BN * ROWB : STAGES * (BM + BN) * ROWB;
 }
-
-template <int BM, int BN, int WM, int WN, int STAGES, int CONV, bool GEGLU, bool SPLIT, int MS, bool LN, int PATH, int PIPE, bool ABL>
+template <int BM, int BN, int STAGES, int PIPE, bool PRO> constexpr int ring_bytes_pro() {
+    return PRO && ring_bytes<BM, BN, STAGES, 1>() > ring_bytes<BM, BN, STAGES, PIPE>() ? ring_bytes<BM, BN, STAGES, 1>() : ring_bytes<BM, BN, STAGES, PIPE>();
+}
+
+template <int BM, int BN, int WM, int WN, int STAGES, int CONV, bool GEGLU, bool SPLIT, int MS, bool LN, int PATH, int PIPE, bool ABL, bool PRO = false>
 __device__ __forceinline__ void igemm2_body(const IgemmArgs& a, const int yb) {
     constexpr int NW = WM * WN, T = NW * 64;
     constexpr int TM = BM / WM, TN = BN / WN;
@@ -52,7 +56,8 @@
     constexpr int LPS = LA + LB;
     constexpr int STAGE_BYTES = (BM + BN) * ROWB;
     constexpr int A_BYTES = BM * ROWB;
-    constexpr int RING_BYTES = ring_bytes<BM, BN, STAGES, PIPE>();
+    constexpr int RING_BYTES = ring_bytes_pro<BM, BN, STAGES, PIPE, PRO>();
+    static_assert(!PRO || (MS == 16 && STAGES == 4 && !SPLIT && !LN && !GEGLU && !ABL && PIPE != 0), "prologue GEMM: the pipelined loops' plain tiles");
     static_assert(TM % 32 == 0 && TN % MS == 0, "wave tile: 32-pixel epilogue passes, MFMA-sized channel tiles");
     static_assert(!GEGLU || TN % 64 == 0, "GEGLU: whole 64-row [32 value | 32 gate] groups per wave");
     extern __shared__ __attribute__((aligned(16))) char smem[];
@@ -82,6 +87,115 @@
     const int per = (nk_all + nsplit - 1) / nsplit;
     const int k_begin = split * per;
     const int nk = max(0, min(per, nk_all - k_begin));
+
+    acc_t acc[NI][MI];
+#pragma unroll
+    for (int j = 0; j < NI; ++j)
+#pragma unroll
+        for (int i = 0; i < MI; ++i)
+#pragma unroll
+            for (int r = 0; r < AR; ++r) acc[j][i][r] = 0.f;
+
+    const int lrow = lane & (MS - 1), lh = lane / MS, swz = swz_of(lrow);
+    const int lq = 4 * lh;
+    int koff[KS];
+#pragma unroll
+    for (int ks = 0; ks < KS; ++ks) koff[ks] = lrow * ROWB + ((((MS == 32 ? ks * 2 : 0) + lh) ^ swz) << 4);
+
+    if constexpr (PRO) {
+        const int pnk = a.pK >> 5;
+        unsigned p_b0[LA], p_b1[LA], p_bb[LB], p_ok = 0;
+        int p_lds[LB];
+#pragma unroll
+        for (int i = 0; i < LA; ++i) {
+            const int q = (wave + i * NW) * 64 + lane, r = q >> 2, sp = q & 3, m = m0 + r;
+            const unsigned off = (unsigned)((sp ^ swz_of(r)) << 3);
+            p_b0[i] = p_b1[i] = 0;
+            if (m < a.M) {
+                p_ok |= 1u << i;
+                p_b0[i] = ((unsigned)m * (unsigned)a.pC0 + off) * 2u;
+                p_b1[i] = ((unsigned)m * (unsigned)a.pC1 + off) * 2u;
+            }
+        }
+#pragma unroll
+        for (int i = 0; i < LB; ++i) {
+            int idx = wave + i * NW;
+            if (idx >= B_INSTR) idx = B_INSTR - 1;
+            const int q = idx * 64 + lane, r = q >> 2, sp = q & 3;
+            p_bb[i] = ((unsigned)(n0 + r) * (unsigned)a.pK + (unsigned)((sp ^ swz_of(r)) << 3)) * 2u;
+            p_lds[i] = A_BYTES + idx * 1024;
+        }
+        const unsigned lds0 = __builtin_amdgcn_readfirstlane(lds_addr(smem));
+        auto p_piece = [&](int kn, int p) {
+            const int pc = kn << 5;
+            const bool s1 = pc >= a.pC0;
+            const char* sbase = s1 ? (const char*)(a.pA1 + (pc - a.pC0)) : (const char*)(a.pA0 + pc);
+            const unsigned lbase = lds0 + (unsigned)(kn & 3) * STAGE_BYTES;
+            if (p < LA) glds16_m0(((p_ok >> p) & 1) ? sbase + (s1 ? p_b1[p] : p_b0[p]) : (const char*)a.zero, lbase + (unsigned)(wave + p * NW) * 1024u);
+            else glds16_sv(p_bb[p - LA], (const char*)a.pWt + ((size_t)kn << 6), lbase + (unsigned)p_lds[p - LA]);
+        };
+#pragma unroll
+        for (int sg = 0; sg < STAGES - 1; ++sg)
+            if (sg < pnk) {
+#pragma unroll
+                for (int pp = 0; pp < LPS; ++pp) p_piece(sg, pp);
+            }
+        constexpr int RW = NI % 5 == 0 ? 5 : 4, WD = 3;
+        static_assert(NI % RW == 0 && WD < RW && NI >= RW, "W ring");
+        auto rdX = [&](int kt, int i) { return *(const h8*)(smem + (kt & 3) * STAGE_BYTES + (wm * TM + i * MS) * ROWB + koff[0]); };
+        auto rdW = [&](int kt, int j) { return *(const h8*)(smem + (kt & 3) * STAGE_BYTES + A_BYTES + (wn * TN + j * MS) * ROWB + koff[0]); };
+        h8 xa[MI], xb[MI], wr[RW];
+        {
+            const int younger = min(pnk - 1, STAGES - 2);
+            if (younger >= 2) wait_vmcnt<2 * LPS>(); else if (younger == 1) wait_vmcnt<LPS>(); else wait_vmcnt<0>();
+            __builtin_amdgcn_s_barrier();
+#pragma unroll
+            for (int i = 0; i < MI; ++i) xa[i] = rdX(0, i);
+#pragma unroll
+            for (int d = 0; d < WD; ++d) wr[d] = rdW(0, d);
+        }
+        auto step = [&](auto RF, int kt, h8 (&cur)[MI], h8 (&nxt)[MI]) {
+            constexpr bool REFILL = decltype(RF)::value;
+            if (REFILL || kt + 2 < pnk) wait_vmcnt<LPS>(); else wait_vmcnt<0>();
+            __builtin_amdgcn_s_waitcnt(0xC07F);
+            __builtin_amdgcn_s_barrier();
+#pragma unroll
+            for (int j = 0; j < NI; ++j) {
+                __builtin_amdgcn_sched_barrier(0);
+                if constexpr (REFILL) {
+#pragma unroll
+                    for (int p = 0; p < LPS; ++p)
+                        if (p * NI / LPS == j) p_piece(kt + STAGES - 1, p);
+                }
+                { const int jn = j + WD; wr[jn % RW] = jn < NI ? rdW(kt, jn) : rdW(kt + 1, jn - NI); }
+#pragma unroll
+                for (int i = 0; i < MI; ++i)
+                    if (i * NI / MI == j) nxt[i] = rdX(kt + 1, i);
+#pragma unroll
+                for (int i = 0; i < MI; ++i)
+                    acc[j][i] = __builtin_amdgcn_mfma_f32_16x16x32_f16(wr[j % RW], cur[i], acc[j][i], 0, 0, 0);
+            }
+            __builtin_amdgcn_sched_barrier(0);
+        };
+        const int nr = max(pnk - (STAGES - 1), 0);
+        int kt = 0;
+        for (; kt + 1 < nr; kt += 2) {
+            step(std::true_type{}, kt, xa, xb);
+            step(std::true_type{}, kt + 1, xb, xa);
+        }
+        if (kt < nr) {
+            step(std::true_type{}, kt, xa, xb);
+            ++kt;
+#pragma unroll
+            for (int i = 0; i < MI; ++i) xa[i] = xb[i];
+        }
+        if (kt < pnk) step(std::false_type{}, kt, xa, xb);
+        if (kt + 1 < pnk) step(std::false_type{}, kt + 1, xb, xa);
+        if (kt + 2 < pnk) step(std::false_type{}, kt + 2, xa, xb);
+        wait_vmcnt<0>();
+        asm volatile("s_waitcnt lgkmcnt(0)" ::: "memory");
+        __builtin_amdgcn_s_barrier();
+    }
 
     int a_pix[LA], a_yx[LA], a_off[LA];
     int b_off[LB], b_lds[LB];
@@ -183,20 +297,6 @@
 #pragma unroll
         for (int p = 0; p < LPS; ++p) stage_piece(kt, tap, cc, buf, p);
     };
-
-    acc_t acc[NI][MI];
-#pragma unroll
-    for (int j = 0; j < NI; ++j)
-#pragma unroll
-        for (int i = 0; i < MI; ++i)
-#pragma unroll
-            for (int r = 0; r < AR; ++r) acc[j][i][r] = 0.f;
-
-    const int lrow = lane & (MS - 1), lh = lane / MS, swz = swz_of(lrow);
-    const int lq = 4 * lh;
-    int koff[KS];
-#pragma unroll
-    for (int ks = 0; ks < KS; ++ks) koff[ks] = lrow * ROWB + ((((MS == 32 ? ks * 2 : 0) + lh) ^ swz) << 4);
 
     int tap = 0, cc = k_begin << 5;
     if (CONV) { const int q = k_begin >> 1; tap = q % NT; cc = (q / NT) * 64 + (k_begin & 1) * 32; }
@@ -274,6 +374,9 @@
     const int last_row = min(m0 + BM, a.M) - 1;
     const int nsmp = a.rowvec ? last_row / rps - smp0 + 1 : 0;
     const bool rv_in_lds = nsmp <= RV_MAX;
+    if constexpr (PRO) {
+        for (int c = tid; c < BN; c += T) bias_l[c] = (a.bias ? a.bias[n0 + c] : 0.f) + (a.bias2 ? a.bias2[n0 + c] : 0.f);
+    } else
     for (int c = tid; c < BN; c += T) bias_l[c] = a.bias ? a.bias[n0 + c] : 0.f;
     if constexpr (LN) {
         for (int c = tid; c < BN; c += T) u_l[c] = a.ln_u[n0 + c];
@@ -749,14 +852,14 @@
     }
 }
 
-template <int BM, int BN, int WM, int WN, int STAGES, int CONV, bool GEGLU, bool SPLIT, int MS, bool LN, int PATH, int PIPE, bool ABL>
+template <int BM, int BN, int WM, int WN, int STAGES, int CONV, bool GEGLU, bool SPLIT, int MS, bool LN, int PATH, int PIPE, bool ABL, bool PRO = false>
 __global__ __launch_bounds__(WM * WN * 64) void igemm2_kernel(const IgemmArgs a) {
-    igemm2_body<BM, BN, WM, WN, STAGES, CONV, GEGLU, SPLIT, MS, LN, PATH, PIPE, ABL>(a, (int)blockIdx.y);
+    igemm2_body<BM, BN, WM, WN, STAGES, CONV, GEGLU, SPLIT, MS, LN, PATH, PIPE, ABL, PRO>(a, (int)blockIdx.y);
 }
 struct IgemmArgsG { IgemmArgs g[FGDM_MAX_GROUP]; };
-template <int BM, int BN, int WM, int WN, int STAGES, int CONV, bool GEGLU, bool SPLIT, int MS, bool LN, int PATH, int PIPE, bool ABL>
+template <int BM, int BN, int WM, int WN, int STAGES, int CONV, bool GEGLU, bool SPLIT, int MS, bool LN, int PATH, int PIPE, bool ABL, bool PRO = false>
 __global__ __launch_bounds__(WM * WN * 64) void igemm2_pair_kernel(const IgemmArgsG p) {
-    igemm2_body<BM, BN, WM, WN, STAGES, CONV, GEGLU, SPLIT, MS, LN, PATH, PIPE, ABL>(p.g[blockIdx.y], 0);
+    igemm2_body<BM, BN, WM, WN, STAGES, CONV, GEGLU, SPLIT, MS, LN, PATH, PIPE, ABL, PRO>(p.g[blockIdx.y], 0);
 }
 
 template <bool LN>
@@ -1011,12 +1114,12 @@
     return hipGetLastError() == hipSuccess ? FGDM_OK : FGDM_ERR_HIP;
 }
 
-template <int BM, int BN, int WM, int WN, int STAGES, int CONV, bool GEGLU, bool SPLIT, int MS, bool LN, int PATH, int PIPE, bool ABL>
+template <int BM, int BN, int WM, int WN, int STAGES, int CONV, bool GEGLU, bool SPLIT, int MS, bool LN, int PATH, int PIPE, bool ABL, bool PRO = false>
 int launch2p(const IgemmArgs& a, hipStream_t s) {
-    constexpr int ring = ring_bytes<BM, BN, STAGES, PIPE>();
+    constexpr int ring = ring_bytes_pro<BM, BN, STAGES, PIPE, PRO>();
     constexpr int smem = ring + (1 + RV_MAX) * BN * 4 + (2 * BM + BN) * 4;
     static_assert(smem <= 160 * 1024, "LDS budget");
-    constexpr auto k = igemm2_kernel<BM, BN, WM, WN, STAGES, CONV, GEGLU, SPLIT, MS, LN, PATH, PIPE, ABL>;
+    constexpr auto k = igemm2_kernel<BM, BN, WM, WN, STAGES, CONV, GEGLU, SPLIT, MS, LN, PATH, PIPE, ABL, PRO>;
     if (fgdm_dyn_lds<k>(smem) != FGDM_OK) return FGDM_ERR_HIP;
     const int ntm = (a.M + BM - 1) / BM, ntn = (a.N + BN - 1) / BN;
     const unsigned gx = (unsigned)(ntm * ntn * (SPLIT ? a.splitk : 1));
@@ -1029,14 +1132,14 @@
         };
         if (phases) { fgdm_record(single); return FGDM_OK; }
         if constexpr (PIPE != 0 && PATH != 0 && !SPLIT && !ABL && MS == 16) {
-            constexpr auto kp = igemm2_pair_kernel<BM, BN, WM, WN, STAGES, CONV, GEGLU, SPLIT, MS, LN, PATH, PIPE, ABL>;
+            constexpr auto kp = igemm2_pair_kernel<BM, BN, WM, WN, STAGES, CONV, GEGLU, SPLIT, MS, LN, PATH, PIPE, ABL, PRO>;
             if (fgdm_dyn_lds<kp>(smem) != FGDM_OK) return FGDM_ERR_HIP;
             static_assert(sizeof(IgemmArgs) <= FGDM_GROUP_BLOB, "the recorded blob holds an IgemmArgs");
             FgdmGroupFn pf = [](const void* const* av, int n, unsigned grid_x, hipStream_t rs) -> int {
                 if (n < 2 || n > FGDM_MAX_GROUP) return FGDM_ERR_ARG;
                 IgemmArgsG pg;
                 for (int i = 0; i < FGDM_MAX_GROUP; ++i) pg.g[i] = *(const IgemmArgs*)av[i < n ? i : 0];
-                hipLaunchKernelGGL((igemm2_pair_kernel<BM, BN, WM, WN, STAGES, CONV, GEGLU, SPLIT, MS, LN, PATH, PIPE, ABL>), dim3(grid_x, n),
+                hipLaunchKernelGGL((igemm2_pair_kernel<BM, BN, WM, WN, STAGES, CONV, GEGLU, SPLIT, MS, LN, PATH, PIPE, ABL, PRO>), dim3(grid_x, n),
                                    dim3(WM * WN * 64), smem, rs, pg);
                 return hipGetLastError() == hipSuccess ? FGDM_OK : FGDM_ERR_HIP;
             };
@@ -1155,9 +1258,26 @@
 }
 
 static bool halo_geometry(const IgemmArgs& a) {
-    if (a.mode != IG_CONV3 || a.Ho != a.H || a.Wo != a.W || (a.C0 & 63) || (a.C1 & 63) || (a.K % 288) || a.debug) return false;
-    if ((a.W == 16 || a.W == 32 || a.W == 64) && (a.H * a.W) % 256 == 0) return true;
-    return a.W == 8 && a.H == 8;
+    return !a.debug && halo_geometry_dims(a.mode == IG_CONV3, a.H, a.W, a.Ho, a.Wo, a.C0, a.C1, a.K);
+}
+static bool small_operands(size_t rows, int C0, int C1, int N, int K) {
+    return rows * (size_t)std::max(C0, C1) * 2 < (1ull << 32) && (size_t)(N + 320) * K * 2 < (1ull << 32);
+}
+bool igemm2_prologue_ok(const IgemmArgs& a, int cfg) {
+    const int tile = cfg & 15, psel = cfg >> 4;
+    const size_t px = (size_t)a.B * a.H * a.W;
+    SkipFoldQuery q{};
+    q.conv3_s1 = a.mode == IG_CONV3 && !a.debug;
+    q.H = a.H; q.W = a.W; q.Ho = a.Ho; q.Wo = a.Wo; q.C0 = a.C0; q.C1 = a.C1; q.K = a.K; q.N = a.N;
+    q.tile = tile;
+    q.pipe = (psel == 0 ? knob_once(KNOB_IGEMM_PIPE) != 0 : psel == 2) && small_operands(px, a.C0, a.C1, a.N, a.K);
+    q.halo_on = knob_once(KNOB_IGEMM_HALO) != 0;
+    q.splitk = a.splitk > 1 ? a.splitk : 1;
+    q.plain_epilogue = knob_once(KNOB_IGEMM_EPI_PATHS) != 0 && a.out_kind == OUT_F16 && a.act == ACT_NONE && !a.rowvec && !a.resid && !a.stats_out &&
+                       !a.out2 && !a.ln_stats;
+    q.pC0 = a.pC0; q.pC1 = a.pC1; q.pK = a.pK; q.pN = a.N;
+    q.p_small = small_operands((size_t)a.M, a.pC0, a.pC1, a.N, a.pK);
+    return a.pA0 && a.pWt && (a.pC1 == 0 || a.pA1) && a.M == a.B * a.Ho * a.Wo && skip_fold_rule(q);
 }
 
 int igemm2_launch(const IgemmArgs& a, int cfg, hipStream_t s) {
@@ -1165,7 +1285,7 @@
     const int pipe_default = knob_once(KNOB_IGEMM_PIPE);
     const int tile = cfg & 15, psel = cfg >> 4;
     const size_t px = a.mode == IG_LINEAR ? (size_t)a.M : (size_t)a.B * a.H * a.W;
-    const bool small = px * (size_t)std::max(a.C0, a.C1) * 2 < (1ull << 32) && (size_t)(a.N + 320) * a.K * 2 < (1ull << 32);
+    const bool small = small_operands(px, a.C0, a.C1, a.N, a.K);
     const bool pipe = (psel == 0 ? pipe_default != 0 : psel == 2) && small;
     if (a.mode == IG_CONV2_PHASE && (a.splitk > 1 || a.C1 || a.out_kind != OUT_F16 || a.stats_out || a.out2 || a.ln_stats || a.act == ACT_GEGLU ||
                                      a.Ho != 2 * a.H || a.Wo != 2 * a.W || a.K != 4 * a.C0 || a.M != a.B * a.H * a.W || !small))
@@ -1174,6 +1294,11 @@
     const int bn = (tile == 1 || tile == 4) ? 256 : tile == 6 ? 128 : tile == 7 ? 160 : 320;
     if (a.N % bn) return FGDM_ERR_ARG;
     if (a.act == ACT_GEGLU && bn != 256) return FGDM_ERR_ARG;
+    if (a.pK) {
+        if (!igemm2_prologue_ok(a, cfg) || !halo) return FGDM_ERR_ARG;
+        return tile == 0 ? launch2p<256, 320, 4, 2, 4, 1, false, false, 16, false, 1, 2, false, true>(a, s)
+                         : launch2p<128, 320, 4, 2, 4, 1, false, false, 16, false, 1, 2, false, true>(a, s);
+    }
     if (a.splitk > 1) {
         if ((tile != 2 && tile != 0) || a.ln_stats) return FGDM_ERR_ARG;
         const int nk_all = a.K >> 5;
diff --git a/fgdm_amd/csrc/knobs.h b/fgdm_amd/csrc/knobs.h
--- a/fgdm_amd/csrc/knobs.h
+++ b/fgdm_amd/csrc/knobs.h
@@ -20,6 +20,7 @@
     X(IGEMM_PERSIST, "FGDM_IGEMM_PERSIST", "1", "GEGLU projections: 1 = persistent, tiles round-robin; 2 = contiguous runs; 0 = off") \
     X(IGEMM_PIPE, "FGDM_IGEMM_PIPE", "1", "0: the phase-locked K loop instead of the software-pipelined one")                   \
     X(IGEMM_UP_PHASE, "FGDM_IGEMM_UP_PHASE", "1", "0: Upsample convs as the 3x3 walk over the virtual upsampled image, not four 2x2 phase GEMMs") \
+    X(IGEMM_SKIP_FOLD, "FGDM_IGEMM_SKIP_FOLD", "1", "0: a ResBlock's 1x1 skip projection as a launch of its own, not the prologue GEMM of its second conv") \
     X(IGEMM_SMALL_M, "FGDM_IGEMM_SMALL_M", "1", "0: linears with a thin 128-row grid stay on 128 x 320 tiles")                  \
     X(IGEMM_SMALL_TILES, "FGDM_IGEMM_SMALL_TILES", "1", "0: the 8x8 level's linears back on the 2-stage kernel")                \
     X(IGEMM_STATS64, "FGDM_IGEMM_STATS64", "1", "0: the 64 x 160 tile leaves the LayerNorm partial sums to the row-statistics pass") \
diff --git a/fgdm_amd/csrc/ops_abi.hip b/fgdm_amd/csrc/ops_abi.hip
--- a/fgdm_amd/csrc/ops_abi.hip
+++ b/fgdm_amd/csrc/ops_abi.hip
@@ -1,5 +1,6 @@
 #include "engine_shared.h"
 #include "replay_plan.h"
+#include "skip_fold.h"
 
 static int op_pack(IgemmArgs& a, TmpDev& tmp, const float* w, const float* bias, int N, int K, int Ks, bool geglu,
                    const int* kmap = nullptr, const float* gamma = nullptr, const float* beta = nullptr) {
@@ -326,6 +327,58 @@
     return dpmpp_loop_step(a, as_stream(stream));
 }
 
+int fgdm_op_conv2d_skip(const void* x, int Cc, const float* w, const float* bias, const void* sx0, int sC0, const void* sx1, int sC1,
+                        const float* sw, const float* sbias, int B, int H, int W, int Cout, void* out, int* folded, void* stream) {
+    if (!x || !w || !sx0 || !sw || !out || B <= 0 || H <= 0 || W <= 0 || Cout <= 0 || Cc <= 0 || (Cc & 63) || sC0 <= 0 || (sC0 & 63) ||
+        sC1 < 0 || (sC1 & 63) || (sC1 > 0) != (sx1 != nullptr))
+        return FGDM_ERR_ARG;
+    hipStream_t s = as_stream(stream);
+    const int K = 9 * Cc, pK = sC0 + sC1, M = B * H * W;
+    std::vector<int> kmap(K);
+    for (int tap = 0; tap < 9; ++tap)
+        for (int c = 0; c < Cc; ++c) kmap[((c >> 6) * 9 + tap) * 64 + (c & 63)] = c * 9 + tap;
+    TmpDev tmp;
+    IgemmArgs a{}, l{};
+    int prc = op_pack(a, tmp, w, bias, Cout, K, K, false, kmap.data());
+    if (prc == FGDM_OK) prc = op_pack(l, tmp, sw, sbias, Cout, pK, pK, false);
+    if (prc != FGDM_OK) return prc;
+    a.zero = l.zero = g_zero_page();
+    if (!a.zero) return FGDM_ERR_NOMEM;
+    a.A0 = (const half_t*)x; a.C0 = Cc;
+    a.B = B; a.H = H; a.W = W; a.Ho = H; a.Wo = W; a.mode = IG_CONV3;
+    a.M = M; a.N = Cout; a.K = K;
+    a.act = ACT_NONE; a.out_kind = OUT_F16; a.out = out; a.ld_out = Cout; a.rows_per_sample = H * W; a.scale = 1.f;
+    if (plan_splitk(a, tmp) != FGDM_OK) return FGDM_ERR_NOMEM;
+    a.pA0 = (const half_t*)sx0; a.pC0 = sC0; a.pA1 = (const half_t*)sx1; a.pC1 = sC1; a.pWt = l.Wt; a.bias2 = l.bias; a.pK = pK;
+    const bool fold = igemm_skip_fold(a);
+    if (folded) *folded = fold ? 1 : 0;
+    int rc = FGDM_OK;
+    if (!fold) {
+        a.pA0 = a.pA1 = a.pWt = nullptr; a.bias2 = nullptr; a.pC0 = a.pC1 = a.pK = 0;
+        half_t* sk = tmp.alloc<half_t>((size_t)M * Cout);
+        if (!sk) return FGDM_ERR_NOMEM;
+        l.A0 = (const half_t*)sx0; l.C0 = sC0; l.A1 = (const half_t*)sx1; l.C1 = sC1;
+        l.B = B; l.H = H; l.W = W; l.Ho = H; l.Wo = W; l.mode = IG_LINEAR;
+        l.M = M; l.N = Cout; l.K = pK;
+        l.act = ACT_NONE; l.out_kind = OUT_F16; l.out = sk; l.ld_out = Cout; l.rows_per_sample = H * W; l.scale = 1.f;
+        if (plan_splitk(l, tmp) != FGDM_OK) return FGDM_ERR_NOMEM;
+        rc = igemm_launch(l, s);
+        a.resid = sk; a.ld_res = Cout;
+    }
+    if (rc == FGDM_OK) rc = igemm_launch(a, s);
+    (void)hipStreamSynchronize(s);
+    return rc;
+}
+
+int fgdm_skip_fold_rule(int conv3_s1, int H, int W, int Ho, int Wo, int C0, int C1, int N, int tile, int pipe, int halo_on, int splitk,
+                        int plain_epilogue, int pC0, int pC1, int pN, int p_small) {
+    SkipFoldQuery q{};
+    q.conv3_s1 = conv3_s1 != 0; q.H = H; q.W = W; q.Ho = Ho; q.Wo = Wo; q.C0 = C0; q.C1 = C1; q.K = 9 * (C0 + C1); q.N = N;
+    q.tile = tile; q.pipe = pipe != 0; q.halo_on = halo_on != 0; q.splitk = splitk; q.plain_epilogue = plain_epilogue != 0;
+    q.pC0 = pC0; q.pC1 = pC1; q.pK = pC0 + pC1; q.pN = pN; q.p_small = p_small != 0;
+    return skip_fold_rule(q) ? 1 : 0;
+}
+
 int fgdm_replay_plan(int n_walks, const int32_t* lens, const uint64_t* key, const uint32_t* grid_x, const uint64_t* shape, int group_max,
                      int chunk, int32_t* out, int out_cap, int* limits) {
     if (limits) { limits[0] = REPLAY_LOOK; limits[1] = FGDM_MAX_GROUP; }
diff --git a/fgdm_amd/csrc/skip_fold.h b/fgdm_amd/csrc/skip_fold.h
--- /dev/null
+++ b/fgdm_amd/csrc/skip_fold.h
@@ -0,0 +1,28 @@
+#pragma once
+
+inline bool halo_geometry_dims(bool conv3_s1, int H, int W, int Ho, int Wo, int C0, int C1, int K) {
+    if (!conv3_s1 || Ho != H || Wo != W || (C0 & 63) || (C1 & 63) || (K % 288)) return false;
+    if ((W == 16 || W == 32 || W == 64) && (H * W) % 256 == 0) return true;
+    return W == 8 && H == 8;
+}
+
+struct SkipFoldQuery {
+    bool conv3_s1;
+    int H, W, Ho, Wo;
+    int C0, C1, K, N;
+    int tile;
+    bool pipe;
+    bool halo_on;
+    int splitk;
+    bool plain_epilogue;
+    int pC0, pC1, pK, pN;
+    bool p_small;
+};
+
+inline bool skip_fold_rule(const SkipFoldQuery& q) {
+    if (q.pK <= 0 || (q.pK & 31) || q.pC0 <= 0 || (q.pC0 & 31) || q.pC1 < 0 || (q.pC1 & 31) || q.pC0 + q.pC1 != q.pK) return false;
+    if (q.pN != q.N || q.N % 320 || !q.p_small) return false;
+    if (q.tile != 0 && q.tile != 2) return false;
+    if (q.splitk != 1 || !q.pipe || !q.halo_on || !q.plain_epilogue) return false;
+    return halo_geometry_dims(q.conv3_s1, q.H, q.W, q.Ho, q.Wo, q.C0, q.C1, q.K);
+}
diff --git a/include/fgdm.h b/include/fgdm.h
--- a/include/fgdm.h
+++ b/include/fgdm.h
@@ -203,6 +203,11 @@
 int fgdm_replay_plan(int n_walks, const int32_t* lens, const uint64_t* key, const uint32_t* grid_x, const uint64_t* shape,
                      int group_max, int chunk, int32_t* out, int out_cap, int* limits);
 
+int fgdm_skip_fold_rule(int conv3_s1, int H, int W, int Ho, int Wo, int C0, int C1, int N, int tile, int pipe, int halo_on, int splitk,
+                        int plain_epilogue, int pC0, int pC1, int pN, int p_small);
+int fgdm_op_conv2d_skip(const void* x, int Cc, const float* w, const float* bias, const void* sx0, int sC0, const void* sx1, int sC1,
+                        const float* sw, const float* sbias, int B, int H, int W, int Cout, void* out, int* folded, void* stream);
+
 #define FGDM_STRIDE2_PAD_BR (-2)
 int fgdm_op_conv2d(const void* x0, int C0, const void* x1, int C1, const float* w, const float* bias,
                    const float* rowvec, const void* resid, int B, int H, int W, int Cout, int ksize, int stride,
```

Result: no change. 8.224, median of 6 (+0.4%).
